# jenndrei/BayHunter

Hardware: AMD Instinct MI355X
Metric: forward-model+logL evals/sec (batched 10-layer models) (higher is better)
Workload: dtype f64

## Files before the change

bayhunter_amd/csrc/bh_device.h:

```cpp
#pragma once
#include <hip/hip_runtime.h>
#include <stddef.h>
#include <stdint.h>

#define BH_WAVE 64
#define BH_COUNTER_WORDS 16
#define BH_TRACE_WAVES 16384
#define BH_DEBUG_WORDS (BH_COUNTER_WORDS + 4 * BH_TRACE_WAVES)
#define BH_BOARD_WORDS (2 * 32768)

__device__ __forceinline__ double bh_rcp_refined(double b)
{
    double r = __builtin_amdgcn_rcp(b);
    double e = __builtin_fma(-b, r, 1.0);
    r = __builtin_fma(r, e, r);
    e = __builtin_fma(-b, r, 1.0);
    r = __builtin_fma(r, e, r);
    return r;
}
__device__ __forceinline__ double bh_quot(double a, double b, double r)
{
    const double q = a * r;
    const double rem = __builtin_fma(-b, q, a);
    return __builtin_fma(rem, r, q);
}
__device__ __forceinline__ bool bh_div_safe(double x)
{
    const unsigned ex = ((unsigned)__double2hiint(x) >> 20) & 0x7ffu;
    return (ex - 623u) <= 800u;
}

#include <atomic>
inline bool bh_allow_big_lds(std::atomic<unsigned long long> *done, const void *const *kernels, int nkernels, int bytes)
{
    int dev = 0;
    if (hipGetDevice(&dev) != hipSuccess || dev < 0 || dev > 63) return false;
    const unsigned long long bit = 1ull << dev;
    if (done->load(std::memory_order_acquire) & bit) return true;
    for (int k = 0; k < nkernels; ++k)
        if (hipFuncSetAttribute(kernels[k], hipFuncAttributeMaxDynamicSharedMemorySize, bytes) != hipSuccess) return false;
    done->fetch_or(bit, std::memory_order_release);
    return true;
}

struct SwdKernelArgs {
    int B, Lmax, K, igr, mode;
    const int32_t *nlay;
    const int32_t *perm;
    const double *h, *vp, *vs, *rho;
    ptrdiff_t sl, sb;
    const double *periods;
    double *vel;
    int ldv;
    int32_t *err;
    unsigned long long *neval;
    int look;
    int fair;
    double *nev_high;
    int fast;
    int counted;
    int farith;
    int32_t *gcount, *glist;
    int second, Bm;
    double *first;
};

struct SwdLaneBuild {
    int key[6];
    unsigned grid_x;
    int fair;
};
void bh_launch_swd(const SwdKernelArgs &a, int iwave, hipStream_t stream, SwdLaneBuild *build = nullptr);
void bh_launch_order(int B, const int32_t *nlay, int32_t *perm, int Lcut, int32_t *split, hipStream_t stream);
size_t bh_swd_lds_bytes(int Lmax, int K, int mode);
size_t bh_swd_nev_high_doubles(int B, int look);

struct SwdTarget {
    int iwave, igr, K, ldv, mode;
    int look;
    int inlook;
    const double *h, *vp, *vs, *rho;
    ptrdiff_t sl, sb;
    const double *periods;
    double *vel;
    int32_t *err;
    const int32_t *perm;
    const int32_t *count;
    int32_t *gcount, *glist;
    int refseq;
    double *first;
};
struct SwdMultiArgs {
    int B, Lmax, ntargets;
    const int32_t *nlay;
    const int32_t *perm;
    const int32_t *split;
    int Lcut;
    int rows[2], lanes[2];
    int wg_n0, wg_n1;
    unsigned long long *neval;
    unsigned *board;
    unsigned stamp;
    unsigned *started;
    int prio_low;
    int fast;
    int adapt_ok;
    int counted;
    int rerun;
    int farith;
    int restart;
    SwdTarget t[8];
};
struct SwdSiteXArgs {
    const int32_t *site;
    int nsites, nt, ldx;
    const int32_t *n;
    const double *x;
    int col[8], off[8];
};
__device__ __forceinline__ int bh_site_count(const SwdSiteXArgs &X, int ty, int ib, int cap)
{
    const int s = X.site[ib];
    if (s < 0 || s >= X.nsites) return -1;
    const int n = X.n[(size_t)s * X.nt + X.col[ty]];
    return n < 0 ? 0 : (n > cap ? cap : n);
}
__device__ __forceinline__ int bh_site_periods(const SwdSiteXArgs &X, int ty, int ib, int cap, const double *&per)
{
    const int n = bh_site_count(X, ty, ib, cap);
    per = n < 0 ? X.x : X.x + (size_t)X.site[ib] * X.ldx + X.off[ty];
    return n;
}
void bh_launch_swd_second_x(const SwdKernelArgs &a, int iwave, const SwdSiteXArgs &x, int ty, hipStream_t stream, SwdLaneBuild *build = nullptr);
int bh_swd_pick_group(int B, int ntargets, int Lmax);
double bh_swd_plan(int B, int Lmax, int ntargets, const int *iwave, int Gforce, int *G, int *look);
size_t bh_swd_group_lds_bytes(int G, int J, int Lmax, int Kmax, int maxmode, bool sitex = false);
struct SwdPairWork {
    int ncu = 0;
    int32_t *perm[2] = {nullptr, nullptr};
    int32_t *slot_rank[2] = {nullptr, nullptr};
    int cap_perm = 0, cap_rank[2] = {0, 0};
    int key_n0 = -1, key_n1 = -1;
};
struct PairOrderTarget {
    int mpw, nwaves;
    const int32_t *slot_rank;
    int32_t *perm;
    int xcd;
};
bool bh_pair_order_fits(int B);
void bh_launch_pair_order(int B, int Lmax, const int32_t *nlay, const double *vs, ptrdiff_t sl, ptrdiff_t sb, int nt,
                          const PairOrderTarget *tg, hipStream_t stream);
struct SwdLaunchInfo {
    unsigned workgroups;
    long waves;
    size_t lds;
    int wpb;
};
inline int bh_trials_fit(int G, int look)
{
    int J = look > 1 ? look : 1;
    while (J > 1 && G * J > BH_WAVE) --J;
    return J;
}
struct SwdGroupAsk {
    int B, Lmax, Lcut, ntargets;
    int G0;
    struct Target {
        int K, look, iwave, mode;
        bool group, refseq;
    } t[8];
    bool fast, farith, restart;
    bool adapt_ok, rerun;
    bool counters;
    bool sitex;
    int scan;
};
struct SwdGroupBuild {
    int fastm;
    bool simple, prof, adapt, cntb, fa;
};
struct SwdGroupPlan {
    bool fits;
    int rows[2], lanes[2];
    int wg_n0, wg_n1;
    size_t wave_lds, lds;
    dim3 grid, block;
    int Gflags;
    bool restart;
    SwdGroupBuild build;
    bool pair;
    int pair_mpw[2], pair_waves[2];
    SwdLaunchInfo info;
};
struct BhTuning;
SwdGroupPlan bh_plan_swd_group(const SwdGroupAsk &q, const BhTuning &tun);
void bh_launch_swd_group(const SwdMultiArgs &a, const SwdGroupPlan &g, hipStream_t stream);
bool bh_launch_swd_group_x(const SwdMultiArgs &a, const SwdGroupPlan &g, const SwdSiteXArgs &x, hipStream_t stream);
struct SwdGroupXStream {
    hipStream_t st;
    const SwdSiteXArgs *x;
};
bool bh_swd_group_builds_fa_x(const SwdMultiArgs &a, const SwdGroupPlan &g, SwdGroupXStream s);
bool bh_swd_group_builds_adapt_x(const SwdMultiArgs &a, const SwdGroupPlan &g, SwdGroupXStream s);
bool bh_swd_group_builds_big_x(const SwdMultiArgs &a, const SwdGroupPlan &g, SwdGroupXStream s);
bool bh_swd_group_builds_fa(const SwdMultiArgs &a, const SwdGroupPlan &g, hipStream_t stream);
bool bh_swd_group_builds_adapt(const SwdMultiArgs &a, const SwdGroupPlan &g, hipStream_t stream);
bool bh_swd_group_builds_big(const SwdMultiArgs &a, const SwdGroupPlan &g, hipStream_t stream);
int bh_swd_lean_trials(int B, int ntargets);
size_t bh_swd_lean_lds_bytes(int J, int Lmax, int Kmax, bool sitex = false);
int bh_launch_swd_lean(const SwdMultiArgs &a, hipStream_t stream, SwdLaunchInfo *info, SwdLaneBuild *build = nullptr);
int bh_launch_swd_lean_x(const SwdMultiArgs &a, const SwdSiteXArgs &x, hipStream_t stream, SwdLaunchInfo *info, SwdLaneBuild *build = nullptr);
void bh_launch_sphere(int B, int Lmax, const int32_t *nlay, const double *h, const double *vp,
                      const double *vs, const double *rho, ptrdiff_t sl, ptrdiff_t sb, double *oh,
                      double *ovp, double *ovs, double *orho_love, double *orho_ray, hipStream_t stream);
void bh_launch_interp(int B, int K0, const double *x0, const double *y0, int ld0, int K1,
                      const double *x1, double *y1, int ld1, hipStream_t stream);

struct RfKernelArgs {
    int B, Lmax, nsamp, nkeep, waveno;
    const int32_t *nlay;
    const double *h, *vp, *vs, *rho, *qp, *qs;
    ptrdiff_t sl, sb;
    double p_s_per_deg, gauss, fsamp, tshift, nsv;
    double *coef;
    double *rf;
    int ldr;
    const double *yobs;
    double *sums;
    double *zwork;
    int lds_min;
    int no_realc;
    int coef_small;
    int no_rot;
};
struct RfSiteArgs {
    const int32_t *site;
    int nsites;
    int ld;
    const double *p, *nsv;
};
size_t bh_rf_coef_doubles(int Lmax);
constexpr size_t BH_RF_MAX_LDS = 160 * 1024;
constexpr int BH_RF_MAX_NSAMP = 1 << 18;
size_t bh_rf_lds_bytes(int nsamp);
int bh_launch_rf(const RfKernelArgs &a, hipStream_t stream, const RfSiteArgs *sites = nullptr);
struct RfSiteMArgs : RfSiteArgs {
    const int32_t *n;
};
int bh_launch_rf_m(const RfKernelArgs &a, hipStream_t stream, const RfSiteMArgs &sites);
struct RfAxisRec {
    double fsamp, tshift, gauss;
    int32_t nsamp, logm, jcut;
    int32_t pad;
};
struct RfSiteTArgs : RfSiteMArgs {
    const RfAxisRec *axis;
    int nsamp_max;
};
RfAxisRec bh_rf_axis_record(int nsamp, double fsamp, double tshift, double gauss);
int bh_launch_rf_t(const RfKernelArgs &a, hipStream_t stream, const RfSiteTArgs &sites);
int bh_launch_rf_probe(int op, int n, const double *in, double *out, hipStream_t stream);

struct LikeTargetDev {
    int law, n, off;
    const double *yobs, *yerr_scaled, *rinv;
    double logdet_extra;
    const double *quad;
    int nsplit;
    const double *pre;
};
int bh_gauss_nsplit(int B, int n);
void bh_launch_gauss_quad(int B, int n, int ldy, const double *ymod, const double *yobs,
                          const double *rinv, int nsplit, double *partial, hipStream_t stream);
struct GaussSiteArgs {
    const int32_t *site;
    int nsites, ldo;
};
void bh_launch_gauss_quad_sites(int B, int n, int ldy, const double *ymod, const double *yobs, const GaussSiteArgs &sites,
                                const double *rinv, int nsplit, double *partial, hipStream_t stream);
struct GaussClassArgs {
    const int32_t *class_of;
    int nclass;
    const int32_t *row_start;
    const int32_t *tile_start;
    const int32_t *perm;
};
inline size_t bh_gauss_class_work_words(int B, int nclass) { return 4 * (size_t)nclass + 2 + (size_t)B; }
void bh_launch_gauss_quad_classes(int B, int n, int ldy, const double *ymod, const double *yobs, const GaussSiteArgs &sites,
                                  const int32_t *class_of, int nclass, const double *rinv, int nsplit, double *partial,
                                  int32_t *work, hipStream_t stream);
struct LikeKernelArgs {
    int B, nt, ldy;
    const double *ymod;
    const int32_t *err_t;
    const double *noise;
    LikeTargetDev t[8];
    double *logL;
    double *misfits;
    int32_t *err;
};
void bh_launch_like(const LikeKernelArgs &a, hipStream_t stream);
inline bool bh_like_small_form(const LikeKernelArgs &a, size_t *lds)
{
    *lds = 0;
    bool small = true;
    for (int t = 0; t < a.nt; ++t) {
        if (a.t[t].law == 3 && a.t[t].quad == nullptr && (size_t)a.t[t].n * sizeof(double) > *lds) *lds = (size_t)a.t[t].n * sizeof(double);
        small = small && (a.t[t].n <= 64 || (a.t[t].pre != nullptr && a.t[t].law != 3)) && !(a.t[t].law == 3 && a.t[t].quad == nullptr);
    }
    return small;
}
struct LikeSiteArgs {
    const int32_t *site;
    int nsites;
    const double *yobs;
    const double *yerr_scaled;
    const double *logdet_extra;
};
void bh_launch_like_sites(const LikeKernelArgs &a, const LikeSiteArgs &sites, hipStream_t stream);
struct LikeSiteXArgs : LikeSiteArgs {
    const int32_t *n;
};
void bh_launch_like_sites_x(const LikeKernelArgs &a, const LikeSiteXArgs &sites, hipStream_t stream);
void bh_launch_like_sites_m(const LikeKernelArgs &a, const LikeSiteXArgs &sites, hipStream_t stream);
struct LikeClassArgs {
    const int32_t *class_of[8];
    const double *rinv[8];
    const double *logdet[8];
};
void bh_launch_like_sites_c(const LikeKernelArgs &a, const LikeSiteXArgs &sites, const LikeClassArgs &classes, hipStream_t stream);
struct LikeLawArgs {
    const int32_t *law;
};
void bh_launch_like_sites_l(const LikeKernelArgs &a, const LikeSiteXArgs &sites, const LikeClassArgs &classes, const LikeLawArgs &laws,
                            hipStream_t stream);

void bh_launch_probe(int op, int n, const double *in, double *out, hipStream_t stream);


struct bh_engine;
__attribute__((visibility("hidden"))) int bh_engine_fail_internal(bh_engine *e, int code, const char *what);
__attribute__((visibility("hidden"))) int bh_engine_device_internal(const bh_engine *e);
```

bayhunter_amd/csrc/bh_engine.hip:

```cpp
#include "../../include/bh_engine_debug.h"
#include "../../include/bh_engine_sites.h"
#include "../../include/bh_engine_sites_rf.h"
#include "../../include/bh_engine_sites_x.h"
#include "../../include/bh_engine_sites_x_all.h"
#include "../../include/bh_engine_sites_missing.h"
#include "../../include/bh_engine_sites_gauss.h"
#include "../../include/bh_engine_sites_rf_axis.h"
#include "../../include/bh_engine_sites_laws.h"
#include "bh_device.h"

#include <algorithm>
#include <cmath>
#include <cstdio>
#include <cstdlib>
#include <cstring>
#include <new>
#include <string>
#include <vector>

#include "bh_tuning.h"
#include <cstring>
#include <mutex>

namespace {
BhTuning g_tuning;
std::once_flag g_tuning_once;
int tuning_value(const char *env, const char *txt, int dflt)
{
    if (!txt) return dflt;
    if (!std::strcmp(env, "BH_SWD_SEARCH")) return (txt[0] == 'f' || txt[0] == '1') ? ((std::strstr(txt, "ray") || txt[0] == '2') ? BH_SEARCH_FAST_RAYLEIGH : BH_SEARCH_FAST) : (txt[0] == '2' ? BH_SEARCH_FAST_RAYLEIGH : BH_SEARCH_REFERENCE);
    if (!std::strcmp(env, "BH_SWD_ARITH")) return (txt[0] == 'e' || txt[0] == '0') ? BH_ARITH_EXACT : BH_ARITH_FAST;
    if (!std::strcmp(env, "BH_SWD_SCAN")) return (txt[0] == 's' || txt[0] == '0') ? BH_SCAN_STEPS : ((txt[0] == 'c' || txt[0] == '1') ? BH_SCAN_COUNTED : BH_SCAN_AUTO);
    char *end = nullptr;
    const long v = std::strtol(txt, &end, 10);
    if (end == txt) return 1;
    return (int)v;
}
void tuning_clamp()
{
    if (g_tuning.rf_lds_gated < 0 || g_tuning.rf_lds_gated > 160 * 1024) g_tuning.rf_lds_gated = 0;
    if (g_tuning.rf_lds_beside > 160 * 1024) g_tuning.rf_lds_beside = -1;
    if (g_tuning.swd_love_inlook < 0 || g_tuning.swd_love_inlook > 4) g_tuning.swd_love_inlook = 0;
    if (g_tuning.swd_gsplit < 0 || g_tuning.swd_gsplit > (1 << 24)) g_tuning.swd_gsplit = 0;
}
void tuning_parse()
{
#ifndef BH_NO_EXPERIMENTS
#define X(field, env, dflt, doc) g_tuning.field = tuning_value(env, std::getenv(env), dflt);
    BH_TUNING_TABLE(X)
#undef X
    tuning_clamp();
#endif
    g_tuning.under_pmc = std::getenv("ROCPROF_COUNTER_COLLECTION") != nullptr ? 1 : 0;
}
}
const BhTuning &bh_tuning()
{
    std::call_once(g_tuning_once, tuning_parse);
    return g_tuning;
}
int bh_tuning_set(const char *name, int value)
{
#ifdef BH_NO_EXPERIMENTS
    (void)name; (void)value;
    return -1;
#else
    (void)bh_tuning();
    if (!name) return -1;
#define X(field, env, dflt, doc) if (!std::strcmp(name, #field)) { g_tuning.field = value; tuning_clamp(); return 0; }
    BH_TUNING_TABLE(X)
#undef X
    return -1;
#endif
}
int bh_tuning_get(const char *name, int *value)
{
    const BhTuning &t = bh_tuning();
    if (!name || !value) return -1;
#define X(field, env, dflt, doc) if (!std::strcmp(name, #field)) { *value = t.field; return 0; }
    BH_TUNING_TABLE(X)
#undef X
    return -1;
}

namespace {

struct DevBuf {
    void *p = nullptr;
    size_t cap = 0;
};

struct TargetHost {
    bh_target_desc d{};
    int off = 0;
    DevBuf x, yobs, yerr_scaled, rinv, quad;
    DevBuf sums;
    DevBuf x60, vel60;
    int kfwd = 0;
    double logdet_extra = 0.0;
    int gc_nclass = 0;
    DevBuf gc_rinv, gc_logdet, gc_class;
    bool site_lacks = false;
    bool law_other = false;
    bool rf_own_counts = false;
    int axis_nsamp_max = 0;
};

}

struct bh_engine {
    int device = 0;
    hipStream_t stream = nullptr;
    hipStream_t aux = nullptr;
    hipEvent_t ev_fork = nullptr, ev_join = nullptr;
    hipStream_t aux2 = nullptr;
    hipEvent_t ev_fork2 = nullptr, ev_join2 = nullptr;
    bool overlap_rf = true;
    int rf_lds_beside_swd = 40 * 1024;
    unsigned *started = nullptr;
    unsigned started_expected = 0;
    int swd_prio_low = 1;
    SwdPairWork pairwork{};
    int swd_trials = 0;
    int last_swd_kernel = -1;
    bh_swd_launch swd_launches[3 * BH_MAX_TARGETS]{};
    int n_swd_launches = 0;
    int err_t_nt = -1, err_t_B = -1;
    std::string err;
    DevBuf nlay, h, vp, vs, rho, qp, qs, periods, vel, errb, rf, coef, ymod, noise, logL,
        misfits, err_t, probe_in, probe_out, counter, sph, perm, board, nevhi, rfz, gfirst, nevhi2;
    unsigned swd_stamp = 0;
    int nt = 0;
    int ldy = 0;
    std::vector<TargetHost> targets;
    int nsites = 0;
    DevBuf site_yobs, site_yerr, site_logdet;
    DevBuf site_idx;
    bool site_rf = false;
    DevBuf site_p, site_nsv;
    bool site_rf_axis = false;
    DevBuf site_axis;
    bool site_x = false;
    bool site_x_all = false;
    bool site_missing = false;
    DevBuf site_xn, site_xper;
    std::vector<int32_t> site_xn_host;
    bool site_missing_gauss = false;
    DevBuf gc_xn;
    DevBuf gc_work;
    bool site_laws = false;
    DevBuf law_tab, law_yerr, law_logdet;
    std::vector<int32_t> site_law_host;
    bool timing = false, counting = false;
    bool no_mfma = false;
    bool as_given = false;
    int force_group = 0;
    int force_look = 0;
    int hint_layers = 0;
    int swd_search = BH_SEARCH_FAST;
    int swd_arith = BH_ARITH_FAST;
    int swd_scan = 2;
    DevBuf guard;
    uint64_t rerun_launches = 0;
    uint64_t guard_total[BH_MAX_TARGETS] = {0};
    bool guard_fresh = true;
    bool guard_last = false;
    struct EventSet {
        hipEvent_t ev[8];
        bool used[4];
    };
    std::vector<EventSet> evsets;
    size_t ncalls = 0;
    uint64_t last_neval = 0;
    bool neval_pending = false;
};

namespace {

int fail(bh_engine *e, int code, const char *what, hipError_t he = hipSuccess)
{
    if (e) {
        e->err = what;
        if (he != hipSuccess) {
            e->err += ": ";
            e->err += hipGetErrorString(he);
        }
    }
    return code;
}

#define HIPCHK(e, call)                                                  \
    do {                                                                 \
        hipError_t _he = (call);                                         \
        if (_he != hipSuccess) return fail((e), BH_EHIP, #call, _he);    \
    } while (0)

int ensure(bh_engine *e, DevBuf &b, size_t bytes)
{
    if (bytes <= b.cap) return BH_OK;
    if (b.p) {
        HIPCHK(e, hipStreamSynchronize(e->stream));
        if (e->aux) HIPCHK(e, hipStreamSynchronize(e->aux));
        if (e->aux2) HIPCHK(e, hipStreamSynchronize(e->aux2));
        HIPCHK(e, hipFree(b.p));
        b.p = nullptr;
        b.cap = 0;
    }
    size_t want = bytes + bytes / 4 + 256;
    hipError_t he = hipMalloc(&b.p, want);
    if (he != hipSuccess) return fail(e, BH_ENOMEM, "hipMalloc", he);
    b.cap = want;
    return BH_OK;
}

void release(DevBuf &b)
{
    if (b.p) (void)hipFree(b.p);
    b.p = nullptr;
    b.cap = 0;
}

void release_target(TargetHost &t)
{
    for (DevBuf *b : {&t.x, &t.yobs, &t.yerr_scaled, &t.rinv, &t.quad, &t.sums, &t.x60, &t.vel60, &t.gc_rinv, &t.gc_logdet, &t.gc_class}) release(*b);
    t.gc_nclass = 0;
}

void release_gauss_classes(bh_engine *e)
{
    for (auto &t : e->targets) {
        for (DevBuf *b : {&t.gc_rinv, &t.gc_logdet, &t.gc_class}) release(*b);
        t.gc_nclass = 0;
    }
    release(e->gc_xn);
}

void release_laws(bh_engine *e)
{
    for (DevBuf *b : {&e->law_tab, &e->law_yerr, &e->law_logdet}) release(*b);
    e->site_laws = false;
    e->site_law_host.clear();
    for (auto &t : e->targets) t.law_other = false;
    release_gauss_classes(e);
}

void release_sites(bh_engine *e)
{
    for (DevBuf *b : {&e->site_yobs, &e->site_yerr, &e->site_logdet, &e->site_idx, &e->site_p, &e->site_nsv, &e->site_xn, &e->site_xper, &e->site_axis}) release(*b);
    e->nsites = 0;
    e->site_rf = e->site_rf_axis = false;
    e->site_x = e->site_x_all = e->site_missing = e->site_missing_gauss = false;
    e->site_xn_host.clear();
    release_laws(e);
    for (auto &t : e->targets) {
        t.site_lacks = t.rf_own_counts = false;
        t.axis_nsamp_max = 0;
    }
}

double scaled_errors(const double *yerr, int n, double *out)
{
    double mn = yerr[0];
    for (int i = 0; i < n; ++i) mn = yerr[i] < mn ? yerr[i] : mn;
    double prod = 1.0;
    for (int i = 0; i < n; ++i) {
        out[i] = yerr[i] / mn;
        prod *= out[i];
    }
    return std::log(prod);
}

size_t span_elems(int B, int Lmax, ptrdiff_t sl, ptrdiff_t sb)
{
    return (size_t)((ptrdiff_t)(Lmax - 1) * sl + (ptrdiff_t)(B - 1) * sb + 1);
}

__global__ void rho_from_vp_kernel(size_t n, const double *vp, double *rho)
{
    const size_t i = (size_t)blockIdx.x * blockDim.x + threadIdx.x;
    if (i < n) rho[i] = vp[i] * 0.32 + 0.77;
}

int check_models(bh_engine *e, int B, int Lmax, ptrdiff_t sl, ptrdiff_t sb)
{
    if (!e) return BH_EINVAL;
    if (B < 0 || Lmax < 1 || Lmax > BH_MAX_LAYERS) return fail(e, BH_EINVAL, "bad B or Lmax (1..100)");
    if (sl <= 0 || sb <= 0) return fail(e, BH_EINVAL, "strides must be positive");
    return BH_OK;
}

struct Staged {
    const int32_t *nlay;
    const double *h, *vp, *vs, *rho, *qp, *qs;
    int typ_layers = 0;
};

int stage_models(bh_engine *e, int B, int Lmax, ptrdiff_t sl, ptrdiff_t sb, Staged &m)
{
    const size_t bytes = span_elems(B, Lmax, sl, sb) * sizeof(double);
    {
        long sum = 0;
        for (int b = 0; b < B; ++b) sum += m.nlay[b];
        m.typ_layers = B > 0 ? (int)((sum + B - 1) / B) : 0;
    }
    int rc;
    if ((rc = ensure(e, e->nlay, (size_t)B * sizeof(int32_t)))) return rc;
    HIPCHK(e, hipMemcpyAsync(e->nlay.p, m.nlay, (size_t)B * sizeof(int32_t), hipMemcpyHostToDevice, e->stream));
    m.nlay = (const int32_t *)e->nlay.p;
    const double **arr[6] = {&m.h, &m.vp, &m.vs, &m.rho, &m.qp, &m.qs};
    DevBuf *buf[6] = {&e->h, &e->vp, &e->vs, &e->rho, &e->qp, &e->qs};
    for (int k = 0; k < 6; ++k) {
        if (!*arr[k]) continue;
        if ((rc = ensure(e, *buf[k], bytes))) return rc;
        HIPCHK(e, hipMemcpyAsync(buf[k]->p, *arr[k], bytes, hipMemcpyHostToDevice, e->stream));
        *arr[k] = (const double *)buf[k]->p;
    }
    return BH_OK;
}

bh_engine::EventSet *cur_set(bh_engine *e)
{
    return (e->timing && e->ncalls > 0) ? &e->evsets[e->ncalls - 1] : nullptr;
}
void ev_begin(bh_engine *e, int fam, hipStream_t st)
{
    bh_engine::EventSet *s = cur_set(e);
    if (!s) return;
    if (!s->used[fam]) {
        (void)hipEventRecord(s->ev[2 * fam], st);
        s->used[fam] = true;
    }
}
void ev_end(bh_engine *e, int fam, hipStream_t st)
{
    bh_engine::EventSet *s = cur_set(e);
    if (s) (void)hipEventRecord(s->ev[2 * fam + 1], st);
}
void call_begin(bh_engine *e, hipStream_t st)
{
    e->neval_pending = false;
    if (!e->timing) return;
    if (e->ncalls == e->evsets.size()) {
        bh_engine::EventSet s{};
        for (auto &ev : s.ev)
            if (hipEventCreate(&ev) != hipSuccess) return;
        e->evsets.push_back(s);
    }
    bh_engine::EventSet &s = e->evsets[e->ncalls++];
    for (bool &u : s.used) u = false;
    (void)hipEventRecord(s.ev[6], st);
    s.used[3] = true;
}
void call_end(bh_engine *e, hipStream_t st)
{
    bh_engine::EventSet *s = cur_set(e);
    if (s) (void)hipEventRecord(s->ev[7], st);
}

int swd_supported(bh_engine *e, int K, int iwave, int &igr, int mode, int flsph)
{
    if (K < 0 || K > BH_MAX_PERIODS) return fail(e, BH_EINVAL, "K must be 0..60 (surfdisp96.f:61-62)");
    if (iwave != BH_WAVE_LOVE && iwave != BH_WAVE_RAYLEIGH) return fail(e, BH_EINVAL, "iwave must be 1 (Love) or 2 (Rayleigh)");
    if (igr < 0) return fail(e, BH_EINVAL, "igr must be 0 (phase velocity) or > 0 (group velocity)");
    if (mode < 1 || mode > 16) return fail(e, BH_EINVAL, "mode must be 1..16");
    if (flsph != 0 && flsph != 1) return fail(e, BH_EINVAL, "flsph must be 0 or 1");
    igr = igr > 0 ? BH_VEL_GROUP : BH_VEL_PHASE;
    return BH_OK;
}

struct SwdSiteJob {
    const SwdSiteXArgs *tab;
    int col, off;
};

struct SwdJob {
    int K, iwave, igr, ldv;
    const double *periods_dev;
    double *vel;
    int32_t *err;
    int mode = 1;
    int flsph = 0;
    SwdSiteJob sx{};
};

int swd_counter(bh_engine *e, hipStream_t st, unsigned long long **out)
{
    *out = nullptr;
    if (!e->counting) return BH_OK;
    int rc = ensure(e, e->counter, BH_DEBUG_WORDS * sizeof(unsigned long long));
    if (rc) return rc;
    if (!e->neval_pending) {
        HIPCHK(e, hipMemsetAsync(e->counter.p, 0, BH_COUNTER_WORDS * sizeof(unsigned long long), st));
        e->neval_pending = true;
    }
    *out = (unsigned long long *)e->counter.p;
    return BH_OK;
}

constexpr int GUARD_HEAD = 24;
int guard_space(bh_engine *e, hipStream_t st, int B, int32_t **counts, int32_t **lists)
{
    const size_t need = ((size_t)GUARD_HEAD + (size_t)BH_MAX_TARGETS * (size_t)(B + 4)) * sizeof(int32_t);
    if (need > e->guard.cap) {
        if (e->guard.p) {
            int32_t cum[BH_MAX_TARGETS];
            HIPCHK(e, hipStreamSynchronize(st));
            HIPCHK(e, hipMemcpy(cum, (int32_t *)e->guard.p + 2 * BH_MAX_TARGETS, sizeof(cum), hipMemcpyDeviceToHost));
            for (int t = 0; t < BH_MAX_TARGETS; ++t) e->guard_total[t] += (uint64_t)(uint32_t)cum[t];
        }
        e->guard_fresh = true;
    }
    int rc = ensure(e, e->guard, need);
    if (rc) return rc;
    *counts = (int32_t *)e->guard.p;
    *lists = (int32_t *)e->guard.p + GUARD_HEAD;
    HIPCHK(e, hipMemsetAsync(e->guard.p, 0, (e->guard_fresh ? GUARD_HEAD : 2 * BH_MAX_TARGETS) * sizeof(int32_t), st));
    e->guard_fresh = false;
    return BH_OK;
}

bool takes_fast(int search, const SwdJob &J)
{
    return J.igr == BH_VEL_PHASE && J.mode <= 1 && (search == BH_SEARCH_FAST || (search == BH_SEARCH_FAST_RAYLEIGH && J.iwave == BH_WAVE_RAYLEIGH));
}

enum SwdOrder { ORDER_NONE, ORDER_DEPTH, ORDER_LENGTH, ORDER_PAIR };

struct SwdPlan {
    bool first_roots[BH_MAX_TARGETS];
    int nsplit;
    int ntargets, kmax, maxmode;
    bool any_sphere;
    int typ_layers;
    int kernel;
    int G, lean_trials;
    int order, Lcut;
    int len_mpw, len_xcd;
    bool sitex;
    bool any_fast, farith, adapt_ok;
    int job[BH_MAX_TARGETS], look[BH_MAX_TARGETS], inlook[BH_MAX_TARGETS], look_group[BH_MAX_TARGETS];
    bool fast[BH_MAX_TARGETS], refseq[BH_MAX_TARGETS];
};

SwdPlan plan_swd(const bh_engine *e, int B, int Lmax, int typ_given, int njobs, const SwdJob *jobs)
{
    const BhTuning &tun = bh_tuning();
    SwdPlan p{};
    p.maxmode = 1;
    for (int j = 0; j < njobs; ++j) p.sitex = p.sitex || jobs[j].sx.tab != nullptr;
    int iw[BH_MAX_TARGETS], nfast = 0;
    for (int j = 0; j < njobs; ++j) {
        const SwdJob &J = jobs[j];
        if (J.K == 0) continue;
        p.first_roots[j] = J.igr == BH_VEL_GROUP && J.mode <= 1 && tun.swd_gsplit > 0 && (long)B * J.K <= (long)tun.swd_gsplit;
        p.nsplit += p.first_roots[j] ? 1 : 0;
        const int t = p.ntargets++;
        p.job[t] = j;
        iw[t] = J.iwave;
        p.fast[t] = takes_fast(e->swd_search, J);
        nfast += p.fast[t] ? 1 : 0;
        p.kmax = J.K > p.kmax ? J.K : p.kmax;
        p.maxmode = J.mode > p.maxmode ? J.mode : p.maxmode;
        p.any_sphere = p.any_sphere || J.flsph == 1;
    }
    const int nlive = p.ntargets;
    if (nlive == 0) return p;
    p.typ_layers = ((long)nlive * B <= 2048 && tun.swd_hint_always == 0) ? 0 : typ_given;
    int look[BH_MAX_TARGETS];
    {
        int Lplan = p.typ_layers > 0 ? p.typ_layers : Lmax;
        if (Lplan > Lmax) Lplan = Lmax;
        bh_swd_plan(B, Lplan, nlive, iw, e->force_group, &p.G, look);
        if (e->force_look > 0)
            for (int t = 0; t < nlive; ++t) look[t] = e->force_look;
    }
    const size_t lds_cap = 64 * 1024;
    if (p.G <= 1 && (p.sitex || bh_swd_lds_bytes(Lmax, p.kmax, p.maxmode) > lds_cap)) p.G = 2;
    {
        bool all = e->swd_arith == BH_ARITH_FAST && e->swd_search == BH_SEARCH_FAST && e->force_group == 0 && e->force_look == 0 &&
                   tun.swd_look_r == 0 && tun.swd_look_l == 0 && tun.swd_no_lean == 0 && p.maxmode <= 1 && p.kmax <= BH_MAX_PERIODS &&
                   Lmax <= 32 && (long)B * nlive <= (tun.swd_lean_pairs > 0 ? (long)tun.swd_lean_pairs : (1L << 20));
        for (int t = 0; t < nlive; ++t) all = all && jobs[p.job[t]].igr == BH_VEL_PHASE;
        if (all) p.lean_trials = e->swd_trials > 0 ? e->swd_trials : bh_swd_lean_trials(B, nlive);
        if (p.lean_trials >= 4 && bh_swd_lean_lds_bytes(p.lean_trials, Lmax, p.kmax, p.sitex) > lds_cap) p.lean_trials = 0;
    }
    const bool lean = p.lean_trials >= 4;
    if (lean && p.G <= 1) p.G = bh_swd_pick_group(B, nlive, Lmax);
    p.kernel = p.G <= 1 ? BH_KERNEL_LANE : (lean ? BH_KERNEL_LEAN : BH_KERNEL_GROUP);
    const bool ordered = B > 1 && tun.no_order == 0 && !e->as_given;
    const bool shallow_bulk = p.typ_layers > 0 && p.typ_layers + 2 < Lmax;
    if (ordered && !lean && tun.swd_no_pair == 0 && p.G > 1 && nlive == 2 && bh_pair_order_fits(B) && !shallow_bulk) {
        long plan_waves = 0, wmin = 0, wmax = 0;
        for (int t = 0; t < nlive; ++t) {
            const int mpw = BH_WAVE / (p.G * bh_trials_fit(p.G, look[t]));
            const long w = (B + mpw - 1) / mpw;
            plan_waves += w;
            wmin = (t == 0 || w < wmin) ? w : wmin;
            wmax = w > wmax ? w : wmax;
        }
        const int pair_min = tun.swd_pair_minwaves;
        if (plan_waves >= (pair_min >= 0 ? pair_min : 7 * (long)e->pairwork.ncu) && (pair_min >= 0 || 2 * wmax >= 3 * wmin))
            p.order = ORDER_PAIR;
    }
    p.Lcut = Lmax;
    if (ordered && p.order != ORDER_PAIR) {
        if (lean && bh_pair_order_fits(B) && tun.swd_lean_no_sort == 0) {
            p.order = ORDER_LENGTH;
            p.len_mpw = 1;
            const int mpw = BH_WAVE / p.lean_trials, per_wg = (nlive == 2) ? 2 : 4;
            if (tun.swd_lean_xcd != 0 && tun.swd_lean_r < 4 && tun.swd_lean_l < 4 && B % mpw == 0 && B % 8 == 0 && (B / mpw) % (8 * per_wg) == 0) {
                p.len_mpw = mpw;
                p.len_xcd = per_wg;
            }
        } else {
            p.order = ORDER_DEPTH;
            if (shallow_bulk) p.Lcut = p.typ_layers + 2;
        }
    }
    p.any_fast = nfast > 0;
    p.farith = e->swd_arith == BH_ARITH_FAST;
    p.adapt_ok = e->force_group == 0 && e->force_look == 0 && tun.swd_look_r == 0 && tun.swd_look_l == 0;
    for (int t = 0; t < nlive; ++t) {
        p.refseq[t] = nfast > 0 && jobs[p.job[t]].igr == BH_VEL_PHASE && !p.fast[t];
        if (p.kernel == BH_KERNEL_LANE) {
            p.look[t] = look[t] > 1 ? look[t] : 1;
            continue;
        }
        p.inlook[t] = (iw[t] != BH_WAVE_LOVE) ? 1 : (tun.swd_love_inlook > 0 ? tun.swd_love_inlook : (look[t] <= 2 ? 2 : 1));
        int L = look[t];
        if (tun.swd_look_r > 0 && iw[t] == BH_WAVE_RAYLEIGH) L = tun.swd_look_r;
        if (tun.swd_look_l > 0 && iw[t] == BH_WAVE_LOVE) L = tun.swd_look_l;
        p.look_group[t] = L;
        if (lean) {
            L = p.lean_trials;
            if (iw[t] == BH_WAVE_RAYLEIGH && tun.swd_lean_r >= 4) L = tun.swd_lean_r;
            if (iw[t] == BH_WAVE_LOVE && tun.swd_lean_l >= 4) L = tun.swd_lean_l;
        }
        p.look[t] = L;
    }
    return p;
}

enum EvalRole { ROLE_NONE, ROLE_SWD, ROLE_SWD60, ROLE_RF };
enum EvalLike { LIKE_PLAIN, LIKE_SITES, LIKE_SITES_X, LIKE_SITES_M, LIKE_SITES_C, LIKE_SITES_L };
enum EvalGauss { GAUSS_PLAIN, GAUSS_SITES, GAUSS_CLASSES };

struct EvalPlan {
    int B, nt, ldy;
    EvalRole role[BH_MAX_TARGETS];
    bool rf_fused[BH_MAX_TARGETS];
    int nswd;
    bool no_forward;
    bool fork;
    bool want_gate;
    int prio_low;
    bool x_table, rf_table;
    bool missing;
    bool rf_needs_table;
    bool rf_axis;
    bool rf_axis_needs_table;
    bool rf_axis_gauss_needs_table;
    bool rf_axis_no_mfma;
    EvalGauss gauss[BH_MAX_TARGETS];
    bool gauss_needs_table;
    bool laws;
    bool law_gauss_needs_table;
    EvalLike like;
    bool err_zero_always;
};

EvalPlan plan_eval(const bh_engine *e, int B, bool sites, bool want_ymod)
{
    const BhTuning &tun = bh_tuning();
    EvalPlan p{};
    p.B = B; p.nt = e->nt; p.ldy = e->ldy;
    bool have_rf = false;
    for (int t = 0; t < p.nt; ++t) {
        const TargetHost &T = e->targets[(size_t)t];
        const bh_target_desc &d = T.d;
        if (d.kind == BH_TARGET_SWD) {
            p.role[t] = T.kfwd == d.n ? ROLE_SWD : ROLE_SWD60;
            ++p.nswd;
        } else if (d.kind == BH_TARGET_RF) {
            p.role[t] = ROLE_RF;
            have_rf = true;
            p.rf_fused[t] = !want_ymod && !sites && tun.rf_no_fuse == 0 && (d.law == BH_LAW_NOCORR || d.law == BH_LAW_EXP) && tun.rf_threads != 128;
        } else {
            p.no_forward = true;
        }
    }
    p.fork = have_rf && p.nswd > 0 && e->overlap_rf;
    p.want_gate = p.fork && e->started != nullptr;
    p.prio_low = p.want_gate ? e->swd_prio_low : 0;
    p.x_table = sites && e->site_x;
    p.rf_table = sites && e->site_rf;
    p.missing = p.x_table && e->site_missing;
    p.rf_needs_table = p.missing && have_rf && !p.rf_table;
    p.rf_axis = p.rf_table && p.x_table && e->site_rf_axis;
    p.like = p.missing ? LIKE_SITES_M : (p.x_table ? LIKE_SITES_X : (sites ? LIKE_SITES : LIKE_PLAIN));
    for (int t = 0; t < p.nt; ++t) {
        const TargetHost &T = e->targets[(size_t)t];
        p.gauss[t] = !sites ? GAUSS_PLAIN : (T.gc_nclass > 0 ? GAUSS_CLASSES : GAUSS_SITES);
        if (sites && T.rf_own_counts && !p.rf_axis) p.rf_axis_needs_table = true;
        if (T.d.law != BH_LAW_GAUSS) continue;
        if (p.gauss[t] == GAUSS_CLASSES) p.like = LIKE_SITES_C;
        else if (sites && e->site_missing_gauss && T.site_lacks) p.gauss_needs_table = true;
        else if (sites && T.rf_own_counts) p.rf_axis_gauss_needs_table = true;
        if (sites && T.rf_own_counts && e->no_mfma) p.rf_axis_no_mfma = true;
    }
    p.laws = p.x_table && e->site_laws;
    if (p.laws) {
        p.like = LIKE_SITES_L;
        for (int t = 0; t < p.nt; ++t) {
            const TargetHost &T = e->targets[(size_t)t];
            if (T.d.law == BH_LAW_GAUSS && T.law_other && p.gauss[t] != GAUSS_CLASSES) p.law_gauss_needs_table = true;
        }
    }
    p.err_zero_always = tun.err_memset != 0;
    return p;
}

unsigned gate_need(const SwdLaunchInfo &s)
{
    const unsigned resident = 2048u / (unsigned)(s.lds > 0 && s.wpb > 0 ? s.wpb : 2);
    return s.workgroups < resident ? s.workgroups : resident;
}

struct RfPlace {
    int lds_min = 0, coef_small = 0;
};

RfPlace rf_place(bool beside_swd, bool gated, const BhTuning &tun, int rf_lds_beside_swd)
{
    RfPlace w;
    if (!beside_swd) return w;
    w.lds_min = !gated ? rf_lds_beside_swd : (tun.rf_lds_gated > 0 ? tun.rf_lds_gated : 0);
    w.coef_small = (gated && tun.rf_coef_big == 0) ? 1 : 0;
    return w;
}

SwdGroupPlan plan_group(const bh_engine *e, const SwdPlan &p, int B, int Lmax, const SwdJob *jobs)
{
    SwdGroupAsk q{};
    q.B = B; q.Lmax = Lmax; q.Lcut = p.Lcut; q.ntargets = p.ntargets; q.G0 = p.G;
    for (int t = 0; t < p.ntargets; ++t) {
        const SwdJob &J = jobs[p.job[t]];
        q.t[t] = SwdGroupAsk::Target{J.K, p.look[t], J.iwave, J.mode, J.igr != BH_VEL_PHASE, p.refseq[t]};
    }
    q.fast = p.any_fast; q.farith = p.farith;
    q.restart = true;
    q.adapt_ok = p.adapt_ok; q.counters = e->counting; q.scan = e->swd_scan; q.sitex = p.sitex;
    return bh_plan_swd_group(q, bh_tuning());
}

struct SwdCall {
    bh_engine *e; hipStream_t st;
    int B, Lmax; const Staged &m; ptrdiff_t sl, sb;
    const SwdJob *jobs; const SwdPlan &p;
    const double *sph = nullptr;
    double *first[BH_MAX_TARGETS] = {};
    SwdGroupPlan g{};
    const int32_t *perm = nullptr, *split = nullptr;
    const int32_t *pair_perm[2] = {};
    unsigned long long *counter = nullptr;
    int32_t *gcounts = nullptr, *glists = nullptr;
    SwdSiteXArgs sx{};
    int prio_low = 0;
    SwdLaunchInfo info{};
};

SwdTarget swd_target(const SwdCall &c, int j)
{
    const SwdJob &J = c.jobs[j];
    SwdTarget t{};
    t.iwave = J.iwave; t.igr = c.p.first_roots[j] ? 2 : J.igr; t.K = J.K; t.ldv = J.ldv; t.mode = J.mode;
    t.h = c.m.h; t.vp = c.m.vp; t.vs = c.m.vs; t.rho = c.m.rho; t.sl = c.sl; t.sb = c.sb;
    if (J.flsph == 1) {
        const size_t ne = (size_t)c.Lmax * c.B;
        t.h = c.sph; t.vp = c.sph + ne; t.vs = c.sph + 2 * ne; t.rho = c.sph + (J.iwave == BH_WAVE_LOVE ? 3 : 4) * ne;
        t.sl = c.B; t.sb = 1;
    }
    t.periods = J.periods_dev; t.vel = J.vel; t.err = J.err;
    t.first = c.first[j];
    return t;
}

SwdKernelArgs lane_args(const SwdCall &c, const SwdTarget &t)
{
    SwdKernelArgs a{};
    a.B = c.B; a.Lmax = c.Lmax; a.K = t.K; a.igr = t.igr; a.mode = t.mode; a.perm = c.perm;
    a.nlay = c.m.nlay; a.h = t.h; a.vp = t.vp; a.vs = t.vs; a.rho = t.rho; a.sl = t.sl; a.sb = t.sb;
    a.periods = t.periods; a.vel = t.vel; a.ldv = t.ldv; a.err = t.err; a.first = t.first;
    a.neval = c.counter; a.counted = c.e->swd_scan;
    return a;
}

int swd_board(bh_engine *e, hipStream_t st, unsigned **board)
{
    if (!e->board.p) {
        int rc = ensure(e, e->board, (size_t)BH_BOARD_WORDS * sizeof(unsigned));
        if (rc) return rc;
        HIPCHK(e, hipMemsetAsync(e->board.p, 0, (size_t)BH_BOARD_WORDS * sizeof(unsigned), st));
    }
    *board = (unsigned *)e->board.p;
    return BH_OK;
}

unsigned swd_stamp(bh_engine *e)
{
    const unsigned s = (++e->swd_stamp) & 0xffffu;
    return s != 0 ? s : (++e->swd_stamp) & 0xffffu;
}

int wait_for(bh_engine *e, hipEvent_t ev, hipStream_t from, hipStream_t to)
{
    HIPCHK(e, hipEventRecord(ev, from));
    HIPCHK(e, hipStreamWaitEvent(to, ev, 0));
    return BH_OK;
}

void note_launch(bh_engine *e, int family, int role, const int key[6], bool two, bool inter, bool pair, bool restart, unsigned grid_x, int fair)
{
    if (e->n_swd_launches >= (int)(sizeof(e->swd_launches) / sizeof(e->swd_launches[0]))) return;
    bh_swd_launch &r = e->swd_launches[e->n_swd_launches++];
    r.family = family; r.role = role;
    for (int k = 0; k < 6; ++k) r.key[k] = key[k];
    r.two_classes = two; r.interleaved = inter; r.pair_order = pair; r.restart = restart; r.grid_x = (int)grid_x; r.fair = fair;
}
void note_lane(bh_engine *e, int role, const SwdLaneBuild &b) { note_launch(e, BH_KERNEL_LANE, role, b.key, false, false, false, false, b.grid_x, b.fair); }
void note_group(bh_engine *e, int role, const SwdGroupPlan &g, bool pair)
{
    const SwdGroupBuild &b = g.build;
    const int key[6] = {b.fastm, b.simple, b.prof, b.adapt, b.cntb, b.fa};
    note_launch(e, BH_KERNEL_GROUP, role, key, g.grid.z == 2, g.wg_n1 > 0, pair, g.restart, g.grid.x, 0);
}

void set_group_args(SwdMultiArgs &a, const SwdGroupPlan &g)
{
    for (int k = 0; k < 2; ++k) {
        a.rows[k] = g.rows[k];
        a.lanes[k] = g.lanes[k];
    }
    a.wg_n0 = g.wg_n0;
    a.wg_n1 = g.wg_n1;
    a.fast = g.build.fastm;
    a.counted = g.build.cntb ? 1 : 0;
    a.farith = g.build.fa ? 1 : 0;
    a.restart = g.restart ? 1 : 0;
}

bool build_slot_ranks(int n0, int n1, int ncu, std::vector<int32_t> rank[2])
{
    const int NW = n0 + n1, nwg = (NW + 1) / 2;
    if (ncu <= 0 || nwg > 4 * ncu) return false;
    auto target_of = [&](int W, int &ty, int &wid) {
        if (n1 > 0) {
            const long long N = NW;
            const int l0 = (int)(((long long)W * n1) / N), l1 = (int)((((long long)W + 1) * n1) / N);
            ty = (l1 > l0) ? 1 : 0;
            wid = (l1 > l0) ? l0 : W - l0;
        } else {
            ty = 0;
            wid = W;
        }
    };
    std::vector<int> on_simd[2];
    on_simd[0].assign((size_t)ncu * 4, -1);
    on_simd[1].assign((size_t)ncu * 4, -1);
    for (int W = 0; W < NW; ++W) {
        const int g = W / 2, j = W % 2, cu = g % ncu, pass = g / ncu, simd = (pass + j) % 4;
        on_simd[j][(size_t)cu * 4 + simd] = W;
    }
    std::vector<double> q((size_t)NW, 0.0);
    int npairs = 0;
    for (size_t k = 0; k < on_simd[0].size(); ++k) npairs += (on_simd[0][k] >= 0 && on_simd[1][k] >= 0);
    int ip = 0;
    for (size_t k = 0; k < on_simd[0].size(); ++k) {
        const int a = on_simd[0][k], b = on_simd[1][k];
        if (a >= 0 && b >= 0) {
            const double u = (ip + 0.5) / (2.0 * npairs);
            q[(size_t)((ip & 1) ? a : b)] = u;
            q[(size_t)((ip & 1) ? b : a)] = 1.0 - u;
            ++ip;
        } else if (a >= 0) {
            q[(size_t)a] = 0.0;
        } else if (b >= 0) {
            q[(size_t)b] = 0.0;
        }
    }
    const int nw[2] = {n0, n1};
    for (int t = 0; t < 2; ++t) {
        std::vector<std::pair<double, int>> v;
        for (int W = 0; W < NW; ++W) {
            int ty, wid;
            target_of(W, ty, wid);
            if (ty == t && wid < nw[t] - 1) v.emplace_back(q[(size_t)W], wid);
        }
        std::sort(v.begin(), v.end());
        rank[t].assign((size_t)(nw[t] > 0 ? nw[t] : 1), 0);
        for (size_t r = 0; r < v.size(); ++r) rank[t][(size_t)v[r].second] = (int32_t)r;
    }
    return true;
}

int launch_swd_rerun(bh_engine *e, hipStream_t st, const SwdMultiArgs &main, int32_t *counts, int32_t *lists, const SwdSiteXArgs *sx = nullptr)
{
    SwdMultiArgs a = main;
    a.rerun = 1;
    a.perm = nullptr;
    a.split = nullptr;
    a.Lcut = a.Lmax;
    a.started = nullptr;
    a.stamp = swd_stamp(e);
    a.adapt_ok = 1;
    SwdGroupAsk q{};
    q.B = a.B; q.Lmax = q.Lcut = a.Lmax; q.ntargets = a.ntargets;
    q.G0 = bh_swd_pick_group(a.B, a.ntargets, a.Lmax);
    for (int t = 0; t < a.ntargets; ++t) {
        SwdTarget &T = a.t[t];
        T.perm = lists + (size_t)t * (size_t)(a.B + 4);
        T.count = counts + t;
        T.gcount = nullptr;
        T.glist = nullptr;
        T.look = 64 / q.G0 > 1 ? 64 / q.G0 : 1;
        T.inlook = 1;
        q.t[t] = SwdGroupAsk::Target{T.K, T.look, T.iwave, T.mode, T.igr != 0, T.refseq != 0};
    }
    q.adapt_ok = q.rerun = true; q.counters = a.neval != nullptr; q.scan = e->swd_scan; q.sitex = sx != nullptr;
    const SwdGroupPlan g = bh_plan_swd_group(q, bh_tuning());
    if (!g.fits) return fail(e, BH_EINVAL, "model too deep for LDS");
    set_group_args(a, g);
    if (sx == nullptr) bh_launch_swd_group(a, g, st);
    else if (!bh_launch_swd_group_x(a, g, *sx, st)) return fail(e, BH_EUNSUPPORTED, "no site-period build of this dispersion launch");
    note_group(e, BH_SWD_RERUN, g, false);
    HIPCHK(e, hipGetLastError());
    ++e->rerun_launches;
    return BH_OK;
}

int pair_models(SwdCall &c)
{
    SwdPairWork &pw = c.e->pairwork;
    const SwdGroupPlan &g = c.g;
    const int nt = c.p.ntargets, B = c.B;
    const int *n = g.pair_waves;
    bool ok = true, geom = true;
    if (pw.key_n0 != n[0] || pw.key_n1 != n[1]) {
        std::vector<int32_t> rank[2];
        geom = build_slot_ranks(n[0], n[1], pw.ncu, rank);
        for (int t = 0; ok && geom && t < nt; ++t) {
            if (pw.cap_rank[t] < n[t]) {
                if (pw.slot_rank[t]) (void)hipFree(pw.slot_rank[t]);
                pw.slot_rank[t] = nullptr;
                ok = hipMalloc((void **)&pw.slot_rank[t], (size_t)(n[t] + 64) * sizeof(int32_t)) == hipSuccess;
                pw.cap_rank[t] = ok ? n[t] + 64 : 0;
            }
            if (ok) {
                ok = hipStreamSynchronize(c.st) == hipSuccess &&
                     hipMemcpy(pw.slot_rank[t], rank[t].data(), (size_t)n[t] * sizeof(int32_t), hipMemcpyHostToDevice) == hipSuccess;
            }
        }
        pw.key_n0 = (ok && geom) ? n[0] : -1;
        pw.key_n1 = (ok && geom) ? n[1] : -1;
    }
    if (ok && pw.cap_perm < B) {
        for (int t = 0; t < 2; ++t) {
            if (pw.perm[t]) (void)hipFree(pw.perm[t]);
            pw.perm[t] = nullptr;
            ok = ok && hipStreamSynchronize(c.st) == hipSuccess &&
                 hipMalloc((void **)&pw.perm[t], (size_t)(B + B / 4 + 64) * sizeof(int32_t)) == hipSuccess;
        }
        pw.cap_perm = ok ? B + B / 4 + 64 : 0;
    }
    if (ok) {
        PairOrderTarget tg[2];
        for (int t = 0; t < nt; ++t) tg[t] = PairOrderTarget{g.pair_mpw[t], n[t], geom ? pw.slot_rank[t] : nullptr, pw.perm[t]};
        const SwdTarget t0 = swd_target(c, c.p.job[0]);
        bh_launch_pair_order(B, c.Lmax, c.m.nlay, t0.vs, t0.sl, t0.sb, nt, tg, c.st);
        for (int t = 0; t < nt; ++t) c.pair_perm[t] = pw.perm[t];
    }
    (void)hipGetLastError();
    return BH_OK;
}

int order_models(SwdCall &c)
{
    const SwdPlan &p = c.p;
    if (p.order == ORDER_NONE) return BH_OK;
    if (p.order == ORDER_PAIR) return c.g.pair ? pair_models(c) : BH_OK;
    bh_engine *e = c.e;
    int rc;
    if ((rc = ensure(e, e->perm, ((size_t)c.B + 4) * sizeof(int32_t)))) return rc;
    int32_t *perm = (int32_t *)e->perm.p;
    if (p.order == ORDER_LENGTH) {
        const PairOrderTarget tg{p.len_mpw, c.B / p.len_mpw, nullptr, perm + 4, p.len_xcd};
        bh_launch_pair_order(c.B, c.Lmax, c.m.nlay, c.m.vs, c.sl, c.sb, 1, &tg, c.st);
    } else {
        bh_launch_order(c.B, c.m.nlay, perm + 4, p.Lcut, perm, c.st);
        c.split = (p.Lcut < c.Lmax) ? perm : nullptr;
    }
    c.perm = perm + 4;
    return BH_OK;
}

int launch_swd_lanes(SwdCall &c, SwdMultiArgs &ra)
{
    bh_engine *e = c.e;
    const SwdPlan &p = c.p;
    const int B = c.B, n = p.ntargets;
    const bool fork = n > 1 && e->aux2 != nullptr;
    int rc;
    size_t nev_off[BH_MAX_TARGETS + 1] = {0};
    for (int t = 0; t < n; ++t) nev_off[t + 1] = nev_off[t] + bh_swd_nev_high_doubles(B, p.look[t]);
    if ((rc = ensure(e, e->nevhi, nev_off[n] * sizeof(double)))) return rc;
    long lane_waves = 0;
    for (int t = 0; t < n; ++t) lane_waves += (long)((B + 63) / 64) * p.look[t];
    e->guard_last = p.any_fast;
    ra.B = B; ra.Lmax = c.Lmax; ra.nlay = c.m.nlay; ra.neval = c.counter; ra.counted = e->swd_scan;
    if (p.any_fast && ((rc = guard_space(e, c.st, B, &c.gcounts, &c.glists)) || (rc = swd_board(e, c.st, &ra.board)))) return rc;
    e->last_swd_kernel = BH_KERNEL_LANE;
    ev_begin(e, 0, c.st);
    if (fork && (rc = wait_for(e, e->ev_fork2, c.st, e->aux2))) return rc;
    for (int t = 0; t < n; ++t) {
        const SwdTarget tg = swd_target(c, p.job[t]);
        SwdKernelArgs a = lane_args(c, tg);
        a.look = p.look[t];
        a.fair = lane_waves <= 1024 ? -1 : (lane_waves <= 2048 ? 18 : 12);
        a.nev_high = (double *)e->nevhi.p + nev_off[t];
        a.fast = p.fast[t] ? 1 : 0;
        a.farith = (p.fast[t] && p.farith) ? 1 : 0;
        if (a.fast) {
            a.gcount = c.gcounts + t;
            a.glist = c.glists + (size_t)t * (size_t)(B + 4);
        }
        SwdLaneBuild lb{};
        bh_launch_swd(a, tg.iwave, (fork && (t & 1)) ? e->aux2 : c.st, &lb);
        note_lane(e, BH_SWD_MAIN, lb);
        ra.t[ra.ntargets++] = tg;
    }
    if (fork && (rc = wait_for(e, e->ev_join2, e->aux2, c.st))) return rc;
    HIPCHK(e, hipGetLastError());
    return BH_OK;
}

int launch_swd_multi(SwdCall &c, SwdMultiArgs &a)
{
    bh_engine *e = c.e;
    const SwdPlan &p = c.p;
    const int B = c.B;
    int rc;
    if ((rc = swd_board(e, c.st, &a.board))) return rc;
    a.stamp = swd_stamp(e);
    a.B = B; a.Lmax = c.Lmax; a.nlay = c.m.nlay; a.neval = c.counter; a.perm = c.perm;
    a.split = c.split; a.Lcut = p.Lcut;
    a.ntargets = p.ntargets;
    for (int t = 0; t < p.ntargets; ++t) {
        a.t[t] = swd_target(c, p.job[t]);
        a.t[t].look = p.look[t];
        a.t[t].inlook = p.inlook[t];
        a.t[t].refseq = p.refseq[t] ? 1 : 0;
    }
    a.started = e->started;
    a.prio_low = c.prio_low;
    a.adapt_ok = p.adapt_ok ? 1 : 0;
    if (p.sitex) {
        c.sx = *c.jobs[p.job[0]].sx.tab;
        for (int t = 0; t < p.ntargets; ++t) {
            c.sx.col[t] = c.jobs[p.job[t]].sx.col;
            c.sx.off[t] = c.jobs[p.job[t]].sx.off;
        }
    }
    const bool lean = p.kernel == BH_KERNEL_LEAN;
    if (lean) {
        a.counted = e->swd_scan;
        a.farith = p.farith ? 1 : 0;
        a.fast = p.any_fast ? 1 : 0;
    } else {
        for (int t = 0; t < 2; ++t) a.t[t].perm = c.pair_perm[t];
        set_group_args(a, c.g);
    }
    if (bh_tuning().debug_plan != 0) {
        std::fprintf(stderr, "[bh] dispersion plan B=%d Lmax=%d: lanes per model %d, typical layers %d (hint %d), Lcut %d%s, pairing %d; trials per round:",
                     B, c.Lmax, p.G, c.m.typ_layers, e->hint_layers, p.Lcut, p.Lcut < c.Lmax ? " (two depth classes)" : "", (int)(p.order == ORDER_PAIR));
        for (int t = 0; t < p.ntargets; ++t) std::fprintf(stderr, " %s %d/%d", a.t[t].iwave == BH_WAVE_LOVE ? "L" : "R", p.look_group[t], p.inlook[t]);
        if (!lean) std::fprintf(stderr, "; launched lanes per model %d/%d", c.g.lanes[0], c.g.lanes[1]);
        std::fprintf(stderr, "\n");
    }
    e->guard_last = p.any_fast;
    if (p.any_fast) {
        if ((rc = guard_space(e, c.st, B, &c.gcounts, &c.glists))) return rc;
        for (int t = 0; t < a.ntargets; ++t)
            if (a.t[t].igr == BH_VEL_PHASE) {
                a.t[t].gcount = c.gcounts + t;
                a.t[t].glist = c.glists + (size_t)t * (size_t)(B + 4);
            }
    }
    ev_begin(e, 0, c.st);
    e->last_swd_kernel = p.kernel;
    if (lean) {
        SwdLaneBuild lb{};
        if ((p.sitex ? bh_launch_swd_lean_x(a, c.sx, c.st, &c.info, &lb) : bh_launch_swd_lean(a, c.st, &c.info, &lb)) != 0)
            return fail(e, BH_EINVAL, "model too deep for LDS");
        note_launch(e, BH_KERNEL_LEAN, BH_SWD_MAIN, lb.key, false, p.ntargets == 2, false, false, lb.grid_x, 0);
    } else {
        if (!p.sitex) bh_launch_swd_group(a, c.g, c.st);
        else if (!bh_launch_swd_group_x(a, c.g, c.sx, c.st)) return fail(e, BH_EUNSUPPORTED, "no site-period build of this dispersion launch");
        note_group(e, BH_SWD_MAIN, c.g, c.pair_perm[0] != nullptr);
        c.info = c.g.info;
    }
    const hipError_t le = hipGetLastError();
    if (le != hipSuccess) return fail(e, BH_EHIP, "dispersion kernel launch", le);
    if (e->started) e->started_expected += c.info.workgroups;
    return BH_OK;
}

int launch_second_roots(const SwdCall &c)
{
    bh_engine *e = c.e;
    const int B = c.B;
    const bool sitex = c.p.sitex && e->site_x_all;
    int J2 = 16;
    {
        long searches = 0;
        for (int t = 0; t < c.p.ntargets; ++t) searches += c.p.first_roots[c.p.job[t]] ? (long)B * c.jobs[c.p.job[t]].K : 0;
        while (J2 > 1 && searches * J2 > 2048L * 64) J2 >>= 1;
    }
    size_t off[BH_MAX_TARGETS + 1] = {0};
    int n = 0;
    for (int t = 0; t < c.p.ntargets; ++t)
        if (c.p.first_roots[c.p.job[t]]) {
            off[n + 1] = off[n] + bh_swd_nev_high_doubles(B * c.jobs[c.p.job[t]].K, J2);
            ++n;
        }
    int rc = ensure(e, e->nevhi2, off[n] * sizeof(double));
    if (rc) return rc;
    const bool fork = n > 1 && e->aux2 != nullptr;
    if (fork && (rc = wait_for(e, e->ev_fork2, c.st, e->aux2))) return rc;
    n = 0;
    for (int t = 0; t < c.p.ntargets; ++t) {
        if (!c.p.first_roots[c.p.job[t]]) continue;
        const SwdTarget tg = swd_target(c, c.p.job[t]);
        SwdKernelArgs a = lane_args(c, tg);
        a.B = B * tg.K; a.Bm = B; a.second = 1;
        a.igr = BH_VEL_GROUP; a.mode = 1; a.perm = nullptr;
        a.look = J2;
        const long waves = ((long)a.B * J2 + 63) / 64;
        a.fair = waves <= 1024 ? -1 : (waves <= 2048 ? 18 : 12);
        a.nev_high = (double *)e->nevhi2.p + off[n];
        SwdLaneBuild lb{};
        if (sitex) bh_launch_swd_second_x(a, tg.iwave, c.sx, t, (fork && (n & 1)) ? e->aux2 : c.st, &lb);
        else bh_launch_swd(a, tg.iwave, (fork && (n & 1)) ? e->aux2 : c.st, &lb);
        note_lane(e, BH_SWD_SECOND, lb);
        ++n;
    }
    if (fork && (rc = wait_for(e, e->ev_join2, e->aux2, c.st))) return rc;
    HIPCHK(e, hipGetLastError());
    return BH_OK;
}

int launch_swd_jobs(bh_engine *e, hipStream_t st, int B, int Lmax, const Staged &m, ptrdiff_t sl,
                    ptrdiff_t sb, int njobs, const SwdJob *jobs, int prio_low, SwdLaunchInfo *main)
{
    if (B == 0 || njobs == 0) return BH_OK;
    const SwdPlan p = plan_swd(e, B, Lmax, m.typ_layers > 0 ? m.typ_layers : e->hint_layers, njobs, jobs);
    SwdCall c{e, st, B, Lmax, m, sl, sb, jobs, p};
    c.prio_low = prio_low;
    if (p.kernel == BH_KERNEL_GROUP) {
        c.g = plan_group(e, p, B, Lmax, jobs);
        if (!c.g.fits) return fail(e, BH_EINVAL, "model too deep for LDS");
    }
    int rc;
    if (p.nsplit > 0) {
        if ((rc = ensure(e, e->gfirst, (size_t)p.nsplit * B * sizeof(double)))) return rc;
        int n = 0;
        for (int j = 0; j < njobs; ++j)
            if (p.first_roots[j]) c.first[j] = (double *)e->gfirst.p + (size_t)(n++) * B;
    }
    if (p.ntargets == 0) return BH_OK;
    e->n_swd_launches = 0;
    if (p.any_sphere) {
        const size_t ne = (size_t)Lmax * B;
        if ((rc = ensure(e, e->sph, 5 * ne * sizeof(double)))) return rc;
        double *base = (double *)e->sph.p;
        bh_launch_sphere(B, Lmax, m.nlay, m.h, m.vp, m.vs, m.rho, sl, sb, base, base + ne, base + 2 * ne, base + 3 * ne, base + 4 * ne, st);
        c.sph = base;
    }
    if ((rc = swd_counter(e, st, &c.counter)) || (rc = order_models(c))) return rc;
    SwdMultiArgs a{};
    rc = p.kernel == BH_KERNEL_LANE ? launch_swd_lanes(c, a) : launch_swd_multi(c, a);
    if (main) *main = c.info;
    if (!rc && p.any_fast && !(p.kernel == BH_KERNEL_GROUP && c.g.restart)) rc = launch_swd_rerun(e, st, a, c.gcounts, c.glists, p.sitex ? &c.sx : nullptr);
    if (!rc && p.nsplit > 0) rc = launch_second_roots(c);
    ev_end(e, 0, st);
    return rc;
}

struct RfJob {
    double p, gauss;
    int nsamp;
    double fsamp, tshift, nsv;
    int waveno, nkeep;
    double *rf; int ldr;
    const double *yobs; double *sums;
    const RfSiteArgs *sites;
    const RfSiteMArgs *msites;
    const RfSiteTArgs *tsites;
};

int launch_rf(bh_engine *e, hipStream_t st, int B, int Lmax, const Staged &m, ptrdiff_t sl, ptrdiff_t sb, const RfJob &j, const RfPlace &where)
{
    if (B == 0) return BH_OK;
    int rc;
    if ((rc = ensure(e, e->coef, (size_t)B * bh_rf_coef_doubles(Lmax) * sizeof(double)))) return rc;
    RfKernelArgs a{};
    a.B = B; a.Lmax = Lmax; a.nsamp = j.nsamp; a.nkeep = j.nkeep; a.waveno = j.waveno;
    a.nlay = m.nlay; a.h = m.h; a.vp = m.vp; a.vs = m.vs; a.rho = m.rho; a.qp = m.qp; a.qs = m.qs;
    a.sl = sl; a.sb = sb;
    a.p_s_per_deg = j.p; a.gauss = j.gauss; a.fsamp = j.fsamp; a.tshift = j.tshift; a.nsv = j.nsv;
    a.coef = (double *)e->coef.p; a.rf = j.rf; a.ldr = j.ldr;
    a.yobs = j.yobs; a.sums = j.sums;
    if (!j.tsites && bh_rf_lds_bytes(j.nsamp) > BH_RF_MAX_LDS) {
        if ((rc = ensure(e, e->rfz, (size_t)B * (size_t)(j.nsamp / 2) * 2 * sizeof(double)))) return rc;
        a.zwork = (double *)e->rfz.p;
    }
    a.lds_min = where.lds_min;
    a.coef_small = where.coef_small;
    ev_begin(e, 1, st);
    const int lrc = j.tsites ? bh_launch_rf_t(a, st, *j.tsites) : j.msites ? bh_launch_rf_m(a, st, *j.msites) : bh_launch_rf(a, st, j.sites);
    ev_end(e, 1, st);
    if (lrc != 0) return fail(e, BH_EUNSUPPORTED, "receiver function: nsamp above 262144 is not supported");
    HIPCHK(e, hipGetLastError());
    return BH_OK;
}

int prepare_like_target(bh_engine *e, hipStream_t st, int B, int ldy, const double *ymod_d, TargetHost &T,
                        LikeTargetDev &L, bool fused, const int32_t *site, EvalGauss how)
{
    L.law = T.d.law; L.n = T.d.n; L.off = T.off;
    L.yobs = (const double *)T.yobs.p;
    L.yerr_scaled = (const double *)T.yerr_scaled.p;
    L.rinv = (const double *)T.rinv.p;
    L.logdet_extra = T.logdet_extra;
    L.quad = nullptr;
    L.nsplit = 0;
    L.pre = fused ? (const double *)T.sums.p : nullptr;
    if (T.d.law == BH_LAW_GAUSS && !e->no_mfma) {
        const int nsplit = bh_gauss_nsplit(B, T.d.n);
        int rc = ensure(e, T.quad, (size_t)B * nsplit * sizeof(double));
        if (rc) return rc;
        if (how == GAUSS_CLASSES && (rc = ensure(e, e->gc_work, bh_gauss_class_work_words(B, T.gc_nclass) * sizeof(int32_t)))) return rc;
        ev_begin(e, 2, st);
        if (how == GAUSS_CLASSES) {
            const GaussSiteArgs gs{site, e->nsites, ldy};
            bh_launch_gauss_quad_classes(B, T.d.n, ldy, ymod_d + T.off, (const double *)e->site_yobs.p + T.off, gs, (const int32_t *)T.gc_class.p,
                                         T.gc_nclass, (const double *)T.gc_rinv.p, nsplit, (double *)T.quad.p, (int32_t *)e->gc_work.p, st);
        } else if (site) {
            const GaussSiteArgs gs{site, e->nsites, ldy};
            bh_launch_gauss_quad_sites(B, T.d.n, ldy, ymod_d + T.off, (const double *)e->site_yobs.p + T.off, gs, L.rinv, nsplit,
                                       (double *)T.quad.p, st);
        } else {
            bh_launch_gauss_quad(B, T.d.n, ldy, ymod_d + T.off, L.yobs, L.rinv, nsplit, (double *)T.quad.p, st);
        }
        L.quad = (const double *)T.quad.p;
        L.nsplit = nsplit;
    }
    return BH_OK;
}

int rf_args_ok(bh_engine *e, int nsamp, int nkeep, double gauss, double fsamp, int waveno)
{
    if (nsamp < 4 || (nsamp & (nsamp - 1)) != 0)
        return fail(e, BH_EINVAL, "nsamp must be a power of two >= 4");
    if (nsamp > BH_RF_MAX_NSAMP)
        return fail(e, BH_EUNSUPPORTED, "nsamp above 262144 is not supported");
    if (nkeep < 0 || nkeep > nsamp) return fail(e, BH_EINVAL, "nkeep must be 0..nsamp");
    if (!(gauss > 0.0) || !(fsamp > 0.0)) return fail(e, BH_EINVAL, "gauss and fsamp must be > 0");
    if (waveno != BH_RF_P && waveno != BH_RF_SV) return fail(e, BH_EINVAL, "waveno must be 0 (P) or 1 (SV)");
    return BH_OK;
}

}

extern "C" {

int bh_abi_version(void) { return BH_ABI_VERSION; }

int bh_engine_create(int device, bh_engine **out)
{
    if (!out) return BH_EINVAL;
    *out = nullptr;
    int ndev = 0;
    if (hipGetDeviceCount(&ndev) != hipSuccess || ndev <= 0) return BH_EHIP;
    if (device < 0 || device >= ndev) return BH_EINVAL;
    bh_engine *e = new (std::nothrow) bh_engine;
    if (!e) return BH_ENOMEM;
    e->device = device;
    if (hipSetDevice(device) != hipSuccess || hipStreamCreate(&e->stream) != hipSuccess ||
        hipStreamCreateWithFlags(&e->aux, hipStreamNonBlocking) != hipSuccess ||
        hipEventCreateWithFlags(&e->ev_fork, hipEventDisableTiming) != hipSuccess ||
        hipEventCreateWithFlags(&e->ev_join, hipEventDisableTiming) != hipSuccess ||
        hipStreamCreateWithFlags(&e->aux2, hipStreamNonBlocking) != hipSuccess ||
        hipEventCreateWithFlags(&e->ev_fork2, hipEventDisableTiming) != hipSuccess ||
        hipEventCreateWithFlags(&e->ev_join2, hipEventDisableTiming) != hipSuccess) {
        delete e;
        return BH_EHIP;
    }
    const BhTuning &tun = bh_tuning();
    if (tun.no_overlap) e->overlap_rf = false;
    if (tun.rf_lds_beside >= 0) e->rf_lds_beside_swd = tun.rf_lds_beside;
    {
        hipDeviceProp_t prop;
        e->pairwork.ncu = (hipGetDeviceProperties(&prop, device) == hipSuccess) ? prop.multiProcessorCount : 0;
    }
    if (tun.swd_prio_low >= 0) e->swd_prio_low = tun.swd_prio_low != 0 ? 1 : 0;
    {
        int can = 0;
        (void)hipDeviceGetAttribute(&can, hipDeviceAttributeCanUseStreamWaitValue, device);
        if (tun.no_started) can = 0;
        if (tun.under_pmc) can = 0;
        if (can && hipMalloc((void **)&e->started, 8) != hipSuccess) e->started = nullptr;
        if (e->started && hipMemset(e->started, 0, 8) != hipSuccess) {
            (void)hipFree(e->started);
            e->started = nullptr;
        }
        (void)hipGetLastError();
    }
    e->force_group = tun.swd_group;
    e->force_look = tun.swd_lookahead;
    if (tun.swd_search >= 0) e->swd_search = tun.swd_search;
    if (tun.swd_arith >= 0) e->swd_arith = tun.swd_arith != 0 ? BH_ARITH_FAST : BH_ARITH_EXACT;
    if (tun.swd_scan >= 0) e->swd_scan = tun.swd_scan;
    if (tun.no_mfma) e->no_mfma = true;
    *out = e;
    return BH_OK;
}

int bh_engine_set_typical_layers(bh_engine *e, int nlay)
{
    if (!e) return BH_EINVAL;
    if (nlay < 0 || nlay > BH_MAX_LAYERS) return fail(e, BH_EINVAL, "typical layer count must be 0 (unknown) or 1..100");
    e->hint_layers = nlay;
    return BH_OK;
}

int bh_engine_set_model_order(bh_engine *e, int sort_by_depth)
{
    if (!e) return BH_EINVAL;
    e->as_given = (sort_by_depth == 0);
    return BH_OK;
}

int bh_engine_set_swd_search(bh_engine *e, int search)
{
    if (!e) return BH_EINVAL;
    if (search != BH_SEARCH_REFERENCE && search != BH_SEARCH_FAST && search != BH_SEARCH_FAST_RAYLEIGH)
        return fail(e, BH_EINVAL, "search must be BH_SEARCH_REFERENCE (0), BH_SEARCH_FAST (1) or BH_SEARCH_FAST_RAYLEIGH (2)");
    e->swd_search = search;
    return BH_OK;
}

int bh_engine_get_swd_search(const bh_engine *e) { return e ? e->swd_search : 0; }

int bh_engine_set_swd_scan(bh_engine *e, int scan)
{
    if (!e) return BH_EINVAL;
    if (scan != BH_SCAN_STEPS && scan != BH_SCAN_COUNTED && scan != BH_SCAN_AUTO) return fail(e, BH_EINVAL, "scan must be BH_SCAN_STEPS, BH_SCAN_COUNTED or BH_SCAN_AUTO");
    e->swd_scan = scan;
    return BH_OK;
}
int bh_engine_get_swd_scan(const bh_engine *e) { return e ? e->swd_scan : 0; }

int bh_engine_set_tuning(bh_engine *e, const char *name, int value)
{
    if (!e) return BH_EINVAL;
    if (bh_tuning_set(name, value) != 0) return fail(e, BH_EINVAL, "unknown experiment switch (csrc/bh_tuning.h), or a build with BH_NO_EXPERIMENTS");
    return BH_OK;
}
int bh_engine_get_tuning(bh_engine *e, const char *name, int *value)
{
    if (!e) return BH_EINVAL;
    if (bh_tuning_get(name, value) != 0) return fail(e, BH_EINVAL, "unknown experiment switch (csrc/bh_tuning.h)");
    return BH_OK;
}

int bh_engine_set_swd_arith(bh_engine *e, int arith)
{
    if (!e) return BH_EINVAL;
    if (arith != BH_ARITH_EXACT && arith != BH_ARITH_FAST) return fail(e, BH_EINVAL, "arith must be BH_ARITH_EXACT (0) or BH_ARITH_FAST (1)");
    e->swd_arith = arith;
    return BH_OK;
}
int bh_engine_get_swd_arith(const bh_engine *e) { return e ? e->swd_arith : 0; }
int bh_engine_last_swd_kernel(const bh_engine *e) { return e ? e->last_swd_kernel : -1; }
int bh_engine_last_swd_launches(const bh_engine *e, bh_swd_launch *out, int max, int *n)
{
    if (!e || !n || max < 0 || (max > 0 && !out)) return BH_EINVAL;
    const int m = e->n_swd_launches < max ? e->n_swd_launches : max;
    for (int i = 0; i < m; ++i) out[i] = e->swd_launches[i];
    *n = m;
    return BH_OK;
}
int bh_engine_set_swd_trials(bh_engine *e, int trials)
{
    if (!e) return BH_EINVAL;
    if (trials != 0 && trials != 4 && trials != 8 && trials != 16 && trials != 32 && trials != 64)
        return fail(e, BH_EINVAL, "trials must be 0 (by the call's shape), 4, 8, 16, 32 or 64");
    e->swd_trials = trials;
    return BH_OK;
}
int bh_engine_get_swd_trials(const bh_engine *e) { return e ? e->swd_trials : 0; }
int bh_engine_guard_stats(bh_engine *e, int32_t *counts, uint64_t *rerun_launches, uint64_t *total)
{
    if (!e) return BH_EINVAL;
    if (rerun_launches) *rerun_launches = e->rerun_launches;
    if (counts || total) {
        int32_t w[3 * BH_MAX_TARGETS] = {0};
        if (e->guard.p && !e->guard_fresh) {
            HIPCHK(e, hipDeviceSynchronize());
            HIPCHK(e, hipMemcpy(w, e->guard.p, sizeof(w), hipMemcpyDeviceToHost));
        }
        if (counts)
            for (int t = 0; t < BH_MAX_TARGETS; ++t) counts[t] = e->guard_last ? w[t] + w[BH_MAX_TARGETS + t] : 0;
        if (total)
            for (int t = 0; t < BH_MAX_TARGETS; ++t) total[t] = e->guard_total[t] + (uint64_t)(uint32_t)w[2 * BH_MAX_TARGETS + t];
    }
    return BH_OK;
}

int bh_engine_set_swd_lookahead(bh_engine *e, int trials_per_round)
{
    if (!e) return BH_EINVAL;
    if (trials_per_round < 0 || trials_per_round > 16)
        return fail(e, BH_EINVAL, "look-ahead must be 0 (auto) or 1..16 trial velocities per round");
    e->force_look = trials_per_round;
    return BH_OK;
}

int bh_engine_set_swd_group(bh_engine *e, int lanes_per_model)
{
    if (!e) return BH_EINVAL;
    if (lanes_per_model < 0 || lanes_per_model > 32)
        return fail(e, BH_EINVAL, "lanes per model must be 0 (auto) or 1..32");
    e->force_group = lanes_per_model;
    return BH_OK;
}

void bh_engine_destroy(bh_engine *e)
{
    if (!e) return;
    (void)hipSetDevice(e->device);
    (void)hipStreamSynchronize(e->stream);
    for (DevBuf *b : {&e->nlay, &e->h, &e->vp, &e->vs, &e->rho, &e->qp, &e->qs, &e->periods, &e->vel,
                      &e->errb, &e->rf, &e->coef, &e->ymod, &e->noise, &e->logL, &e->misfits,
                      &e->err_t, &e->probe_in, &e->probe_out, &e->counter, &e->sph, &e->perm, &e->board, &e->nevhi, &e->guard, &e->rfz, &e->gfirst, &e->nevhi2, &e->gc_work})
        release(*b);
    for (auto &t : e->targets) {
        release_target(t);
    }
    release_sites(e);
    for (auto &s : e->evsets)
        for (auto &ev : s.ev)
            if (ev) (void)hipEventDestroy(ev);
    if (e->started) (void)hipFree(e->started);
    for (int t = 0; t < 2; ++t) {
        if (e->pairwork.perm[t]) (void)hipFree(e->pairwork.perm[t]);
        if (e->pairwork.slot_rank[t]) (void)hipFree(e->pairwork.slot_rank[t]);
    }
    if (e->ev_fork) (void)hipEventDestroy(e->ev_fork);
    if (e->ev_join) (void)hipEventDestroy(e->ev_join);
    if (e->aux) (void)hipStreamDestroy(e->aux);
    if (e->ev_fork2) (void)hipEventDestroy(e->ev_fork2);
    if (e->ev_join2) (void)hipEventDestroy(e->ev_join2);
    if (e->aux2) (void)hipStreamDestroy(e->aux2);
    (void)hipStreamDestroy(e->stream);
    delete e;
}

const char *bh_engine_last_error(const bh_engine *e) { return e ? e->err.c_str() : "null engine"; }

}

int bh_engine_fail_internal(bh_engine *e, int code, const char *what) { return fail(e, code, what); }
int bh_engine_device_internal(const bh_engine *e) { return e->device; }

extern "C" {
void *bh_engine_stream(bh_engine *e) { return e ? (void *)e->stream : nullptr; }

int bh_engine_synchronize(bh_engine *e)
{
    if (!e) return BH_EINVAL;
    HIPCHK(e, hipStreamSynchronize(e->stream));
    return BH_OK;
}

int bh_engine_set_instrumentation(bh_engine *e, int timing, int counting)
{
    if (!e) return BH_EINVAL;
    e->timing = timing != 0;
    e->counting = counting != 0;
    return BH_OK;
}

int bh_timing_reset(bh_engine *e)
{
    if (!e) return BH_EINVAL;
    e->ncalls = 0;
    return BH_OK;
}

int bh_timing_collect(bh_engine *e, int *ncalls, double *total_ms, double family_ms[3])
{
    if (!e) return BH_EINVAL;
    double tot = 0.0, fam[3] = {0.0, 0.0, 0.0};
    for (size_t i = 0; i < e->ncalls; ++i) {
        bh_engine::EventSet &s = e->evsets[i];
        HIPCHK(e, hipEventSynchronize(s.ev[7]));
        float ms = 0.f;
        HIPCHK(e, hipEventElapsedTime(&ms, s.ev[6], s.ev[7]));
        tot += ms;
        for (int f = 0; f < 3; ++f) {
            if (!s.used[f]) continue;
            float fm = 0.f;
            HIPCHK(e, hipEventElapsedTime(&fm, s.ev[2 * f], s.ev[2 * f + 1]));
            fam[f] += fm;
        }
    }
    if (ncalls) *ncalls = (int)e->ncalls;
    if (total_ms) *total_ms = tot;
    if (family_ms)
        for (int f = 0; f < 3; ++f) family_ms[f] = fam[f];
    return BH_OK;
}

int bh_timing_steps(bh_engine *e, int max, double *step_ms, int *n)
{
    if (!e || !step_ms || !n || max < 0) return BH_EINVAL;
    int k = 0;
    for (size_t i = 0; i < e->ncalls && k < max; ++i, ++k) {
        bh_engine::EventSet &s = e->evsets[i];
        HIPCHK(e, hipEventSynchronize(s.ev[7]));
        float ms = 0.f;
        if (i + 1 < e->ncalls) HIPCHK(e, hipEventElapsedTime(&ms, s.ev[6], e->evsets[i + 1].ev[6]));
        else HIPCHK(e, hipEventElapsedTime(&ms, s.ev[6], s.ev[7]));
        step_ms[k] = ms;
    }
    *n = k;
    return BH_OK;
}

int bh_debug_counters(bh_engine *e, uint64_t out[16])
{
    if (!e || !out) return BH_EINVAL;
    if (!e->counter.p) return fail(e, BH_EINVAL, "counting was never enabled");
    HIPCHK(e, hipStreamSynchronize(e->stream));
    HIPCHK(e, hipMemcpy(out, e->counter.p, 16 * sizeof(uint64_t), hipMemcpyDeviceToHost));
    return BH_OK;
}

int bh_debug_trace(bh_engine *e, uint64_t *out, int nwaves)
{
    if (!e || !out || nwaves < 0 || nwaves > BH_TRACE_WAVES) return BH_EINVAL;
    if (!e->counter.p) return fail(e, BH_EINVAL, "counting was never enabled");
    HIPCHK(e, hipStreamSynchronize(e->stream));
    HIPCHK(e, hipMemcpy(out, (uint64_t *)e->counter.p + BH_COUNTER_WORDS, (size_t)4 * nwaves * sizeof(uint64_t), hipMemcpyDeviceToHost));
    return BH_OK;
}

int bh_last_neval(bh_engine *e, uint64_t *neval)
{
    if (!e || !neval) return BH_EINVAL;
    if (e->neval_pending) {
        unsigned long long v = 0;
        HIPCHK(e, hipMemcpy(&v, e->counter.p, sizeof(v), hipMemcpyDeviceToHost));
        e->last_neval = v;
        e->neval_pending = false;
    }
    *neval = e->last_neval;
    return BH_OK;
}

int bh_swd_batch(bh_engine *e, int memspace, void *stream, int B, int Lmax, const int32_t *nlay,
                 const double *h, const double *vp, const double *vs, const double *rho,
                 ptrdiff_t sl, ptrdiff_t sb, int K, const double *periods, int iwave, int igr,
                 int mode, int flsph, double *vel, int32_t *err)
{
    int rc;
    if ((rc = check_models(e, B, Lmax, sl, sb))) return rc;
    if ((rc = swd_supported(e, K, iwave, igr, mode, flsph))) return rc;
    if (!nlay || !h || !vp || !vs || !rho || !periods || !vel || !err) return fail(e, BH_EINVAL, "null argument");
    if (B == 0) return BH_OK;
    HIPCHK(e, hipSetDevice(e->device));
    const bool host = (memspace != BH_DEVICE);
    hipStream_t st = (!host && stream) ? (hipStream_t)stream : e->stream;
    Staged m{nlay, h, vp, vs, rho, nullptr, nullptr};
    SwdJob job{K, iwave, igr, K, periods, vel, err, mode, flsph};
    if (host) {
        if ((rc = stage_models(e, B, Lmax, sl, sb, m))) return rc;
        if ((rc = ensure(e, e->periods, (size_t)BH_MAX_PERIODS * sizeof(double)))) return rc;
        if ((rc = ensure(e, e->vel, (size_t)B * K * sizeof(double)))) return rc;
        if ((rc = ensure(e, e->errb, (size_t)B * sizeof(int32_t)))) return rc;
        HIPCHK(e, hipMemcpyAsync(e->periods.p, periods, (size_t)K * sizeof(double), hipMemcpyHostToDevice, st));
        job.periods_dev = (const double *)e->periods.p; job.vel = (double *)e->vel.p; job.err = (int32_t *)e->errb.p;
    }
    call_begin(e, st);
    rc = launch_swd_jobs(e, st, B, Lmax, m, sl, sb, 1, &job, 0, nullptr);
    call_end(e, st);
    if (rc || !host) return rc;
    HIPCHK(e, hipMemcpyAsync(vel, e->vel.p, (size_t)B * K * sizeof(double), hipMemcpyDeviceToHost, st));
    HIPCHK(e, hipMemcpyAsync(err, e->errb.p, (size_t)B * sizeof(int32_t), hipMemcpyDeviceToHost, st));
    HIPCHK(e, hipStreamSynchronize(st));
    return BH_OK;
}

int bh_rf_batch(bh_engine *e, int memspace, void *stream, int B, int Lmax, const int32_t *nlay,
                const double *h, const double *vp, const double *vs, const double *rho,
                const double *qp, const double *qs, ptrdiff_t sl, ptrdiff_t sb, double p,
                double gauss, int nsamp, double fsamp, double tshift, double nsv, int waveno,
                int nkeep, double *rf)
{
    int rc;
    if ((rc = check_models(e, B, Lmax, sl, sb))) return rc;
    if ((rc = rf_args_ok(e, nsamp, nkeep, gauss, fsamp, waveno))) return rc;
    if (!nlay || !h || !vp || !vs || !rho || !rf) return fail(e, BH_EINVAL, "null argument");
    if (B == 0 || nkeep == 0) return BH_OK;
    HIPCHK(e, hipSetDevice(e->device));
    const bool host = (memspace != BH_DEVICE);
    hipStream_t st = (!host && stream) ? (hipStream_t)stream : e->stream;
    Staged m{nlay, h, vp, vs, rho, qp, qs};
    RfJob job{p, gauss, nsamp, fsamp, tshift, nsv, waveno, nkeep, rf, nkeep, nullptr, nullptr, nullptr};
    if (host) {
        if ((rc = stage_models(e, B, Lmax, sl, sb, m))) return rc;
        if ((rc = ensure(e, e->rf, (size_t)B * nkeep * sizeof(double)))) return rc;
        job.rf = (double *)e->rf.p;
    }
    call_begin(e, st);
    rc = launch_rf(e, st, B, Lmax, m, sl, sb, job, RfPlace{});
    call_end(e, st);
    if (rc || !host) return rc;
    HIPCHK(e, hipMemcpyAsync(rf, e->rf.p, (size_t)B * nkeep * sizeof(double), hipMemcpyDeviceToHost, st));
    HIPCHK(e, hipStreamSynchronize(st));
    return BH_OK;
}

int bh_targets_set(bh_engine *e, int nt, const bh_target_desc *td)
{
    if (!e) return BH_EINVAL;
    if (nt < 0 || nt > BH_MAX_TARGETS || (nt > 0 && !td)) return fail(e, BH_EINVAL, "nt must be 0..8");
    HIPCHK(e, hipSetDevice(e->device));
    HIPCHK(e, hipStreamSynchronize(e->stream));
    for (auto &t : e->targets) {
        release_target(t);
    }
    release_sites(e);
    e->targets.clear();
    e->nt = 0;
    e->ldy = 0;
    int off = 0;
    std::vector<TargetHost> tmp((size_t)nt);
    for (int i = 0; i < nt; ++i) {
        const bh_target_desc &d = td[i];
        TargetHost &t = tmp[(size_t)i];
        t.d = d;
        t.off = off;
        int rc = BH_OK;
        if (d.n < 1 || !d.yobs) rc = fail(e, BH_EINVAL, "target needs n >= 1 and yobs");
        if (!rc && d.law != BH_LAW_NOCORR && d.law != BH_LAW_NOCORR_SCALED && d.law != BH_LAW_EXP && d.law != BH_LAW_GAUSS)
            rc = fail(e, BH_EINVAL, "unknown covariance law");
        if (!rc && d.kind == BH_TARGET_SWD) {
            if (!d.x) rc = fail(e, BH_EINVAL, "SWD target needs periods x");
            if (!rc) rc = swd_supported(e, d.n > BH_MAX_PERIODS ? BH_MAX_PERIODS : d.n, d.iwave, t.d.igr, d.mode, d.flsph);
        } else if (!rc && d.kind == BH_TARGET_RF) {
            rc = rf_args_ok(e, d.nsamp, d.n, d.gauss, d.fsamp, d.waveno);
        } else if (!rc && d.kind == BH_TARGET_USER) {
        } else if (!rc) {
            rc = fail(e, BH_EINVAL, "unknown target kind");
        }
        if (!rc && d.law == BH_LAW_NOCORR_SCALED && !d.yerr) rc = fail(e, BH_EINVAL, "scaled-error law needs yerr");
        if (!rc && d.law == BH_LAW_GAUSS && !d.rinv) rc = fail(e, BH_EINVAL, "Gauss law needs rinv");
        const size_t nb = (size_t)d.n * sizeof(double);
        if (!rc) rc = ensure(e, t.yobs, nb);
        if (!rc && hipMemcpy(t.yobs.p, d.yobs, nb, hipMemcpyHostToDevice) != hipSuccess) rc = fail(e, BH_EHIP, "copy yobs");
        if (!rc && d.kind == BH_TARGET_SWD) {
            rc = ensure(e, t.x, nb);
            if (!rc && hipMemcpy(t.x.p, d.x, nb, hipMemcpyHostToDevice) != hipSuccess) rc = fail(e, BH_EHIP, "copy x");
            t.kfwd = d.n;
            if (!rc && d.n > BH_MAX_PERIODS) {
                double lo = d.x[0], hi = d.x[0];
                for (int k = 1; k < d.n; ++k) {
                    lo = d.x[k] < lo ? d.x[k] : lo;
                    hi = d.x[k] > hi ? d.x[k] : hi;
                }
                double g[BH_MAX_PERIODS];
                const double step = (hi - lo) / (double)(BH_MAX_PERIODS - 1);
                for (int k = 0; k < BH_MAX_PERIODS; ++k) g[k] = (double)k * step + lo;
                g[BH_MAX_PERIODS - 1] = hi;
                t.kfwd = BH_MAX_PERIODS;
                rc = ensure(e, t.x60, sizeof(g));
                if (!rc && hipMemcpy(t.x60.p, g, sizeof(g), hipMemcpyHostToDevice) != hipSuccess) rc = fail(e, BH_EHIP, "copy x60");
            }
        }
        if (!rc && d.law == BH_LAW_NOCORR_SCALED) {
            std::vector<double> se((size_t)d.n);
            t.logdet_extra = scaled_errors(d.yerr, d.n, se.data());
            rc = ensure(e, t.yerr_scaled, nb);
            if (!rc && hipMemcpy(t.yerr_scaled.p, se.data(), nb, hipMemcpyHostToDevice) != hipSuccess) rc = fail(e, BH_EHIP, "copy yerr");
        }
        if (!rc && d.law == BH_LAW_GAUSS) {
            t.logdet_extra = d.logdet_r;
            rc = ensure(e, t.rinv, nb * (size_t)d.n);
            if (!rc && hipMemcpy(t.rinv.p, d.rinv, nb * (size_t)d.n, hipMemcpyHostToDevice) != hipSuccess) rc = fail(e, BH_EHIP, "copy rinv");
        }
        if (rc) {
            for (auto &u : tmp) release_target(u);
            return rc;
        }
        t.d.x = t.d.yobs = t.d.yerr = t.d.rinv = nullptr;
        off += d.n;
    }
    e->targets.swap(tmp);
    e->nt = nt;
    e->ldy = off;
    e->err_t_nt = e->err_t_B = -1;
    return BH_OK;
}

}

namespace {

int stage_like_io(bh_engine *e, hipStream_t st, LikeKernelArgs &la)
{
    const int B = la.B, nt = la.nt;
    int rc;
    if ((rc = ensure(e, e->noise, (size_t)B * 2 * nt * sizeof(double)))) return rc;
    if ((rc = ensure(e, e->logL, (size_t)B * sizeof(double)))) return rc;
    if ((rc = ensure(e, e->misfits, (size_t)B * (nt + 1) * sizeof(double)))) return rc;
    if ((rc = ensure(e, e->errb, (size_t)B * sizeof(int32_t)))) return rc;
    HIPCHK(e, hipMemcpyAsync(e->noise.p, la.noise, (size_t)B * 2 * nt * sizeof(double), hipMemcpyHostToDevice, st));
    la.noise = (const double *)e->noise.p; la.logL = (double *)e->logL.p;
    la.misfits = (double *)e->misfits.p; la.err = (int32_t *)e->errb.p;
    return BH_OK;
}

int return_like_io(bh_engine *e, hipStream_t st, const LikeKernelArgs &la, double *logL, double *misfits, int32_t *err)
{
    HIPCHK(e, hipMemcpyAsync(logL, la.logL, (size_t)la.B * sizeof(double), hipMemcpyDeviceToHost, st));
    HIPCHK(e, hipMemcpyAsync(misfits, la.misfits, (size_t)la.B * (la.nt + 1) * sizeof(double), hipMemcpyDeviceToHost, st));
    HIPCHK(e, hipMemcpyAsync(err, la.err, (size_t)la.B * sizeof(int32_t), hipMemcpyDeviceToHost, st));
    return BH_OK;
}

struct EvalCall {
    hipStream_t st;
    int Lmax;
    Staged m;
    ptrdiff_t sl, sb;
    const int32_t *site;
    double *ymod;
    LikeKernelArgs la;
};

int eval_args_ok(bh_engine *e, const EvalPlan &p, bool host, const EvalCall &c)
{
    if (p.nt < 1) return fail(e, BH_EINVAL, "no targets registered (bh_targets_set)");
    if (p.no_forward) return fail(e, BH_EINVAL, "a BH_TARGET_USER target has no forward model: use bh_loglike_batch");
    if (p.rf_needs_table) return fail(e, BH_EINVAL, "bh_sites_set_missing with a receiver-function target needs bh_sites_set_rf");
    if (p.rf_axis_needs_table) return fail(e, BH_EINVAL, "bh_sites_set_axes with a receiver-function count that differs from its descriptor's needs the table of bh_sites_set_rf_axis");
    if (p.gauss_needs_table) return fail(e, BH_EINVAL, "bh_sites_set_missing_gauss with a Gauss-law target that a site lacks needs the table of bh_sites_set_gauss");
    if (p.law_gauss_needs_table) return fail(e, BH_EINVAL, "bh_sites_set_laws with a Gauss-law target that has a site under another law needs the table of bh_sites_set_gauss (that site in class -1)");
    if (p.rf_axis_gauss_needs_table) return fail(e, BH_EINVAL, "bh_sites_set_axes with a Gauss-law receiver function whose counts differ from its descriptor's needs the table of bh_sites_set_gauss (every site's matrix padded to the capacity)");
    if (p.rf_axis_no_mfma) return fail(e, BH_EUNSUPPORTED, "BH_NO_MFMA: the in-kernel mat-vec does not serve a Gauss-law receiver function with per-site counts (bh_sites_set_axes)");
    if (!c.m.nlay || !c.m.h || !c.m.vp || !c.m.vs || !c.la.noise || !c.la.logL || !c.la.misfits || !c.la.err) return fail(e, BH_EINVAL, "null argument");
    if (c.site && host)
        for (int b = 0; b < p.B; ++b)
            if (c.site[b] < 0 || c.site[b] >= e->nsites) return fail(e, BH_EINVAL, "site index out of range (bh_sites_set)");
    return BH_OK;
}

int stage_eval_inputs(bh_engine *e, bool host, int B, EvalCall &c)
{
    int rc;
    if (host) {
        if ((rc = stage_models(e, B, c.Lmax, c.sl, c.sb, c.m))) return rc;
        if ((rc = stage_like_io(e, c.st, c.la))) return rc;
        if (c.site) {
            if ((rc = ensure(e, e->site_idx, (size_t)B * sizeof(int32_t)))) return rc;
            HIPCHK(e, hipMemcpyAsync(e->site_idx.p, c.site, (size_t)B * sizeof(int32_t), hipMemcpyHostToDevice, c.st));
            c.site = (const int32_t *)e->site_idx.p;
        }
        c.ymod = nullptr;
    }
    if (!c.m.rho) {
        const size_t nel = span_elems(B, c.Lmax, c.sl, c.sb);
        if ((rc = ensure(e, e->rho, nel * sizeof(double)))) return rc;
        hipLaunchKernelGGL(rho_from_vp_kernel, dim3((unsigned)((nel + 255) / 256)), dim3(256), 0, c.st, nel, c.m.vp, (double *)e->rho.p);
        c.m.rho = (const double *)e->rho.p;
    }
    return BH_OK;
}

int size_eval_workspaces(bh_engine *e, const EvalPlan &p, EvalCall &c)
{
    int rc;
    if (!c.ymod) {
        if ((rc = ensure(e, e->ymod, (size_t)p.B * p.ldy * sizeof(double)))) return rc;
        c.ymod = (double *)e->ymod.p;
    }
    const size_t cap0 = e->err_t.cap;
    if ((rc = ensure(e, e->err_t, (size_t)p.nt * p.B * sizeof(int32_t)))) return rc;
    if (e->err_t.cap != cap0) e->err_t_nt = e->err_t_B = -1;
    c.la.ymod = c.ymod; c.la.err_t = (const int32_t *)e->err_t.p;
    for (int t = 0; t < p.nt; ++t) {
        TargetHost &T = e->targets[(size_t)t];
        if (p.role[t] == ROLE_SWD60 && (rc = ensure(e, T.vel60, (size_t)p.B * T.kfwd * sizeof(double)))) return rc;
        if (p.rf_fused[t] && (rc = ensure(e, T.sums, (size_t)p.B * 4 * sizeof(double)))) return rc;
    }
    return BH_OK;
}

int run_forward(bh_engine *e, const EvalPlan &p, const EvalCall &c)
{
    const int B = p.B, nt = p.nt, ldy = p.ldy;
    hipStream_t st = c.st, rst = p.fork ? e->aux : st;
    int rc;
    if (p.err_zero_always || e->err_t_nt != nt || e->err_t_B != B) {
        HIPCHK(e, hipMemsetAsync(e->err_t.p, 0, (size_t)nt * B * sizeof(int32_t), st));
        e->err_t_nt = nt;
        e->err_t_B = B;
    }
    SwdJob jobs[BH_MAX_TARGETS];
    int njobs = 0;
    const SwdSiteXArgs xtab{c.site, e->nsites, nt, ldy, (const int32_t *)e->site_xn.p, (const double *)e->site_xper.p, {}, {}};
    for (int t = 0; t < nt; ++t) {
        const TargetHost &T = e->targets[(size_t)t];
        const bh_target_desc &d = T.d;
        int32_t *errp = (int32_t *)e->err_t.p + (size_t)t * B;
        if (p.role[t] == ROLE_SWD) {
            jobs[njobs++] = SwdJob{d.n, d.iwave, d.igr, ldy, (const double *)T.x.p, c.ymod + T.off, errp, d.mode, d.flsph};
            if (p.x_table) jobs[njobs - 1].sx = SwdSiteJob{&xtab, t, T.off};
        } else if (p.role[t] == ROLE_SWD60) {
            jobs[njobs++] = SwdJob{T.kfwd, d.iwave, d.igr, T.kfwd, (const double *)T.x60.p, (double *)T.vel60.p, errp, d.mode, d.flsph};
        }
    }
    if (p.fork && (rc = wait_for(e, e->ev_fork, st, e->aux))) return rc;
    if (e->started != nullptr && e->started_expected > 0x70000000u) {
        HIPCHK(e, hipStreamSynchronize(st));
        HIPCHK(e, hipStreamSynchronize(e->aux));
        HIPCHK(e, hipMemset(e->started, 0, sizeof(unsigned)));
        e->started_expected = 0;
    }
    SwdLaunchInfo swd{};
    if ((rc = launch_swd_jobs(e, st, B, c.Lmax, c.m, c.sl, c.sb, njobs, jobs, p.prio_low, &swd))) return rc;
    const bool gate = p.want_gate && swd.workgroups > 0;
    if (gate)
        HIPCHK(e, hipStreamWaitValue32(e->aux, e->started, e->started_expected - swd.workgroups + gate_need(swd), hipStreamWaitValueGte, 0xffffffffu));
    const RfPlace where = rf_place(p.fork, gate && bh_tuning().rf_keep_floor == 0, bh_tuning(), e->rf_lds_beside_swd);
    for (int t = 0; t < nt; ++t) {
        TargetHost &T = e->targets[(size_t)t];
        const bh_target_desc &d = T.d;
        if (p.role[t] == ROLE_SWD60)
            bh_launch_interp(B, T.kfwd, (const double *)T.x60.p, (const double *)T.vel60.p, T.kfwd, d.n,
                             (const double *)T.x.p, c.ymod + T.off, ldy, st);
        if (p.role[t] != ROLE_RF) continue;
        RfSiteArgs rs{};
        if (p.rf_table) rs = RfSiteArgs{c.site, e->nsites, nt, (const double *)e->site_p.p + t, (const double *)e->site_nsv.p + t};
        RfSiteMArgs rm{};
        if (p.missing) {
            static_cast<RfSiteArgs &>(rm) = rs;
            rm.n = (const int32_t *)e->site_xn.p + t;
        }
        RfSiteTArgs ra{};
        if (p.rf_axis) {
            static_cast<RfSiteArgs &>(ra) = rs;
            ra.n = (const int32_t *)e->site_xn.p + t;
            ra.axis = (const RfAxisRec *)e->site_axis.p + t;
            ra.nsamp_max = T.axis_nsamp_max;
        }
        const RfJob job{d.p_s_per_deg, d.gauss, d.nsamp, d.fsamp, d.tshift, d.nsv, d.waveno, d.n, c.ymod + T.off, ldy,
                        p.rf_fused[t] ? (const double *)T.yobs.p : nullptr, p.rf_fused[t] ? (double *)T.sums.p : nullptr, p.rf_table ? &rs : nullptr,
                        p.missing ? &rm : nullptr, p.rf_axis ? &ra : nullptr};
        if ((rc = launch_rf(e, rst, B, c.Lmax, c.m, c.sl, c.sb, job, where))) return rc;
    }
    return p.fork ? wait_for(e, e->ev_join, e->aux, st) : BH_OK;
}

int run_like(bh_engine *e, hipStream_t st, LikeKernelArgs la, const bool *fused, EvalLike like, const int32_t *site, const EvalGauss *gauss)
{
    int rc;
    for (int t = 0; t < la.nt; ++t)
        if ((rc = prepare_like_target(e, st, la.B, la.ldy, la.ymod, e->targets[(size_t)t], la.t[t], fused[t], site, gauss[t]))) return rc;
    LikeSiteXArgs lx{};
    lx.site = site; lx.nsites = e->nsites; lx.yobs = (const double *)e->site_yobs.p; lx.yerr_scaled = (const double *)e->site_yerr.p;
    lx.logdet_extra = (const double *)e->site_logdet.p; lx.n = (const int32_t *)e->site_xn.p;
    if (like == LIKE_SITES_C || like == LIKE_SITES_L) {
        LikeClassArgs lc{};
        for (int t = 0; t < la.nt; ++t) {
            const TargetHost &T = e->targets[(size_t)t];
            if (gauss[t] != GAUSS_CLASSES || T.d.law != BH_LAW_GAUSS) continue;
            lc.class_of[t] = (const int32_t *)T.gc_class.p;
            lc.rinv[t] = (const double *)T.gc_rinv.p;
            lc.logdet[t] = (const double *)T.gc_logdet.p;
        }
        if (!e->site_x) lx.n = (const int32_t *)e->gc_xn.p;
        ev_begin(e, 2, st);
        if (like == LIKE_SITES_L) {
            lx.yerr_scaled = (const double *)e->law_yerr.p;
            lx.logdet_extra = (const double *)e->law_logdet.p;
            const LikeLawArgs lw{(const int32_t *)e->law_tab.p};
            bh_launch_like_sites_l(la, lx, lc, lw, st);
        } else {
            bh_launch_like_sites_c(la, lx, lc, st);
        }
        ev_end(e, 2, st);
        return BH_OK;
    }
    ev_begin(e, 2, st);
    if (like == LIKE_SITES_M) bh_launch_like_sites_m(la, lx, st);
    else if (like == LIKE_SITES_X) bh_launch_like_sites_x(la, lx, st);
    else if (like == LIKE_SITES) bh_launch_like_sites(la, lx, st);
    else bh_launch_like(la, st);
    ev_end(e, 2, st);
    return BH_OK;
}

int evaluate(bh_engine *e, int memspace, void *stream, int B, int Lmax, const int32_t *nlay, const double *h, const double *vp,
             const double *vs, const double *rho, ptrdiff_t sl, ptrdiff_t sb, const int32_t *site, const double *noise,
             double *logL, double *misfits, int32_t *err, double *ymod)
{
    int rc;
    if ((rc = check_models(e, B, Lmax, sl, sb))) return rc;
    const bool host = (memspace != BH_DEVICE);
    const EvalPlan p = plan_eval(e, B, site != nullptr, ymod != nullptr);
    LikeKernelArgs la{};
    la.B = B; la.nt = p.nt; la.ldy = p.ldy; la.noise = noise; la.logL = logL; la.misfits = misfits; la.err = err;
    EvalCall c{(!host && stream) ? (hipStream_t)stream : e->stream, Lmax, Staged{nlay, h, vp, vs, rho, nullptr, nullptr}, sl, sb, site, ymod, la};
    if ((rc = eval_args_ok(e, p, host, c))) return rc;
    if (B == 0) return BH_OK;
    HIPCHK(e, hipSetDevice(e->device));
    if ((rc = stage_eval_inputs(e, host, B, c)) || (rc = size_eval_workspaces(e, p, c))) return rc;
    call_begin(e, c.st);
    if ((rc = run_forward(e, p, c)) || (rc = run_like(e, c.st, c.la, p.rf_fused, p.like, c.site, p.gauss))) return rc;
    call_end(e, c.st);
    HIPCHK(e, hipGetLastError());
    if (!host) return BH_OK;
    if ((rc = return_like_io(e, c.st, c.la, logL, misfits, err))) return rc;
    if (ymod) HIPCHK(e, hipMemcpyAsync(ymod, c.ymod, (size_t)B * p.ldy * sizeof(double), hipMemcpyDeviceToHost, c.st));
    HIPCHK(e, hipStreamSynchronize(c.st));
    return BH_OK;
}

}

extern "C" {

int bh_evaluate_batch(bh_engine *e, int memspace, void *stream, int B, int Lmax,
                      const int32_t *nlay, const double *h, const double *vp, const double *vs,
                      const double *rho, ptrdiff_t sl, ptrdiff_t sb, const double *noise,
                      double *logL, double *misfits, int32_t *err, double *ymod)
{
    return evaluate(e, memspace, stream, B, Lmax, nlay, h, vp, vs, rho, sl, sb, nullptr, noise, logL, misfits, err, ymod);
}

static int sites_register(bh_engine *e, int nsites, const int32_t *n, const double *yobs, const double *yerr)
{
    const int nt = e->nt, ldy = e->ldy;
    HIPCHK(e, hipSetDevice(e->device));
    HIPCHK(e, hipStreamSynchronize(e->stream));
    release_sites(e);
    const size_t S = (size_t)nsites;
    std::vector<double> se(S * ldy, 1.0), ld(S * nt, 0.0), yo;
    if (n) yo.assign(S * ldy, 0.0);
    for (size_t s = 0; s < S; ++s)
        for (int t = 0; t < nt; ++t) {
            const TargetHost &T = e->targets[(size_t)t];
            const int ns = n ? n[s * nt + t] : T.d.n;
            ld[s * nt + t] = T.logdet_extra;
            if (T.d.law == BH_LAW_NOCORR_SCALED)
                ld[s * nt + t] = scaled_errors(yerr + s * ldy + T.off, ns, se.data() + s * ldy + T.off);
            if (n) std::copy(yobs + s * ldy + T.off, yobs + s * ldy + T.off + ns, yo.data() + s * ldy + T.off);
        }
    int rc;
    if ((rc = ensure(e, e->site_yobs, S * ldy * sizeof(double))) || (rc = ensure(e, e->site_yerr, S * ldy * sizeof(double))) ||
        (rc = ensure(e, e->site_logdet, S * nt * sizeof(double)))) {
        release_sites(e);
        return rc;
    }
    if (hipMemcpy(e->site_yobs.p, n ? yo.data() : yobs, S * ldy * sizeof(double), hipMemcpyHostToDevice) != hipSuccess ||
        hipMemcpy(e->site_yerr.p, se.data(), S * ldy * sizeof(double), hipMemcpyHostToDevice) != hipSuccess ||
        hipMemcpy(e->site_logdet.p, ld.data(), S * nt * sizeof(double), hipMemcpyHostToDevice) != hipSuccess) {
        release_sites(e);
        return fail(e, BH_EHIP, "copy site table");
    }
    e->nsites = nsites;
    return BH_OK;
}

int bh_sites_set(bh_engine *e, int nsites, const double *yobs, const double *yerr)
{
    if (!e) return BH_EINVAL;
    if (e->nt < 1) return fail(e, BH_EINVAL, "no targets registered (bh_targets_set)");
    if (nsites < 1 || !yobs) return fail(e, BH_EINVAL, "bh_sites_set needs nsites >= 1 and yobs");
    bool scaled = false;
    for (const auto &T : e->targets) scaled = scaled || T.d.law == BH_LAW_NOCORR_SCALED;
    if (scaled && !yerr) return fail(e, BH_EINVAL, "a BH_LAW_NOCORR_SCALED target needs yerr of every site");
    return sites_register(e, nsites, nullptr, yobs, yerr);
}

static int sites_register_x(bh_engine *e, const char *who, bool all, bool missing, bool missing_gauss, bool axes, int nsites, const int32_t *n, const double *x, const double *yobs, const double *yerr)
{
    if (!e) return BH_EINVAL;
    const std::string w(who);
    if (e->nt < 1) return fail(e, BH_EINVAL, "no targets registered (bh_targets_set)");
    if (nsites < 1 || !n || !x || !yobs) return fail(e, BH_EINVAL, (w + " needs nsites >= 1, n, x and yobs").c_str());
    const int nt = e->nt, ldy = e->ldy;
    bool scaled = false;
    for (const auto &T : e->targets) scaled = scaled || T.d.law == BH_LAW_NOCORR_SCALED;
    if (scaled && !yerr) return fail(e, BH_EINVAL, "a BH_LAW_NOCORR_SCALED target needs yerr of every site");
    const size_t S = (size_t)nsites;
    if (missing) {
        for (size_t s = 0; s < S; ++s) {
            bool any = false;
            for (int t = 0; t < nt; ++t) any = any || n[s * nt + t] != 0;
            if (!any) return fail(e, BH_EINVAL, (w + ": a site with no target (every count 0)").c_str());
        }
        for (int t = 0; t < nt; ++t) {
            bool any = false, lacks = false;
            for (size_t s = 0; s < S; ++s) {
                any = any || n[s * nt + t] != 0;
                lacks = lacks || n[s * nt + t] == 0;
            }
            if (!any) return fail(e, BH_EINVAL, (w + ": a target no site has (every count 0)").c_str());
            if (lacks && !missing_gauss && e->targets[(size_t)t].d.law == BH_LAW_GAUSS)
                return fail(e, BH_EUNSUPPORTED, (w + ": a Gauss-law target that a site lacks (the contraction gathers every site's rows)").c_str());
        }
    }
    for (int t = 0; t < nt; ++t) {
        const TargetHost &T = e->targets[(size_t)t];
        const bh_target_desc &d = T.d;
        if (d.kind != BH_TARGET_SWD) {
            for (size_t s = 0; s < S; ++s) {
                if (axes && d.kind == BH_TARGET_RF && n[s * nt + t] >= 0 && n[s * nt + t] <= d.n) continue;
                if (axes && d.kind == BH_TARGET_RF) return fail(e, BH_EINVAL, (w + ": a receiver function's sample count is below 0 or above its descriptor's n (the capacity)").c_str());
                if (n[s * nt + t] != d.n && !(missing && n[s * nt + t] == 0)) return fail(e, BH_EINVAL, (w + ": the sample count of a target that is no dispersion curve differs from its descriptor's").c_str());
            }
            continue;
        }
        if (d.law == BH_LAW_GAUSS) return fail(e, BH_EINVAL, (w + ": a dispersion target with the Gauss law (its R^-1 depends on the sample count)").c_str());
        if (T.kfwd != d.n) return fail(e, BH_EUNSUPPORTED, (w + ": a dispersion target of more than 60 periods (the interpolation path)").c_str());
        for (size_t s = 0; s < S; ++s) {
            const int ns = n[s * nt + t];
            if (missing && ns == 0) continue;
            if (ns < 1 || ns > d.n) return fail(e, BH_EINVAL, (w + ": a site's period count is below 1 or above the descriptor's n (the capacity)").c_str());
            for (int i = 0; i < ns; ++i) {
                const double v = x[s * ldy + T.off + i];
                if (!std::isfinite(v) || !(v > 0.0)) return fail(e, BH_EINVAL, (w + ": a period that is not finite and positive").c_str());
            }
        }
        if (!all && (d.igr != BH_VEL_PHASE || d.mode > 1)) {
            std::vector<double> x0((size_t)d.n);
            HIPCHK(e, hipSetDevice(e->device));
            HIPCHK(e, hipMemcpy(x0.data(), T.x.p, (size_t)d.n * sizeof(double), hipMemcpyDeviceToHost));
            for (size_t s = 0; s < S; ++s)
                if (n[s * nt + t] != d.n || std::memcmp(x0.data(), x + s * ldy + T.off, (size_t)d.n * sizeof(double)) != 0)
                    return fail(e, BH_EUNSUPPORTED, (w + ": per-site periods on a group-velocity or higher-mode target").c_str());
        }
    }
    int rc = sites_register(e, nsites, n, yobs, yerr);
    if (rc) return rc;
    std::vector<double> xs(S * ldy, 0.0);
    for (size_t s = 0; s < S; ++s)
        for (int t = 0; t < nt; ++t) {
            const TargetHost &T = e->targets[(size_t)t];
            if (T.d.kind == BH_TARGET_SWD) std::copy(x + s * ldy + T.off, x + s * ldy + T.off + n[s * nt + t], xs.data() + s * ldy + T.off);
        }
    if ((rc = ensure(e, e->site_xn, S * nt * sizeof(int32_t))) || (rc = ensure(e, e->site_xper, S * ldy * sizeof(double)))) {
        release_sites(e);
        return rc;
    }
    if (hipMemcpy(e->site_xn.p, n, S * nt * sizeof(int32_t), hipMemcpyHostToDevice) != hipSuccess ||
        hipMemcpy(e->site_xper.p, xs.data(), S * ldy * sizeof(double), hipMemcpyHostToDevice) != hipSuccess) {
        release_sites(e);
        return fail(e, BH_EHIP, "copy site table");
    }
    e->site_x = true;
    e->site_x_all = all;
    e->site_missing = missing;
    e->site_missing_gauss = missing_gauss;
    e->site_xn_host.assign(n, n + S * nt);
    for (int t = 0; t < nt; ++t)
        for (size_t s = 0; s < S; ++s)
            if (n[s * nt + t] == 0) e->targets[(size_t)t].site_lacks = true;
            else if (e->targets[(size_t)t].d.kind == BH_TARGET_RF && n[s * nt + t] != e->targets[(size_t)t].d.n) e->targets[(size_t)t].rf_own_counts = true;
    return BH_OK;
}

int bh_sites_set_x(bh_engine *e, int nsites, const int32_t *n, const double *x, const double *yobs, const double *yerr)
{
    return sites_register_x(e, "bh_sites_set_x", false, false, false, false, nsites, n, x, yobs, yerr);
}

int bh_sites_set_x_all(bh_engine *e, int nsites, const int32_t *n, const double *x, const double *yobs, const double *yerr)
{
    return sites_register_x(e, "bh_sites_set_x_all", true, false, false, false, nsites, n, x, yobs, yerr);
}

int bh_sites_set_missing(bh_engine *e, int nsites, const int32_t *n, const double *x, const double *yobs, const double *yerr)
{
    return sites_register_x(e, "bh_sites_set_missing", true, true, false, false, nsites, n, x, yobs, yerr);
}

int bh_sites_set_missing_gauss(bh_engine *e, int nsites, const int32_t *n, const double *x, const double *yobs, const double *yerr)
{
    return sites_register_x(e, "bh_sites_set_missing_gauss", true, true, true, false, nsites, n, x, yobs, yerr);
}

int bh_sites_set_axes(bh_engine *e, int nsites, const int32_t *n, const double *x, const double *yobs, const double *yerr)
{
    return sites_register_x(e, "bh_sites_set_axes", true, true, true, true, nsites, n, x, yobs, yerr);
}

int bh_sites_set_gauss(bh_engine *e, int target, int nsites, int nclass, const int32_t *class_of, const double *rinv, const double *logdet_r)
{
    if (!e) return BH_EINVAL;
    if (e->nsites < 1) return fail(e, BH_EINVAL, "no site table registered (bh_sites_set)");
    if (nsites != e->nsites) return fail(e, BH_EINVAL, "bh_sites_set_gauss: nsites differs from the site table's");
    if (target < 0 || target >= e->nt || e->targets[(size_t)target].d.law != BH_LAW_GAUSS)
        return fail(e, BH_EINVAL, "bh_sites_set_gauss: not a BH_LAW_GAUSS target");
    if (nclass < 1) return fail(e, BH_EINVAL, "bh_sites_set_gauss: nclass must be at least 1");
    if (!class_of || !rinv || !logdet_r) return fail(e, BH_EINVAL, "null argument");
    TargetHost &T = e->targets[(size_t)target];
    const size_t nn = (size_t)T.d.n * (size_t)T.d.n, S = (size_t)nsites, nt = (size_t)e->nt;
    if ((size_t)nclass > BH_SITES_GAUSS_MAXBYTES / sizeof(double) / nn)
        return fail(e, BH_EUNSUPPORTED, "bh_sites_set_gauss: the matrices take more than BH_SITES_GAUSS_MAXBYTES (1 GiB)");
    if (nclass > BH_SITES_GAUSS_MAXCLASSES) return fail(e, BH_EUNSUPPORTED, "bh_sites_set_gauss: more than BH_SITES_GAUSS_MAXCLASSES (4096) classes");
    for (size_t s = 0; s < S; ++s) {
        const int c = class_of[s];
        if (c < -1 || c >= nclass) return fail(e, BH_EINVAL, "bh_sites_set_gauss: a class index outside [-1, nclass)");
        const bool has = e->site_xn_host.empty() || e->site_xn_host[s * nt + (size_t)target] != 0;
        if (has && e->site_laws) {
            const bool gauss = e->site_law_host[s * nt + (size_t)target] == BH_LAW_GAUSS;
            if (gauss && c < 0) return fail(e, BH_EINVAL, "bh_sites_set_gauss: class -1 for a site under the Gauss law on the target (bh_sites_set_laws)");
            if (!gauss && c >= 0) return fail(e, BH_EINVAL, "bh_sites_set_gauss: a class for a site under another law than BH_LAW_GAUSS on the target (bh_sites_set_laws)");
            continue;
        }
        if (has && c < 0) return fail(e, BH_EINVAL, "bh_sites_set_gauss: class -1 for a site that has the target");
        if (!has && c >= 0) return fail(e, BH_EINVAL, "bh_sites_set_gauss: a class for a site that lacks the target (count 0)");
    }
    for (size_t i = 0; i < (size_t)nclass * nn; ++i)
        if (!std::isfinite(rinv[i])) return fail(e, BH_EINVAL, "bh_sites_set_gauss: a non-finite value in rinv");
    for (int c = 0; c < nclass; ++c)
        if (!std::isfinite(logdet_r[c])) return fail(e, BH_EINVAL, "bh_sites_set_gauss: a non-finite value in logdet_r");
    HIPCHK(e, hipSetDevice(e->device));
    HIPCHK(e, hipStreamSynchronize(e->stream));
    T.gc_nclass = 0;
    int rc;
// ... 209 lines not shown
```

bayhunter_amd/csrc/swd_kernel.hip:

```cpp
#include "../../include/bh_engine_debug.h"
#include "bh_device.h"
#include "bh_tuning.h"
#include <cmath>
#include <cstdlib>

#define BH_HD __device__ __forceinline__
#define BH_TAB static __device__ const
#include "bh_libm.h"

namespace {
#include "swd_common.h"

constexpr int LANE_TAB_PAD = (LIBM_TAB_BYTES + 15) & ~15;
#ifndef BH_NEV_LO
#define BH_NEV_LO 5
#endif
constexpr int NEV_LO = BH_NEV_LO;
__host__ __device__ inline size_t lane_wave_bytes(int Lmax, int K, int mode)
{
    const size_t b = (size_t)4 * Lmax * 64 * sizeof(float) + (size_t)2 * NEV_LO * 64 * sizeof(double) +
                     (size_t)((K + 1) & ~1) * sizeof(double) + (mode > 1 ? (size_t)2 * K * 64 * sizeof(double) : 0);
    return (b + 15) & ~(size_t)15;
}

#ifndef BH_SWD_SITEX
#define BH_SWD_SITEX 0
#endif
template <int IFUNC, bool LOOK, int LANE_WPB, int FAST, bool SIMPLE, bool FA = false>
#if BH_SWD_SITEX
__global__ __launch_bounds__(BH_WAVE * LANE_WPB) void swd_kernel(SwdKernelArgs A, SwdSiteXArgs X)
#else
__global__ __launch_bounds__(BH_WAVE * LANE_WPB) void swd_kernel(SwdKernelArgs A)
#endif
{
    extern __shared__ __align__(16) unsigned char smem_all[];
    const int lane = threadIdx.x & (BH_WAVE - 1);
    const int wave = threadIdx.x / BH_WAVE;
    const int wid = blockIdx.x * LANE_WPB + wave;
    const int J = LOOK ? A.look : 1;
    const int r = lane & (J - 1);
    const int lbase = lane - r;
    const int sidx = (wid * BH_WAVE + lane) / J;
#if BH_SWD_SITEX
    static_assert(!SIMPLE && FAST == 0 && !FA, "the site-period build is the launch of second roots");
    const bool inrange = sidx < A.B;
    const int iv = inrange ? (A.perm ? A.perm[sidx] : sidx) : 0;
    const bool second = true;
    const int ib = iv % A.Bm;
    const int Lmax = A.Lmax;
    const double *per = X.x;
    const int Kown = inrange ? bh_site_periods(X, 0, ib, A.K, per) : -1;
    const bool valid = inrange && iv / A.Bm < Kown;
    const int K = valid ? Kown : 0;
    constexpr int KROW = 0;
#else
    const bool valid = sidx < A.B;
    const int iv = valid ? (A.perm ? A.perm[sidx] : sidx) : 0;
    const bool second = !SIMPLE && FAST == 0 && A.second != 0;
    const int ib = second ? iv % A.Bm : iv;
    const int Lmax = A.Lmax;
    const int K = A.K;
#endif

    const LibmTabs LT = stage_libm_tables(smem_all, threadIdx.x, BH_WAVE * LANE_WPB);
#if BH_SWD_SITEX
    unsigned char *smem = smem_all + LANE_TAB_PAD + (size_t)wave * lane_wave_bytes(Lmax, KROW, 1);
#else
    unsigned char *smem = smem_all + LANE_TAB_PAD + (size_t)wave * lane_wave_bytes(Lmax, K, A.mode);
#endif
    float *mdl = reinterpret_cast<float *>(smem);
    double *xs = reinterpret_cast<double *>(smem + (size_t)4 * Lmax * BH_WAVE * sizeof(float));
    double *ys = xs + NEV_LO * BH_WAVE;
#if BH_SWD_SITEX
    double *cpl = ys + NEV_LO * BH_WAVE;
#else
    double *per = ys + NEV_LO * BH_WAVE;
    double *cpl = per + ((K + 1) & ~1);

    for (int k = lane; k < K; k += BH_WAVE) per[k] = A.periods[k];
#endif

    const int mmax = valid ? A.nlay[ib] : 2;
    int mtop = mmax;
    for (int off = 32; off > 0; off >>= 1) mtop = max(mtop, __shfl_xor(mtop, off));
    {
        const ptrdiff_t base = (ptrdiff_t)ib * A.sb;
        for (int l = 0; l < Lmax; ++l) {
            float fd = 0.f, fa = 1.f, fb = 1.f, fr = 1.f;
            if (valid && l < mmax) {
                const ptrdiff_t o = base + (ptrdiff_t)l * A.sl;
                fd = (float)A.h[o];
                fa = (float)A.vp[o];
                fb = (float)A.vs[o];
                fr = (float)A.rho[o];
            }
            mdl[(0 * Lmax + l) * BH_WAVE + lane] = fd;
            mdl[(1 * Lmax + l) * BH_WAVE + lane] = fa;
            mdl[(2 * Lmax + l) * BH_WAVE + lane] = fb;
            mdl[(3 * Lmax + l) * BH_WAVE + lane] = fr;
        }
    }
    __syncthreads();
    ModelLds md;
    md.d = mdl + 0 * Lmax * BH_WAVE + lane;
    md.a = mdl + 1 * Lmax * BH_WAVE + lane;
    md.b = mdl + 2 * Lmax * BH_WAVE + lane;
    md.rho = mdl + 3 * Lmax * BH_WAVE + lane;
    const int llw = (md.Bf(0) <= 0.0f) ? 2 : 1;

    SearchT<BH_WAVE, NEV_LO, FAST, SIMPLE> S;
#if BH_SWD_SITEX
    S.init(md, mmax, valid, BH_VEL_GROUP, K, per, xs + lane, ys + lane, A.vel + (size_t)ib * A.ldv, r == 0, 1,
           cpl + lane, cpl + lane, IFUNC, A.counted != 0, false, FA);
#else
    S.init(md, mmax, valid, A.igr, K, per, xs + lane, ys + lane, A.vel + (size_t)ib * A.ldv, r == 0, A.mode,
           cpl + lane, cpl + (size_t)K * BH_WAVE + lane, IFUNC, A.counted != 0, false, FA);
#endif
    {
        const size_t nl = (size_t)gridDim.x * LANE_WPB * BH_WAVE;
        double *hx = A.nev_high + (size_t)wid * BH_WAVE + lane;
        S.set_high(hx, hx + (size_t)(NEV_MAX - NEV_LO) * nl, nl);
    }
    if (second) S.template enter_second<IFUNC == 1>(iv / A.Bm, A.first[ib]);

    unsigned hw_id;
    asm volatile("s_getreg_b32 %0, hwreg(HW_REG_HW_ID)" : "=s"(hw_id));
    const unsigned nrounds = hw_id & 1u;
    const bool fair = A.fair != 0;
    while (__ballot(S.active) != 0ull) {
        if (fair) {
            const unsigned slice = (unsigned)(__builtin_readcyclecounter() >> A.fair);
            if (((slice ^ nrounds) & 1u) != 0u) __builtin_amdgcn_s_setprio(3);
            else __builtin_amdgcn_s_setprio(0);
        }
        if (!S.active) continue;
        const double omg = S.omega;
        const double cev = LOOK ? S.template candidate<IFUNC == 1>(r) : S.ceval;
        const double wvno = omg / cev;
        double del;
        int nv = -1;
        DivRange dr;
        dr.reset();
        if (FA) {
            if (IFUNC == 1) del = fa::love_secular(wvno, omg, md, mmax, llw, mtop, &nv);
            else del = fa::rayleigh_secular(wvno, omg, md, mmax, llw, mtop);
        } else if (IFUNC == 1)
            del = love_secular<false>(wvno, omg, md, mmax, llw, mtop, dr, LT, &nv);
        else
            del = rayleigh_secular<false>(wvno, omg, md, mmax, llw, mtop, dr, LT);
        if (!FA && !dr.ok()) {
            if (IFUNC == 1)
                del = love_secular<true>(wvno, omg, md, mmax, llw, mtop, dr, LT, &nv);
            else
                del = rayleigh_secular<true>(wvno, omg, md, mmax, llw, mtop, dr, LT);
        }
        if (!LOOK) {
            S.template advance<IFUNC == 1>(del, nv);
        } else {
            bool live = true;
            for (int j = 0; j < J; ++j) {
                const double cj = __shfl(cev, lbase + j);
                const double dj = __shfl(del, lbase + j);
                const int nj = (IFUNC == 1) ? __shfl(nv, lbase + j) : -1;
                if (j > 0) live = live && S.active && S.ceval == cj && S.omega == omg;
                if (__ballot(live) == 0ull) break;
                if (live) S.template advance<IFUNC == 1>(dj, nj);
            }
        }
    }
    if (valid && r == 0) {
        if (!second) A.err[ib] = S.errflag;
        if (!SIMPLE && FAST == 0 && A.igr == 2 && A.first != nullptr) A.first[ib] = S.del1st;
        if (FAST != 0 && S.has(S.F_GUARD) && A.gcount != nullptr) {
            A.glist[atomicAdd(A.gcount, 1)] = ib;
            atomicAdd(A.gcount + 2 * BH_MAX_TARGETS, 1);
        }
    }
    if (A.neval != nullptr) {
        unsigned long long tot = (r == 0) ? S.evals : 0u, lps = tot * (unsigned long long)(valid ? mmax - 1 : 0);
        for (int off = 32; off > 0; off >>= 1) {
            tot += __shfl_xor(tot, off);
            lps += __shfl_xor(lps, off);
        }
        if (lane == 0) {
            atomicAdd(A.neval, tot);
            atomicAdd(A.neval + (IFUNC == 2 ? 8 : 9), tot);
            atomicAdd(A.neval + (IFUNC == 2 ? 10 : 11), lps);
        }
    }
}

#if !BH_SWD_SITEX
__global__ __launch_bounds__(1024) void order_kernel(int B, const int32_t *nlay, int32_t *perm, int Lcut, int32_t *split)
{
    __shared__ int bin[BH_MAX_LAYERS + 2];
    const int tid = threadIdx.x;
    for (int i = tid; i < BH_MAX_LAYERS + 2; i += 1024) bin[i] = 0;
    __syncthreads();
    for (int b = tid; b < B; b += 1024) {
        int n = nlay[b];
        n = n < 0 ? 0 : (n > BH_MAX_LAYERS + 1 ? BH_MAX_LAYERS + 1 : n);
        atomicAdd(&bin[n], 1);
    }
    __syncthreads();
    if (tid == 0) {
        int acc = 0;
        for (int n = BH_MAX_LAYERS + 1; n >= 0; --n) {
            const int c = bin[n];
            bin[n] = acc;
            acc += c;
            if (n == Lcut + 1 && split != nullptr) split[0] = acc;
        }
        if (split != nullptr && Lcut + 1 > BH_MAX_LAYERS + 1) split[0] = 0;
    }
    __syncthreads();
    for (int b = tid; b < B; b += 1024) {
        int n = nlay[b];
        n = n < 0 ? 0 : (n > BH_MAX_LAYERS + 1 ? BH_MAX_LAYERS + 1 : n);
        perm[atomicAdd(&bin[n], 1)] = b;
    }
}

constexpr int PAIR_BUCKETS = 1024;
constexpr int PAIR_MAX_B = 12288;
__global__ __launch_bounds__(1024) void pair_order_kernel(int B, int Lmax, const int32_t *nlay, const double *vs, ptrdiff_t sl, ptrdiff_t sb,
                                                          int nt, PairOrderTarget t0, PairOrderTarget t1)
{
    __shared__ int bin[PAIR_BUCKETS];
    __shared__ int sorted[PAIR_MAX_B];
    __shared__ unsigned cmin_bits, cmax_bits;
    __shared__ int nmin, nmax;
    const int tid = threadIdx.x;
    for (int i = tid; i < PAIR_BUCKETS; i += 1024) bin[i] = 0;
    if (tid == 0) {
        cmin_bits = 0x7f800000u;
        cmax_bits = 0u;
        nmin = BH_MAX_LAYERS + 1;
        nmax = 0;
    }
    __syncthreads();
    constexpr int PER_THREAD = PAIR_MAX_B / 1024;
    float cost[PER_THREAD];
    int depth[PER_THREAD];
    {
        unsigned tcmin = 0x7f800000u, tcmax = 0u;
        int tnmin = BH_MAX_LAYERS + 1, tnmax = 0;
#pragma unroll
        for (int i = 0; i < PER_THREAD; ++i) {
            const int b = tid + 1024 * i;
            cost[i] = 0.0f;
            depth[i] = 1;
            if (b >= B) continue;
            int n = nlay[b];
            n = n < 1 ? 1 : (n > Lmax ? Lmax : n);
            float lo = 1e30f, hi = -1e30f;
            for (int l = 0; l < n; ++l) {
                const float v = (float)vs[(ptrdiff_t)b * sb + (ptrdiff_t)l * sl];
                lo = v < lo ? v : lo;
                hi = v > hi ? v : hi;
            }
            float c = hi - lo;
            c = (c >= 0.0f && c < 1e30f) ? c : 0.0f;
            cost[i] = c;
            depth[i] = n;
            const unsigned cb = __float_as_uint(c);
            tcmin = cb < tcmin ? cb : tcmin;
            tcmax = cb > tcmax ? cb : tcmax;
            tnmin = n < tnmin ? n : tnmin;
            tnmax = n > tnmax ? n : tnmax;
        }
        for (int off = 32; off > 0; off >>= 1) {
            tcmin = min(tcmin, (unsigned)__shfl_xor((int)tcmin, off));
            tcmax = max(tcmax, (unsigned)__shfl_xor((int)tcmax, off));
            tnmin = min(tnmin, __shfl_xor(tnmin, off));
            tnmax = max(tnmax, __shfl_xor(tnmax, off));
        }
        if ((tid & (BH_WAVE - 1)) == 0) {
            atomicMin(&cmin_bits, tcmin);
            atomicMax(&cmax_bits, tcmax);
            atomicMin(&nmin, tnmin);
            atomicMax(&nmax, tnmax);
        }
    }
    __syncthreads();
    const bool ragged = nmin != nmax;
    const bool blocked = !ragged && t0.xcd > 0;
    const int per = B / 8;
    const float cmin = __uint_as_float(cmin_bits), cmax = __uint_as_float(cmax_bits);
    const float scale = (cmax > cmin) ? (float)(PAIR_BUCKETS - 1) / (cmax - cmin) : 0.0f;
    auto bucket = [&](int i) {
        if (ragged) return (nmax - depth[i]) < PAIR_BUCKETS ? (nmax - depth[i]) : PAIR_BUCKETS - 1;
        int k = (int)((cmax - cost[i]) * scale);
        k = k < 0 ? 0 : (k > PAIR_BUCKETS - 1 ? PAIR_BUCKETS - 1 : k);
        if (blocked) k = ((tid + 1024 * i) / per) * (PAIR_BUCKETS / 8) + (k >> 3);
        return k;
    };
#pragma unroll
    for (int i = 0; i < PER_THREAD; ++i)
        if (tid + 1024 * i < B) atomicAdd(&bin[bucket(i)], 1);
    __syncthreads();
    {
        __shared__ int wsum[1024 / BH_WAVE];
        const int lane = tid & (BH_WAVE - 1), wv = tid / BH_WAVE;
        const int mine = bin[tid];
        int acc = mine;
        for (int off = 1; off < BH_WAVE; off <<= 1) {
            const int o = __shfl_up(acc, off);
            if (lane >= off) acc += o;
        }
        if (lane == BH_WAVE - 1) wsum[wv] = acc;
        __syncthreads();
        if (tid < 1024 / BH_WAVE) {
            int w = wsum[tid];
            for (int off = 1; off < 1024 / BH_WAVE; off <<= 1) {
                const int o = __shfl_up(w, off);
                if (tid >= off) w += o;
            }
            wsum[tid] = w;
        }
        __syncthreads();
        bin[tid] = (wv > 0 ? wsum[wv - 1] : 0) + acc - mine;
        __syncthreads();
    }
#pragma unroll
    for (int i = 0; i < PER_THREAD; ++i)
        if (tid + 1024 * i < B) sorted[atomicAdd(&bin[bucket(i)], 1)] = tid + 1024 * i;
    __syncthreads();
    for (int t = 0; t < nt; ++t) {
        const PairOrderTarget T = t == 0 ? t0 : t1;
        for (int pos = tid; pos < B; pos += 1024) {
            const int wid = pos / T.mpw, m = pos - wid * T.mpw;
            int src = pos;
            if (!ragged && T.slot_rank != nullptr && wid < T.nwaves - 1) src = T.slot_rank[wid] * T.mpw + m;
            if (blocked) {
                const int x = (T.xcd == 2) ? (wid >> 1) & 7 : (wid >> 2) & 7;
                const int q = (T.xcd == 2) ? (((wid >> 4) << 1) | (wid & 1)) : (((wid >> 5) << 2) | (wid & 3));
                src = x * per + q * T.mpw + m;
            }
            T.perm[pos] = sorted[src];
        }
    }
}

__device__ __forceinline__ double sphere_log(double x)
{
    double y;
    return bhp_log(x, &y, bhp_log_data) ? y : log(x);
}
__device__ __forceinline__ float sphere_powf(float x, float y)
{
    float r;
    return bhp_powf(x, y, &r, bhp_powf_log2_data, bhp_exp2f_data) ? r : powf(x, y);
}

__global__ void sphere_kernel(int B, int Lmax, const int32_t *nlay, const double *h, const double *vp,
                              const double *vs, const double *rho, ptrdiff_t sl, ptrdiff_t sb, double *oh,
                              double *ovp, double *ovs, double *orl, double *orr)
{
    const int b = blockIdx.x * blockDim.x + threadIdx.x;
    if (b >= B) return;
    const int mmax = nlay[b];
    const double ar = 6370.0;
    double dr = 0.0, r0 = ar;
    for (int i = 0; i < mmax; ++i) {
        const ptrdiff_t o = (ptrdiff_t)b * sb + (ptrdiff_t)i * sl;
        const float d = (i == mmax - 1) ? 1.0f : (float)h[o];
        const float a = (float)vp[o], bb = (float)vs[o], rt = (float)rho[o];
        dr = dr + (double)d;
        const double r1 = ar - dr;
        const double z0 = ar * sphere_log(ar / r0);
        const double z1 = ar * sphere_log(ar / r1);
        const float dn = (i == mmax - 1) ? 0.0f : (float)(z1 - z0);
        const double tmp = (ar + ar) / (r0 + r1);
        const float btp = (float)tmp;
        float p5 = btp * btp;
        p5 = p5 * p5;
        p5 = btp * p5;
        const size_t q = (size_t)i * B + b;
        oh[q] = (double)dn;
        ovp[q] = (double)(float)((double)a * tmp);
        ovs[q] = (double)(float)((double)bb * tmp);
        orl[q] = (double)(rt * (1.0f / p5));
        orr[q] = (double)(rt * sphere_powf(btp, -2.275f));
        r0 = r1;
    }
}

__global__ void interp_kernel(int B, int K0, const double *x0, const double *y0, int ld0, int K1,
                              const double *x1, double *y1, int ld1)
{
    const int t = blockIdx.x * blockDim.x + threadIdx.x;
    if (t >= B * K1) return;
    const int b = t / K1, k = t % K1;
    const double x = x1[k];
    const double *fp = y0 + (size_t)b * ld0;
    double r;
    if (x < x0[0]) r = fp[0];
    else if (x > x0[K0 - 1]) r = fp[K0 - 1];
    else {
        int j = 0;
        for (int lo = 0, hi = K0; lo < hi;) {
            const int mid = (lo + hi) >> 1;
            if (x0[mid] <= x) { j = mid; lo = mid + 1; } else hi = mid;
        }
        if (j == K0 - 1 || x0[j] == x) r = fp[j];
        else {
            const double slope = (fp[j + 1] - fp[j]) / (x0[j + 1] - x0[j]);
            r = slope * (x - x0[j]) + fp[j];
            if (r != r) {
                r = slope * (x - x0[j + 1]) + fp[j + 1];
                if (r != r && fp[j] == fp[j + 1]) r = fp[j];
            }
        }
    }
    y1[(size_t)b * ld1 + k] = r;
}
#endif

}

#if BH_SWD_SITEX
void bh_launch_swd_second_x(const SwdKernelArgs &a, int iwave, const SwdSiteXArgs &x, int ty, hipStream_t stream, SwdLaneBuild *build)
{
    SwdKernelArgs b = a;
    SwdSiteXArgs xt = x;
    xt.col[0] = x.col[ty];
    xt.off[0] = x.off[ty];
    int J = 1;
    while (2 * J <= a.look && 2 * J <= 16) J *= 2;
    b.look = J;
    b.second = 1; b.igr = BH_VEL_GROUP; b.mode = 1; b.fast = 0; b.farith = 0;
    const int no_fair = bh_tuning().swd_no_fair ? 1 : 0;
    const int slice = bh_tuning().swd_slice;
    b.fair = (no_fair || a.fair < 0) ? 0 : (slice > 0 ? slice : (a.fair > 0 ? a.fair : 16));
    const int mpw = BH_WAVE / J;
    const int waves = (a.B + mpw - 1) / mpw;
    const size_t wb = lane_wave_bytes(a.Lmax, 0, 1);
    const bool two = a.fair == 12 && LANE_TAB_PAD + 2 * wb <= 64 * 1024;
    const size_t lds = LANE_TAB_PAD + (two ? 2 : 1) * wb;
    const dim3 grid(two ? (waves + 1) / 2 : waves), block((two ? 2 : 1) * BH_WAVE);
    if (build != nullptr) *build = SwdLaneBuild{{iwave == 1 ? 1 : 2, J > 1, two ? 2 : 1, 0, false, false}, grid.x, b.fair};
#define BH_SECOND_LAUNCH(IF, LK, WP) hipLaunchKernelGGL((swd_kernel<IF, LK, WP, 0, false>), grid, block, lds, stream, b, xt)
#define BH_SECOND_PICK_WP(IF, LK) do { if (two) BH_SECOND_LAUNCH(IF, LK, 2); else BH_SECOND_LAUNCH(IF, LK, 1); } while (0)
#define BH_SECOND_PICK_LK(IF) do { if (J > 1) BH_SECOND_PICK_WP(IF, true); else BH_SECOND_PICK_WP(IF, false); } while (0)
    if (iwave == 1) BH_SECOND_PICK_LK(1);
    else BH_SECOND_PICK_LK(2);
#undef BH_SECOND_PICK_LK
#undef BH_SECOND_PICK_WP
#undef BH_SECOND_LAUNCH
}
#else

void bh_launch_order(int B, const int32_t *nlay, int32_t *perm, int Lcut, int32_t *split, hipStream_t stream)
{
    hipLaunchKernelGGL(order_kernel, dim3(1), dim3(1024), 0, stream, B, nlay, perm, Lcut, split);
}

void bh_launch_pair_order(int B, int Lmax, const int32_t *nlay, const double *vs, ptrdiff_t sl, ptrdiff_t sb, int nt,
                          const PairOrderTarget *tg, hipStream_t stream)
{
    hipLaunchKernelGGL(pair_order_kernel, dim3(1), dim3(1024), 0, stream, B, Lmax, nlay, vs, sl, sb, nt, tg[0], tg[nt > 1 ? 1 : 0]);
}
bool bh_pair_order_fits(int B) { return B <= PAIR_MAX_B; }

void bh_launch_sphere(int B, int Lmax, const int32_t *nlay, const double *h, const double *vp,
                      const double *vs, const double *rho, ptrdiff_t sl, ptrdiff_t sb, double *oh,
                      double *ovp, double *ovs, double *orho_love, double *orho_ray, hipStream_t stream)
{
    hipLaunchKernelGGL(sphere_kernel, dim3((B + 127) / 128), dim3(128), 0, stream, B, Lmax, nlay, h, vp, vs, rho,
                       sl, sb, oh, ovp, ovs, orho_love, orho_ray);
}

void bh_launch_interp(int B, int K0, const double *x0, const double *y0, int ld0, int K1,
                      const double *x1, double *y1, int ld1, hipStream_t stream)
{
    const int n = B * K1;
    hipLaunchKernelGGL(interp_kernel, dim3((n + 255) / 256), dim3(256), 0, stream, B, K0, x0, y0, ld0, K1, x1, y1, ld1);
}

size_t bh_swd_lds_bytes(int Lmax, int K, int mode) { return LANE_TAB_PAD + lane_wave_bytes(Lmax, K, mode); }

size_t bh_swd_nev_high_doubles(int B, int look)
{
    int J = 1;
    while (2 * J <= look && 2 * J <= 16) J *= 2;
    const int mpw = BH_WAVE / J;
    const size_t waves = (size_t)(((B + mpw - 1) / mpw + 1) / 2) * 2;
    return (size_t)2 * (NEV_MAX - NEV_LO) * waves * BH_WAVE;
}

void bh_launch_swd(const SwdKernelArgs &a, int iwave, hipStream_t stream, SwdLaneBuild *build)
{
    SwdKernelArgs b = a;
    int J = 1;
    while (2 * J <= a.look && 2 * J <= 16) J *= 2;
    b.look = J;
    const int no_fair = bh_tuning().swd_no_fair ? 1 : 0;
    const int slice = bh_tuning().swd_slice;
    b.fair = (no_fair || a.fair < 0) ? 0 : (slice > 0 ? slice : (a.fair > 0 ? a.fair : 16));
    const int mpw = BH_WAVE / J;
    const int waves = (a.B + mpw - 1) / mpw;
    const bool two = a.fair == 12 && LANE_TAB_PAD + 2 * lane_wave_bytes(a.Lmax, a.K, a.mode) <= 64 * 1024;
    const size_t wb = lane_wave_bytes(a.Lmax, a.K, a.mode);
    const size_t lds = LANE_TAB_PAD + (two ? 2 : 1) * wb;
    const dim3 grid(two ? (waves + 1) / 2 : waves), block((two ? 2 : 1) * BH_WAVE);
    const bool no_simple = bh_tuning().swd_no_simple != 0;
    const bool simple = a.igr == 0 && a.mode <= 1 && !no_simple && (J > 1 || a.fast);
    if (build != nullptr) {
        const int fs = (a.fast && a.igr == 0) ? 2 : 0;
        *build = SwdLaneBuild{{iwave == 1 ? 1 : 2, J > 1, two ? 2 : 1, fs, simple, fs == 2 && simple && a.farith != 0}, grid.x, b.fair};
    }
#define BH_LANE_LAUNCH(IF, LK, WP, FS, SI) hipLaunchKernelGGL((swd_kernel<IF, LK, WP, FS, SI>), grid, block, lds, stream, b)
#define BH_LANE_PICK_FS(IF, LK, WP)                                                  \
    do {                                                                             \
        if (a.fast && a.igr == 0) {                                                  \
            if (simple && a.farith) hipLaunchKernelGGL((swd_kernel<IF, LK, WP, 2, true, true>), grid, block, lds, stream, b); \
            else if (simple) BH_LANE_LAUNCH(IF, LK, WP, 2, true);                    \
            else BH_LANE_LAUNCH(IF, LK, WP, 2, false);                               \
        } else if (simple) BH_LANE_LAUNCH(IF, LK, WP, 0, true);                      \
        else BH_LANE_LAUNCH(IF, LK, WP, 0, false);                                   \
    } while (0)
#define BH_LANE_PICK_WP(IF, LK) do { if (two) BH_LANE_PICK_FS(IF, LK, 2); else BH_LANE_PICK_FS(IF, LK, 1); } while (0)
#define BH_LANE_PICK_LK(IF) do { if (J > 1) BH_LANE_PICK_WP(IF, true); else BH_LANE_PICK_WP(IF, false); } while (0)
    if (iwave == 1) BH_LANE_PICK_LK(1);
    else BH_LANE_PICK_LK(2);
#undef BH_LANE_PICK_LK
#undef BH_LANE_PICK_WP
#undef BH_LANE_PICK_FS
#undef BH_LANE_LAUNCH
}

namespace {
constexpr int PLAN_LEVELS = 5;
const int plan_trials[PLAN_LEVELS] = {1, 2, 3, 4, 7};
const double plan_dur[2][PLAN_LEVELS] = {{0.735, 0.54, 0.39, 0.33, 0.26}, {1.0, 0.64, 0.52, 0.45, 0.36}};
constexpr int PLAN_SLOTS = 2048;
constexpr double PLAN_LANE_PER_MODEL = 3.44;
constexpr int PLAN_LANE_LEVELS = 5;
const double plan_lane_dur[PLAN_LANE_LEVELS] = {1.0, 0.60, 0.40, 0.30, 0.26};

int plan_fit(int G, int level)
{
    int J = plan_trials[level];
    while (J > 1 && G * J > BH_WAVE) --J;
    return J;
}
}

int bh_swd_pick_group(int B, int ntargets, int Lmax)
{
    int G = Lmax - 1;
    if (G < 5) G = 5;
    if (G > 16) G = 16;
    (void)B; (void)ntargets;
    return G;
}

double bh_swd_plan(int B, int Lmax, int ntargets, const int *iwave, int Gforce, int *G, int *look)
{
    const int Gg = Gforce > 1 ? Gforce : bh_swd_pick_group(B, ntargets, Lmax);
    int lvl[8] = {0, 0, 0, 0, 0, 0, 0, 0}, best_lvl[8] = {0, 0, 0, 0, 0, 0, 0, 0};
    double best = 1e300;
    auto cost = [&](const int *l) {
        long waves = 0;
        double dmax = 0.0, dsum = 0.0;
        for (int t = 0; t < ntargets; ++t) {
            const int J = plan_fit(Gg, l[t]);
            const int mpw = BH_WAVE / (Gg * J);
            waves += (B + mpw - 1) / mpw;
            const double d = plan_dur[iwave[t] == 2 ? 1 : 0][l[t]];
            dmax = d > dmax ? d : dmax;
            dsum += d;
        }
        const long rounds = (waves + PLAN_SLOTS - 1) / PLAN_SLOTS;
        return (double)rounds * dmax * (waves > PLAN_SLOTS / 2 ? 1.15 : 1.0) + 1e-3 * dsum;
    };
    if (ntargets <= 4) {
        for (;;) {
            const double c = cost(lvl);
            if (c < best) {
                best = c;
                for (int t = 0; t < ntargets; ++t) best_lvl[t] = lvl[t];
            }
            int t = 0;
            while (t < ntargets && ++lvl[t] == PLAN_LEVELS) lvl[t++] = 0;
            if (t == ntargets) break;
        }
    } else {
        for (int l = 0; l < PLAN_LEVELS; ++l) {
            for (int t = 0; t < ntargets; ++t) lvl[t] = l;
            const double c = cost(lvl);
            if (c < best) {
                best = c;
                for (int t = 0; t < ntargets; ++t) best_lvl[t] = l;
            }
        }
    }
    double c1 = 1e300;
    int J1 = 1;
    bool any_rayleigh = false;
    for (int t = 0; t < ntargets; ++t) any_rayleigh = any_rayleigh || iwave[t] == 2;
    for (int l = 0; l < PLAN_LANE_LEVELS; ++l) {
        const int J = 1 << l;
        const int mpw = BH_WAVE / J;
        const long w = (long)ntargets * ((B + mpw - 1) / mpw);
        double c = PLAN_LANE_PER_MODEL * plan_lane_dur[l] * (any_rayleigh ? 1.0 : 0.85);
        if (w > PLAN_SLOTS) c *= 1.4 * std::pow((double)w / PLAN_SLOTS, 0.85);
        else if (w > PLAN_SLOTS / 2) c *= 1.25 + 0.15 * (double)(w - PLAN_SLOTS / 2) / (PLAN_SLOTS / 2);
        if (c < c1) {
            c1 = c;
            J1 = J;
        }
    }
    if (Gforce == 1 || (Gforce <= 0 && c1 < best)) {
        *G = 1;
        for (int t = 0; t < ntargets; ++t) look[t] = J1;
        return c1;
    }
    *G = Gg;
    for (int t = 0; t < ntargets; ++t) look[t] = plan_fit(Gg, best_lvl[t]);
    return best;
}
#endif
```

bayhunter_amd/engine.py:

```python
import contextlib
import ctypes as C
import os
import sys

import numpy as np

_HERE = os.path.dirname(os.path.abspath(__file__))
LIB_PATH = os.path.join(_HERE, "libbh_engine.so")

BH_OK, BH_EINVAL, BH_EHIP, BH_ENOMEM, BH_EUNSUPPORTED = 0, -1, -2, -3, -4
HOST, DEVICE = 0, 1
WAVE_LOVE, WAVE_RAYLEIGH = 1, 2
VEL_PHASE, VEL_GROUP = 0, 1
RF_P, RF_SV = 0, 1
LAW_NOCORR, LAW_NOCORR_SCALED, LAW_EXP, LAW_GAUSS = 0, 1, 2, 3
TARGET_SWD, TARGET_RF, TARGET_USER = 0, 1, 2
SEARCH_REFERENCE, SEARCH_FAST, SEARCH_FAST_RAYLEIGH = 0, 1, 2
ARITH_EXACT, ARITH_FAST = 0, 1
SCAN_STEPS, SCAN_COUNTED, SCAN_AUTO = 0, 1, 2
MAX_PERIODS, MAX_LAYERS, MAX_TARGETS = 60, 100, 8

_d = C.POINTER(C.c_double)
_i32 = C.POINTER(C.c_int32)


class EngineError(RuntimeError):
    pass


class SwdLaunch(C.Structure):
    _fields_ = [("family", C.c_int), ("role", C.c_int), ("key", C.c_int * 6), ("two_classes", C.c_int), ("interleaved", C.c_int),
                ("pair_order", C.c_int), ("restart", C.c_int), ("grid_x", C.c_int), ("fair", C.c_int)]


class TargetDesc(C.Structure):
    _fields_ = [("kind", C.c_int32), ("law", C.c_int32), ("n", C.c_int32),
                ("iwave", C.c_int32), ("igr", C.c_int32), ("mode", C.c_int32), ("flsph", C.c_int32),
                ("waveno", C.c_int32), ("nsamp", C.c_int32),
                ("p_s_per_deg", C.c_double), ("gauss", C.c_double), ("fsamp", C.c_double),
                ("tshift", C.c_double), ("nsv", C.c_double),
                ("x", _d), ("yobs", _d), ("yerr", _d), ("rinv", _d), ("logdet_r", C.c_double)]


BH_MAX_TARGETS = 8
BH_CHAIN_MAXLAYERS = 32
BH_CHAIN_MAXDEPTH = 7


class ChainConfig(C.Structure):
    _fields_ = [("nt", C.c_int32), ("maxlayers", C.c_int32), ("layermin", C.c_int32), ("layermax", C.c_int32),
                ("iter_burnin", C.c_int32), ("iterations", C.c_int32),
                ("vsmin", C.c_double), ("vsmax", C.c_double), ("zmin", C.c_double), ("zmax", C.c_double),
                ("thickmin", C.c_double), ("lvz", C.c_double), ("hvz", C.c_double),
                ("vpvsmin", C.c_double), ("vpvsmax", C.c_double), ("mantle_vs", C.c_double), ("mantle_vpvs", C.c_double),
                ("acc_lo", C.c_double), ("acc_hi", C.c_double),
                ("noise_lo", C.c_double * (2 * BH_MAX_TARGETS)), ("noise_hi", C.c_double * (2 * BH_MAX_TARGETS)),
                ("seed", C.c_uint64), ("chain_offset", C.c_int64)]


class ChainPrior(C.Structure):
    _fields_ = [("layermin", C.c_int32), ("layermax", C.c_int32),
                ("vsmin", C.c_double), ("vsmax", C.c_double), ("zmin", C.c_double), ("zmax", C.c_double),
                ("thickmin", C.c_double), ("lvz", C.c_double), ("hvz", C.c_double),
                ("vpvsmin", C.c_double), ("vpvsmax", C.c_double), ("mantle_vs", C.c_double), ("mantle_vpvs", C.c_double),
                ("acc_lo", C.c_double), ("acc_hi", C.c_double),
                ("noise_lo", C.c_double * (2 * BH_MAX_TARGETS)), ("noise_hi", C.c_double * (2 * BH_MAX_TARGETS))]


CHAIN_STATE_FIELDS = ("n", "vs", "z", "vpvs", "noise", "like", "misfits", "propdist", "proposed", "accepted", "naccepted",
                      "beta", "pn", "move", "valid", "pvs", "pz", "pvpvs", "pnoise", "dvs2", "lay_n", "lay_h", "lay_vp", "lay_vs",
                      "inject", "lay_rho")


class ChainState(C.Structure):
    _fields_ = [(k, C.c_void_p) for k in CHAIN_STATE_FIELDS]


class ChainRecord(C.Structure):
    _fields_ = [("models", C.c_void_p), ("likes", C.c_void_p), ("vpvs", C.c_void_p), ("misfits", C.c_void_p), ("noise", C.c_void_p),
                ("beta", C.c_void_p), ("rows", C.c_int64), ("thinning", C.c_int64), ("row0", C.c_int64)]


_lib = None


def load_library():
    global _lib
    if _lib is not None:
        return _lib
    if not os.path.exists(LIB_PATH):
        raise EngineError("native engine %s is not built; run `python -c 'import __graft_entry__ as g; "
                          "g.build()'` (or `make -C bayhunter_amd/csrc`)" % LIB_PATH)
    if "torch" not in sys.modules and os.environ.get("BH_NO_TORCH", "0") != "1":
        try:
            import torch
        except Exception:
            pass
    L = C.CDLL(LIB_PATH, mode=C.RTLD_GLOBAL)
    vp = C.c_void_p
    L.bh_abi_version.restype = C.c_int
    L.bh_engine_create.argtypes = [C.c_int, C.POINTER(vp)]
    L.bh_engine_destroy.argtypes = [vp]
    L.bh_engine_destroy.restype = None
    L.bh_engine_last_error.argtypes = [vp]
    L.bh_engine_last_error.restype = C.c_char_p
    L.bh_engine_stream.argtypes = [vp]
    L.bh_engine_stream.restype = vp
    L.bh_engine_synchronize.argtypes = [vp]
    L.bh_engine_set_instrumentation.argtypes = [vp, C.c_int, C.c_int]
    L.bh_engine_set_swd_group.argtypes = [vp, C.c_int]
    L.bh_engine_set_swd_lookahead.argtypes = [vp, C.c_int]
    L.bh_engine_set_swd_search.argtypes = [vp, C.c_int]
    L.bh_engine_get_swd_search.argtypes = [vp]
    L.bh_engine_set_swd_arith.argtypes = [vp, C.c_int]
    L.bh_engine_last_swd_kernel.argtypes = [vp]
    L.bh_engine_last_swd_launches.argtypes = [vp, C.POINTER(SwdLaunch), C.c_int, C.POINTER(C.c_int)]
    L.bh_engine_set_swd_trials.argtypes = [vp, C.c_int]
    L.bh_engine_get_swd_trials.argtypes = [vp]
    L.bh_engine_get_swd_arith.argtypes = [vp]
    L.bh_engine_set_swd_scan.argtypes = [vp, C.c_int]
    L.bh_engine_get_swd_scan.argtypes = [vp]
    L.bh_engine_set_tuning.argtypes = [vp, C.c_char_p, C.c_int]
    L.bh_engine_get_tuning.argtypes = [vp, C.c_char_p, C.POINTER(C.c_int)]
    L.bh_engine_guard_stats.argtypes = [vp, C.POINTER(C.c_int32), C.POINTER(C.c_uint64), C.POINTER(C.c_uint64)]
    L.bh_engine_set_typical_layers.argtypes = [vp, C.c_int]
    L.bh_engine_set_model_order.argtypes = [vp, C.c_int]
    L.bh_timing_reset.argtypes = [vp]
    L.bh_timing_collect.argtypes = [vp, C.POINTER(C.c_int), _d, _d]
    L.bh_timing_steps.argtypes = [vp, C.c_int, _d, C.POINTER(C.c_int)]
    L.bh_last_neval.argtypes = [vp, C.POINTER(C.c_uint64)]
    L.bh_debug_counters.argtypes = [vp, C.POINTER(C.c_uint64)]
    L.bh_debug_trace.argtypes = [vp, C.POINTER(C.c_uint64), C.c_int]
    L.bh_swd_batch.argtypes = [vp, C.c_int, vp, C.c_int, C.c_int, vp, vp, vp, vp, vp, C.c_ssize_t,
                               C.c_ssize_t, C.c_int, vp, C.c_int, C.c_int, C.c_int, C.c_int, vp, vp]
    L.bh_rf_batch.argtypes = [vp, C.c_int, vp, C.c_int, C.c_int, vp, vp, vp, vp, vp, vp, vp,
                              C.c_ssize_t, C.c_ssize_t, C.c_double, C.c_double, C.c_int, C.c_double,
                              C.c_double, C.c_double, C.c_int, C.c_int, vp]
    L.bh_targets_set.argtypes = [vp, C.c_int, C.POINTER(TargetDesc)]
    L.bh_evaluate_batch.argtypes = [vp, C.c_int, vp, C.c_int, C.c_int, vp, vp, vp, vp, vp,
                                    C.c_ssize_t, C.c_ssize_t, vp, vp, vp, vp, vp]
    L.bh_loglike_batch.argtypes = [vp, C.c_int, vp, C.c_int, vp, vp, vp, vp, vp, vp]
    L.bh_probe_math.argtypes = [vp, C.c_int, C.c_int, _d, _d]
    L.bh_sites_set.argtypes = [vp, C.c_int, vp, vp]
    L.bh_sites_set_rf.argtypes = [vp, C.c_int, vp, vp]
    L.bh_sites_set_x.argtypes = [vp, C.c_int, vp, vp, vp, vp]
    L.bh_sites_set_x_all.argtypes = [vp, C.c_int, vp, vp, vp, vp]
    L.bh_sites_set_missing.argtypes = [vp, C.c_int, vp, vp, vp, vp]
    L.bh_sites_set_missing_gauss.argtypes = [vp, C.c_int, vp, vp, vp, vp]
    L.bh_sites_set_gauss.argtypes = [vp, C.c_int, C.c_int, C.c_int, vp, vp, vp]
    L.bh_sites_set_axes.argtypes = [vp, C.c_int, vp, vp, vp, vp]
    L.bh_sites_set_rf_axis.argtypes = [vp, C.c_int, vp, vp, vp, vp]
    L.bh_sites_set_laws.argtypes = [vp, C.c_int, vp, vp]
    L.bh_chain_propose_sites.argtypes = [vp, C.POINTER(ChainConfig), C.POINTER(ChainState), C.c_int, C.c_int, vp]
    L.bh_chain_propose_window_sites.argtypes = [vp, C.POINTER(ChainConfig), C.POINTER(ChainState), C.c_int, C.c_int, C.c_int, C.c_ssize_t, vp]
    _cc, _cs, _cp = C.POINTER(ChainConfig), C.POINTER(ChainState), C.c_void_p
    L.bh_chain_propose_priors.argtypes = [vp, _cc, _cs, C.c_int, C.c_int, _cp, C.c_int, vp, vp]
    L.bh_chain_propose_window_priors.argtypes = [vp, _cc, _cs, C.c_int, C.c_int, C.c_int, C.c_ssize_t, _cp, C.c_int, vp, vp]
    L.bh_chain_accept_priors.argtypes = [vp, _cc, _cs, C.c_int, C.c_int, vp, vp, _cp, C.c_int, vp]
    L.bh_chain_accept_window_priors.argtypes = [vp, _cc, _cs, C.c_int, C.c_int, C.c_int, C.c_ssize_t, vp, vp, _cp, C.c_int, vp]
    _cr = C.POINTER(ChainRecord)
    L.bh_chain_accept_window_record.argtypes = [vp, _cc, _cs, C.c_int, C.c_int, C.c_int, C.c_ssize_t, vp, vp, _cr]
    L.bh_chain_accept_window_priors_record.argtypes = [vp, _cc, _cs, C.c_int, C.c_int, C.c_int, C.c_ssize_t, vp, vp, _cp, C.c_int, vp, _cr]
    L.bh_evaluate_sites.argtypes = [vp, C.c_int, vp, C.c_int, C.c_int, vp, vp, vp, vp, vp,
                                    C.c_ssize_t, C.c_ssize_t, vp, vp, vp, vp, vp, vp]
    L.bh_chain_propose.argtypes = [vp, C.POINTER(ChainConfig), C.POINTER(ChainState), C.c_int, C.c_int]
    L.bh_chain_accept.argtypes = [vp, C.POINTER(ChainConfig), C.POINTER(ChainState), C.c_int, C.c_int, vp, vp]
    L.bh_chain_propose_window.argtypes = [vp, C.POINTER(ChainConfig), C.POINTER(ChainState), C.c_int, C.c_int, C.c_int, C.c_ssize_t]
    L.bh_chain_accept_window.argtypes = [vp, C.POINTER(ChainConfig), C.POINTER(ChainState), C.c_int, C.c_int, C.c_int, C.c_ssize_t, vp, vp]
    L.bh_posterior_create.argtypes = [vp, C.POINTER(vp)]
    L.bh_posterior_destroy.argtypes = [vp]
    L.bh_posterior_destroy.restype = None
    L.bh_posterior_load.argtypes = [vp, C.c_int, vp, C.c_int, C.c_int64, C.c_int, C.c_int64, vp, vp, C.c_int, vp, vp, vp]
    L.bh_posterior_columns.argtypes = [vp, C.c_int, vp, vp, vp, vp, vp, vp, vp, vp, vp]
    L.bh_posterior_hist.argtypes = [vp, C.c_int, vp, vp, C.c_int, vp, vp, vp, vp]
    L.bh_posterior_interfaces.argtypes = [vp, C.c_int, vp, vp]
    for name in ("bh_posterior_create", "bh_posterior_load", "bh_posterior_columns", "bh_posterior_hist", "bh_posterior_interfaces"):
        getattr(L, name).restype = C.c_int
    L.bh_posterior_keep_rows.argtypes = [vp, C.c_int]
    L.bh_posterior_moho.argtypes = [vp, vp, vp, vp, vp]
    L.bh_posterior_attach.argtypes = [vp, C.c_int, vp, C.c_int, C.c_int, C.c_int64, vp, C.c_int]
    L.bh_posterior_scalar_cols.argtypes = [vp, C.c_int, vp]
    L.bh_posterior_scalar_stats.argtypes = [vp, C.c_int, vp, vp, vp, vp, vp, vp, vp, vp, vp]
    L.bh_posterior_scalar_hist.argtypes = [vp, C.c_int, C.c_int, vp, vp, vp]
    L.bh_posterior_scalar_hist2d.argtypes = [vp, C.c_int, C.c_int, C.c_int, vp, vp, vp, vp, vp, vp]
    for name in POSTERIOR_SCALARS_SYMBOLS:
        getattr(L, name).restype = C.c_int
    for name in ("bh_engine_create", "bh_engine_synchronize", "bh_engine_set_instrumentation", "bh_engine_set_swd_group", "bh_engine_set_swd_lookahead", "bh_engine_set_swd_search", "bh_engine_get_swd_search", "bh_engine_set_swd_arith", "bh_engine_get_swd_arith", "bh_engine_last_swd_kernel", "bh_engine_set_swd_trials", "bh_engine_get_swd_trials", "bh_engine_set_swd_scan", "bh_engine_get_swd_scan", "bh_engine_set_tuning", "bh_engine_get_tuning", "bh_engine_guard_stats", "bh_engine_set_typical_layers", "bh_engine_set_model_order",
                 "bh_timing_reset", "bh_timing_collect", "bh_timing_steps", "bh_last_neval", "bh_debug_counters", "bh_debug_trace", "bh_swd_batch", "bh_rf_batch", "bh_targets_set",
                 "bh_evaluate_batch", "bh_loglike_batch", "bh_probe_math", "bh_chain_propose", "bh_chain_accept",
                 "bh_chain_propose_window", "bh_chain_accept_window", "bh_sites_set", "bh_evaluate_sites", "bh_sites_set_rf", "bh_sites_set_x", "bh_sites_set_x_all",
                 "bh_sites_set_missing", "bh_chain_propose_sites", "bh_chain_propose_window_sites") + SITE_GAUSS_SYMBOLS + SITE_PRIORS_SYMBOLS + SITE_RF_AXIS_SYMBOLS + SITE_LAWS_SYMBOLS + CHAIN_RECORD_SYMBOLS:
        getattr(L, name).restype = C.c_int
    if L.bh_abi_version() != 10:
        raise EngineError("ABI version mismatch")
    _lib = L
    return L


EXPORTED_SYMBOLS = ("bh_abi_version", "bh_engine_create", "bh_engine_destroy", "bh_engine_last_error",
                    "bh_engine_stream", "bh_engine_synchronize", "bh_engine_set_swd_search", "bh_engine_get_swd_search",
                    "bh_engine_set_swd_arith", "bh_engine_get_swd_arith", "bh_engine_set_swd_trials", "bh_engine_get_swd_trials",
                    "bh_engine_guard_stats", "bh_engine_set_typical_layers", "bh_engine_set_model_order",
                    "bh_swd_batch", "bh_rf_batch", "bh_targets_set", "bh_evaluate_batch", "bh_loglike_batch",
                    "bh_chain_propose", "bh_chain_accept", "bh_chain_propose_window", "bh_chain_accept_window")
DEBUG_SYMBOLS = ("bh_engine_set_swd_group", "bh_engine_set_swd_lookahead", "bh_engine_last_swd_kernel", "bh_engine_last_swd_launches",
                 "bh_engine_set_swd_scan",
                 "bh_engine_get_swd_scan", "bh_engine_set_tuning",
                 "bh_engine_get_tuning", "bh_probe_math", "bh_engine_set_instrumentation", "bh_timing_reset",
                 "bh_timing_collect", "bh_timing_steps", "bh_last_neval", "bh_debug_counters", "bh_debug_trace")
SITE_SYMBOLS = ("bh_sites_set", "bh_evaluate_sites")
SITE_RF_SYMBOLS = ("bh_sites_set_rf",)
SITE_X_SYMBOLS = ("bh_sites_set_x",)
SITE_X_ALL_SYMBOLS = ("bh_sites_set_x_all",)
SITE_MISSING_SYMBOLS = ("bh_sites_set_missing", "bh_chain_propose_sites", "bh_chain_propose_window_sites")
SITE_GAUSS_SYMBOLS = ("bh_sites_set_gauss", "bh_sites_set_missing_gauss")
SITE_RF_AXIS_SYMBOLS = ("bh_sites_set_axes", "bh_sites_set_rf_axis")
SITE_LAWS_SYMBOLS = ("bh_sites_set_laws",)
SITE_PRIORS_SYMBOLS = ("bh_chain_propose_priors", "bh_chain_propose_window_priors", "bh_chain_accept_priors",
                       "bh_chain_accept_window_priors")
CHAIN_RECORD_SYMBOLS = ("bh_chain_accept_window_record", "bh_chain_accept_window_priors_record")
POSTERIOR_SYMBOLS = ("bh_posterior_create", "bh_posterior_destroy", "bh_posterior_load", "bh_posterior_columns",
                     "bh_posterior_hist", "bh_posterior_interfaces")
POSTERIOR_SCALARS_SYMBOLS = ("bh_posterior_keep_rows", "bh_posterior_moho", "bh_posterior_attach", "bh_posterior_scalar_cols", "bh_posterior_scalar_stats",
                             "bh_posterior_scalar_hist", "bh_posterior_scalar_hist2d")
SCALARS_MOHO, SCALARS_USER = 0, 1


def _f64(a):
    return np.ascontiguousarray(a, dtype=np.float64)


def _ptr(a):
    return C.c_void_p(a.ctypes.data) if a is not None else None


def pack_models(models, Lmax=None):
    B = len(models)
    nlay = np.array([len(m[0]) for m in models], dtype=np.int32)
    if Lmax is None:
        Lmax = int(nlay.max()) if B else 1
    out = [np.zeros((Lmax, B)) for _ in range(4)]
    for b, m in enumerate(models):
        for a, v in zip(out, m):
            a[:nlay[b], b] = v
    return nlay, out[0], out[1], out[2], out[3]


class Engine(object):

    def __init__(self, device=0):
        self._L = load_library()
        h = C.c_void_p()
        rc = self._L.bh_engine_create(int(device), C.byref(h))
        if rc != BH_OK:
            raise EngineError("bh_engine_create(device=%d) failed with %d: no usable HIP device "
                              "(this package has no CPU fallback)" % (device, rc))
        self._h = h
        self.device = int(device)
        self._owner = None
        self.ntargets = 0
        self.ldy = 0
        self.nsites = 0

    def close(self):
        if getattr(self, "_h", None):
            self._L.bh_engine_destroy(self._h)
            self._h = None

    def __del__(self):
        try:
            self.close()
        except Exception:
            pass

    def _check(self, rc):
        if rc != BH_OK:
            msg = self._L.bh_engine_last_error(self._h)
            raise EngineError("engine call failed (%d): %s" % (rc, msg.decode() if msg else "?"))

    @property
    def stream(self):
        return self._L.bh_engine_stream(self._h)

    def synchronize(self):
        self._check(self._L.bh_engine_synchronize(self._h))

    def set_instrumentation(self, timing=False, counting=False):
        self._check(self._L.bh_engine_set_instrumentation(self._h, int(timing), int(counting)))

    def set_swd_group(self, lanes_per_model):
        self._check(self._L.bh_engine_set_swd_group(self._h, int(lanes_per_model)))

    def set_typical_layers(self, nlay):
        self._check(self._L.bh_engine_set_typical_layers(self._h, int(nlay)))

    def set_model_order(self, sort_by_depth=True):
        self._check(self._L.bh_engine_set_model_order(self._h, int(bool(sort_by_depth))))

    def set_swd_lookahead(self, trials_per_round):
        self._check(self._L.bh_engine_set_swd_lookahead(self._h, int(trials_per_round)))

    def set_swd_search(self, search):
        codes = {"reference": SEARCH_REFERENCE, "fast": SEARCH_FAST, "fast_rayleigh": SEARCH_FAST_RAYLEIGH}
        codes.update({v: v for v in list(codes.values())})
        code = codes.get(search)
        if code is None:
            raise ValueError("search must be 'reference', 'fast' or 'fast_rayleigh'")
        self._check(self._L.bh_engine_set_swd_search(self._h, code))

    def swd_search(self):
        return {SEARCH_FAST: "fast", SEARCH_FAST_RAYLEIGH: "fast_rayleigh"}.get(self._L.bh_engine_get_swd_search(self._h), "reference")

    @contextlib.contextmanager
    def searching(self, search):
        prev = self.swd_search()
        self.set_swd_search(search)
        try:
            yield self
        finally:
            self.set_swd_search(prev)

    def set_swd_arith(self, arith):
        codes = {"exact": ARITH_EXACT, "fast": ARITH_FAST, ARITH_EXACT: ARITH_EXACT, ARITH_FAST: ARITH_FAST}
        code = codes.get(arith)
        if code is None:
            raise ValueError("arith must be 'exact' or 'fast'")
        self._check(self._L.bh_engine_set_swd_arith(self._h, code))

    def set_swd_trials(self, trials):
        self._check(self._L.bh_engine_set_swd_trials(self._h, int(trials)))

    def swd_trials(self):
        return int(self._L.bh_engine_get_swd_trials(self._h))

    @contextlib.contextmanager
    def trying(self, trials):
        prev = self.swd_trials()
        if trials is not None:
            self.set_swd_trials(trials)
        try:
            yield self
        finally:
            if trials is not None:
                self.set_swd_trials(prev)

    def last_swd_kernel(self):
        return {0: "group", 1: "lane", 2: "lean"}.get(self._L.bh_engine_last_swd_kernel(self._h))

    def last_swd_launches(self):
        out = (SwdLaunch * 32)()
        n = C.c_int(0)
        self._check(self._L.bh_engine_last_swd_launches(self._h, out, 32, C.byref(n)))
        return [dict(family={0: "group", 1: "lane", 2: "lean"}[r.family], role={0: "main", 1: "rerun", 2: "second"}[r.role],
                     key=tuple(r.key), two_classes=bool(r.two_classes), interleaved=bool(r.interleaved),
                     pair_order=bool(r.pair_order), restart=bool(r.restart), grid_x=int(r.grid_x), fair=int(r.fair))
                for r in out[:n.value]]

    def swd_arith(self):
        return "fast" if self._L.bh_engine_get_swd_arith(self._h) == ARITH_FAST else "exact"

    @contextlib.contextmanager
    def computing(self, arith):
        prev = self.swd_arith()
        self.set_swd_arith(arith)
        try:
            yield self
        finally:
            self.set_swd_arith(prev)

    def set_swd_scan(self, scan):
        codes = {"steps": SCAN_STEPS, "counted": SCAN_COUNTED, "auto": SCAN_AUTO}
        codes.update({v: v for v in list(codes.values())})
        code = codes.get(scan)
        if code is None:
            raise ValueError("scan must be 'steps', 'counted' or 'auto'")
        self._check(self._L.bh_engine_set_swd_scan(self._h, code))

    def swd_scan(self):
        return {SCAN_STEPS: "steps", SCAN_COUNTED: "counted"}.get(self._L.bh_engine_get_swd_scan(self._h), "auto")

    def guard_stats(self):
        counts = (C.c_int32 * 8)()
        n = C.c_uint64(0)
        self._check(self._L.bh_engine_guard_stats(self._h, counts, C.byref(n), None))
        return list(counts), int(n.value)

    def guard_total(self):
        return sum(self.guard_totals())

    def guard_totals(self):
        tot = (C.c_uint64 * 8)()
        self._check(self._L.bh_engine_guard_stats(self._h, None, None, tot))
        return [int(x) for x in tot]

    def timing_reset(self):
        self._check(self._L.bh_timing_reset(self._h))

    def timing_collect(self):
        n = C.c_int(0)
        tot = C.c_double(0)
        fam = (C.c_double * 3)()
        self._check(self._L.bh_timing_collect(self._h, C.byref(n), C.byref(tot), fam))
        return n.value, tot.value, {"swd": fam[0], "rf": fam[1], "like": fam[2]}

    def timing_steps(self, maxn=4096):
        out = np.zeros(int(maxn))
        n = C.c_int(0)
        self._check(self._L.bh_timing_steps(self._h, int(maxn), out.ctypes.data_as(_d), C.byref(n)))
        return out[:n.value].copy()

    def last_timing(self):
        n, tot, fam = self.timing_collect()
        self.timing_reset()
        return tot, fam

    def debug_counters(self):
        out = (C.c_uint64 * 16)()
        self._check(self._L.bh_debug_counters(self._h, out))
        return [int(v) for v in out]

    def debug_trace(self):
        n = min(self.debug_counters()[7], 16384)
        out = (C.c_uint64 * (4 * max(n, 1)))()
        self._check(self._L.bh_debug_trace(self._h, out, n))
        return np.frombuffer(out, dtype=np.uint64).reshape(-1, 4)[:n].copy()

    def last_neval(self):
        v = C.c_uint64(0)
        self._check(self._L.bh_last_neval(self._h, C.byref(v)))
        return int(v.value)

    @staticmethod
    def _model_args(nlay, h, vp, vs, rho, layout):
        h = _f64(h)
        if layout == "layer_major":
            Lmax, B = h.shape
            sl, sb = max(B, 1), 1
        elif layout == "model_major":
            B, Lmax = h.shape
            sl, sb = 1, Lmax
        else:
            raise ValueError("layout must be 'layer_major' or 'model_major'")
        arrs = [h] + [None if a is None else _f64(a) for a in (vp, vs, rho)]
        for a in arrs:
            if a is not None and a.shape != h.shape:
                raise ValueError("model arrays must have identical shapes")
        nlay = np.ascontiguousarray(nlay, dtype=np.int32)
        if nlay.shape != (B,):
            raise ValueError("nlay must have shape (B,)")
        if B and (nlay.min() < 1 or nlay.max() > Lmax):
            raise ValueError("nlay entries must be in 1..Lmax")
        return B, Lmax, sl, sb, nlay, arrs

    def swd_batch(self, nlay, h, vp, vs, rho, periods, iwave, igr, mode=1, flsph=0,
                  layout="layer_major"):
        B, Lmax, sl, sb, nlay, (h, vp, vs, rho) = self._model_args(nlay, h, vp, vs, rho, layout)
        periods = _f64(periods)
        K = periods.size
        vel = np.zeros((B, K))
        err = np.zeros(B, dtype=np.int32)
        self._check(self._L.bh_swd_batch(self._h, HOST, None, B, Lmax, _ptr(nlay), _ptr(h), _ptr(vp),
                                         _ptr(vs), _ptr(rho), sl, sb, K, _ptr(periods), int(iwave),
                                         int(igr), int(mode), int(flsph), _ptr(vel), _ptr(err)))
        return vel, err

    def rf_batch(self, nlay, h, vp, vs, rho, p, gauss, nsamp, fsamp, tshift, waveno, nkeep,
                 nsv=0.0, qp=None, qs=None, layout="layer_major"):
        B, Lmax, sl, sb, nlay, (h, vp, vs, rho) = self._model_args(nlay, h, vp, vs, rho, layout)
        qp = None if qp is None else _f64(qp)
        qs = None if qs is None else _f64(qs)
        rf = np.zeros((B, int(nkeep)))
        self._check(self._L.bh_rf_batch(self._h, HOST, None, B, Lmax, _ptr(nlay), _ptr(h), _ptr(vp),
                                        _ptr(vs), _ptr(rho), _ptr(qp), _ptr(qs), sl, sb, float(p),
                                        float(gauss), int(nsamp), float(fsamp), float(tshift),
                                        float(nsv), int(waveno), int(nkeep), _ptr(rf)))
        return rf

    def set_targets(self, descs):
        arr = (TargetDesc * max(1, len(descs)))()
        keep = []
        ldy = 0
        for i, d in enumerate(descs):
            t = arr[i]
            t.kind, t.law, t.n = int(d["kind"]), int(d["law"]), int(d["n"])
            t.iwave, t.igr = int(d.get("iwave", 2)), int(d.get("igr", 0))
            t.mode, t.flsph = int(d.get("mode", 1)), int(d.get("flsph", 0))
            t.waveno, t.nsamp = int(d.get("waveno", 0)), int(d.get("nsamp", 0))
            t.p_s_per_deg, t.gauss = float(d.get("p", 6.4)), float(d.get("gauss", 1.0))
            t.fsamp, t.tshift, t.nsv = float(d.get("fsamp", 1.0)), float(d.get("tshift", 0.0)), float(d.get("nsv", 0.0))
            for key in ("x", "yobs", "yerr", "rinv"):
                v = d.get(key)
                if v is not None:
                    v = _f64(v)
                    keep.append(v)
                    setattr(t, key, v.ctypes.data_as(_d))
            t.logdet_r = float(d.get("logdet_r", 0.0))
            ldy += t.n
        self._check(self._L.bh_targets_set(self._h, len(descs), arr))
        self.ntargets = len(descs)
        self.ldy = ldy
        self.nsites = 0

    def evaluate_batch(self, nlay, h, vp, vs, noise, rho=None, layout="layer_major", want_ymod=False):
        B, Lmax, sl, sb, nlay, (h, vp, vs, rho) = self._model_args(nlay, h, vp, vs, rho, layout)
        nt = self.ntargets
        noise = _f64(noise)
        if noise.shape != (B, 2 * nt):
            raise ValueError("noise must have shape (B, 2*ntargets)")
        logL = np.zeros(B)
        misf = np.zeros((B, nt + 1))
        err = np.zeros(B, dtype=np.int32)
        ymod = np.zeros((B, self.ldy)) if want_ymod else None
        self._check(self._L.bh_evaluate_batch(self._h, HOST, None, B, Lmax, _ptr(nlay), _ptr(h),
                                              _ptr(vp), _ptr(vs), _ptr(rho), sl, sb, _ptr(noise),
                                              _ptr(logL), _ptr(misf), _ptr(err), _ptr(ymod)))
        return (logL, misf, err, ymod) if want_ymod else (logL, misf, err)

    def set_sites(self, yobs, yerr=None):
        yobs = _f64(yobs)
        if yobs.ndim != 2 or yobs.shape[1] != self.ldy or yobs.shape[0] < 1:
            raise ValueError("yobs must have shape (nsites, %d)" % self.ldy)
        if yerr is not None:
            yerr = _f64(yerr)
            if yerr.shape != yobs.shape:
                raise ValueError("yerr must have the shape of yobs")
        self._check(self._L.bh_sites_set(self._h, yobs.shape[0], _ptr(yobs), _ptr(yerr)))
        self.nsites = yobs.shape[0]

    def set_sites_x(self, n, x, yobs, yerr=None):
        self._set_sites_x(self._L.bh_sites_set_x, n, x, yobs, yerr)

    def set_sites_x_all(self, n, x, yobs, yerr=None):
        self._set_sites_x(self._L.bh_sites_set_x_all, n, x, yobs, yerr)

    def set_sites_missing(self, n, x, yobs, yerr=None):
        self._set_sites_x(self._L.bh_sites_set_missing, n, x, yobs, yerr)

    def set_sites_missing_gauss(self, n, x, yobs, yerr=None):
        self._set_sites_x(self._L.bh_sites_set_missing_gauss, n, x, yobs, yerr)

    def set_sites_axes(self, n, x, yobs, yerr=None):
        self._set_sites_x(self._L.bh_sites_set_axes, n, x, yobs, yerr)

    def set_sites_rf_axis(self, nsamp, fsamp, tshift, gauss):
        nsamp = np.ascontiguousarray(nsamp, dtype=np.int32)
        fsamp, tshift, gauss = _f64(fsamp), _f64(tshift), _f64(gauss)
        if nsamp.ndim != 2 or nsamp.shape[1] != self.ntargets or any(a.shape != nsamp.shape for a in (fsamp, tshift, gauss)):
            raise ValueError("nsamp, fsamp, tshift and gauss must have shape (nsites, %d)" % self.ntargets)
        self._check(self._L.bh_sites_set_rf_axis(self._h, nsamp.shape[0], _ptr(nsamp), _ptr(fsamp), _ptr(tshift), _ptr(gauss)))

    def set_sites_laws(self, law, yerr=None):
        law = np.ascontiguousarray(law, dtype=np.int32)
        if law.ndim != 2 or law.shape[1] != self.ntargets:
            raise ValueError("law must have shape (nsites, %d)" % self.ntargets)
        if yerr is not None:
            yerr = _f64(yerr)
            if yerr.shape != (law.shape[0], self.ldy):
                raise ValueError("yerr must have shape (nsites, %d)" % self.ldy)
        self._check(self._L.bh_sites_set_laws(self._h, law.shape[0], _ptr(law), _ptr(yerr)))

    def set_sites_gauss(self, target, class_of, rinv, logdet_r):
        class_of = np.ascontiguousarray(class_of, dtype=np.int32)
        rinv, logdet_r = _f64(rinv), _f64(logdet_r)
        if class_of.ndim != 1:
            raise ValueError("class_of must have shape (nsites,)")
        if rinv.ndim != 3 or rinv.shape[1] != rinv.shape[2] or logdet_r.shape != rinv.shape[:1]:
            raise ValueError("rinv must have shape (nclass, n, n) and logdet_r (nclass,)")
        self._check(self._L.bh_sites_set_gauss(self._h, int(target), class_of.shape[0], rinv.shape[0], _ptr(class_of), _ptr(rinv),
                                               _ptr(logdet_r)))

    def _set_sites_x(self, entry, n, x, yobs, yerr):
        n = np.ascontiguousarray(n, dtype=np.int32)
        x, yobs = _f64(x), _f64(yobs)
        if yobs.ndim != 2 or yobs.shape[1] != self.ldy or yobs.shape[0] < 1:
            raise ValueError("yobs must have shape (nsites, %d)" % self.ldy)
        if x.shape != yobs.shape:
            raise ValueError("x must have the shape of yobs")
        if n.shape != (yobs.shape[0], self.ntargets):
            raise ValueError("n must have shape (nsites, %d)" % self.ntargets)
        if yerr is not None:
            yerr = _f64(yerr)
            if yerr.shape != yobs.shape:
                raise ValueError("yerr must have the shape of yobs")
        self._check(entry(self._h, yobs.shape[0], _ptr(n), _ptr(x), _ptr(yobs), _ptr(yerr)))
        self.nsites = yobs.shape[0]

    def set_sites_rf(self, p, nsv):
        p, nsv = _f64(p), _f64(nsv)
        if p.ndim != 2 or p.shape[1] != self.ntargets or nsv.shape != p.shape:
            raise ValueError("p and nsv must have shape (nsites, %d)" % self.ntargets)
        self._check(self._L.bh_sites_set_rf(self._h, p.shape[0], _ptr(p), _ptr(nsv)))

    def evaluate_sites(self, nlay, h, vp, vs, noise, site, rho=None, layout="layer_major", want_ymod=False):
        B, Lmax, sl, sb, nlay, (h, vp, vs, rho) = self._model_args(nlay, h, vp, vs, rho, layout)
        nt = self.ntargets
        noise = _f64(noise)
        if noise.shape != (B, 2 * nt):
            raise ValueError("noise must have shape (B, 2*ntargets)")
        site = np.ascontiguousarray(site, dtype=np.int32)
        if site.shape != (B,):
            raise ValueError("site must have shape (B,)")
        logL = np.zeros(B)
        misf = np.zeros((B, nt + 1))
        err = np.zeros(B, dtype=np.int32)
        ymod = np.zeros((B, self.ldy)) if want_ymod else None
        self._check(self._L.bh_evaluate_sites(self._h, HOST, None, B, Lmax, _ptr(nlay), _ptr(h), _ptr(vp), _ptr(vs), _ptr(rho),
                                              sl, sb, _ptr(site), _ptr(noise), _ptr(logL), _ptr(misf), _ptr(err), _ptr(ymod)))
        return (logL, misf, err, ymod) if want_ymod else (logL, misf, err)

    def loglike_batch(self, ymod, noise, fail=None):
        ymod = _f64(ymod)
        B = ymod.shape[0]
        nt = self.ntargets
        if ymod.shape != (B, self.ldy):
            raise ValueError("ymod must have shape (B, %d)" % self.ldy)
        noise = _f64(noise)
        if noise.shape != (B, 2 * nt):
            raise ValueError("noise must have shape (B, 2*ntargets)")
        if fail is not None:
            fail = np.ascontiguousarray(fail, dtype=np.int32)
            if fail.shape != (nt, B):
                raise ValueError("fail must have shape (ntargets, B)")
        logL = np.zeros(B)
        misf = np.zeros((B, nt + 1))
        err = np.zeros(B, dtype=np.int32)
        self._check(self._L.bh_loglike_batch(self._h, HOST, None, B, _ptr(ymod), _ptr(fail), _ptr(noise),
                                             _ptr(logL), _ptr(misf), _ptr(err)))
        return logL, misf, err

    def set_tuning(self, name, value):
        self._check(self._L.bh_engine_set_tuning(self._h, name.encode(), int(value)))

    def tuning(self, name):
        v = C.c_int(0)
        self._check(self._L.bh_engine_get_tuning(self._h, name.encode(), C.byref(v)))
        return int(v.value)

    def probe_math(self, op, x):
        x = _f64(x).ravel()
        out = np.zeros(x.size // 2 if op in (6, 7) else x.size)
        self._check(self._L.bh_probe_math(self._h, int(op), out.size, x.ctypes.data_as(_d), out.ctypes.data_as(_d)))
        return out

    def swd_batch_dev(self, B, Lmax, nlay, h, vp, vs, rho, sl, sb, K, periods, iwave, igr, vel, err,
                      stream=None, mode=1, flsph=0):
        self._check(self._L.bh_swd_batch(self._h, DEVICE, stream, B, Lmax, nlay, h, vp, vs, rho, sl, sb,
                                         K, periods, iwave, igr, mode, flsph, vel, err))

    def rf_batch_dev(self, B, Lmax, nlay, h, vp, vs, rho, sl, sb, p, gauss, nsamp, fsamp, tshift,
                     waveno, nkeep, rf, stream=None, nsv=0.0, qp=None, qs=None):
        self._check(self._L.bh_rf_batch(self._h, DEVICE, stream, B, Lmax, nlay, h, vp, vs, rho, qp, qs,
                                        sl, sb, p, gauss, nsamp, fsamp, tshift, nsv, waveno, nkeep, rf))

    def evaluate_batch_dev(self, B, Lmax, nlay, h, vp, vs, rho, sl, sb, noise, logL, misfits, err,
                           ymod=None, stream=None):
        self._check(self._L.bh_evaluate_batch(self._h, DEVICE, stream, B, Lmax, nlay, h, vp, vs, rho,
                                              sl, sb, noise, logL, misfits, err, ymod))

    def evaluate_sites_dev(self, B, Lmax, nlay, h, vp, vs, rho, sl, sb, site, noise, logL, misfits, err,
# ... 65 lines not shown
```

include/bh_engine_debug.h:

```cpp
#ifndef BH_ENGINE_DEBUG_H
#define BH_ENGINE_DEBUG_H

#include "bh_engine.h"

#ifdef __cplusplus
extern "C" {
#endif

int bh_engine_set_swd_group(bh_engine *e, int lanes_per_model);
int bh_engine_set_swd_lookahead(bh_engine *e, int trials_per_round);

#define BH_KERNEL_GROUP 0
#define BH_KERNEL_LANE 1
#define BH_KERNEL_LEAN 2
int bh_engine_last_swd_kernel(const bh_engine *e);

typedef struct {
    int family, role, key[6];
    int two_classes, interleaved, pair_order, restart, grid_x, fair;
} bh_swd_launch;
#define BH_SWD_MAIN 0
#define BH_SWD_RERUN 1
#define BH_SWD_SECOND 2
int bh_engine_last_swd_launches(const bh_engine *e, bh_swd_launch *out, int max, int *n);

#define BH_SCAN_STEPS 0
#define BH_SCAN_COUNTED 1
#define BH_SCAN_AUTO 2
int bh_engine_set_swd_scan(bh_engine *e, int scan);
int bh_engine_get_swd_scan(const bh_engine *e);

int bh_engine_set_tuning(bh_engine *e, const char *name, int value);
int bh_engine_get_tuning(bh_engine *e, const char *name, int *value);

int bh_probe_math(bh_engine *e, int op, int n, const double *in, double *out);

int bh_engine_set_instrumentation(bh_engine *e, int timing, int counting);
int bh_timing_reset(bh_engine *e);
int bh_timing_collect(bh_engine *e, int *ncalls, double *total_ms, double family_ms[3]);
int bh_timing_steps(bh_engine *e, int max, double *step_ms, int *n);
int bh_last_neval(bh_engine *e, uint64_t *neval);
int bh_debug_counters(bh_engine *e, uint64_t out[16]);
int bh_debug_trace(bh_engine *e, uint64_t *out, int nwaves);


#ifdef __cplusplus
}
#endif
#endif
```

Measured before the change: 6.093 million.

## Fold memsets into pair-order kernel and split length ordering across eight blocks

Guard, error-flag and counter zeroing memsets are folded into the model-ordering kernel's prologue whenever length or pair ordering runs, which removes separate small launches from the stream. The blocked (XCD-interleaved) length ordering moves from one 1024-thread workgroup to eight workgroups, each sorting its own slice by cost or depth into LDS buckets. Pair ordering now always launches the order kernel, with nt=0 when only fills are needed. This trades a few extra device launches and more ordering code paths for shorter serial prologue work, but the ordering inside each slice may differ slightly from the old global bucket scheme.

```diff
diff --git a/bayhunter_amd/csrc/bh_device.h b/bayhunter_amd/csrc/bh_device.h
--- a/bayhunter_amd/csrc/bh_device.h
+++ b/bayhunter_amd/csrc/bh_device.h
@@ -148,9 +148,15 @@
     int32_t *perm;
     int xcd;
 };
+struct SwdFills {
+    int32_t *guard = nullptr;
+    int32_t *err = nullptr;
+    unsigned long long *counter = nullptr;
+    int nguard = 0, nerr = 0, ncounter = 0;
+};
 bool bh_pair_order_fits(int B);
-void bh_launch_pair_order(int B, int Lmax, const int32_t *nlay, const double *vs, ptrdiff_t sl, ptrdiff_t sb, int nt,
-                          const PairOrderTarget *tg, hipStream_t stream);
+int bh_launch_pair_order(int B, int Lmax, const int32_t *nlay, const double *vs, ptrdiff_t sl, ptrdiff_t sb, int nt,
+                         const PairOrderTarget *tg, const SwdFills &fills, hipStream_t stream);
 struct SwdLaunchInfo {
     unsigned workgroups;
     long waves;
diff --git a/bayhunter_amd/csrc/bh_engine.hip b/bayhunter_amd/csrc/bh_engine.hip
--- a/bayhunter_amd/csrc/bh_engine.hip
+++ b/bayhunter_amd/csrc/bh_engine.hip
@@ -125,6 +125,7 @@
     int last_swd_kernel = -1;
     bh_swd_launch swd_launches[3 * BH_MAX_TARGETS]{};
     int n_swd_launches = 0;
+    int last_swd_order[3] = {0, 0, 0};
     int err_t_nt = -1, err_t_B = -1;
     std::string err;
     DevBuf nlay, h, vp, vs, rho, qp, qs, periods, vel, errb, rf, coef, ymod, noise, logL,
@@ -383,14 +384,19 @@
     SwdSiteJob sx{};
 };
 
-int swd_counter(bh_engine *e, hipStream_t st, unsigned long long **out)
+int swd_counter(bh_engine *e, hipStream_t st, SwdFills *prologue, unsigned long long **out)
 {
     *out = nullptr;
     if (!e->counting) return BH_OK;
     int rc = ensure(e, e->counter, BH_DEBUG_WORDS * sizeof(unsigned long long));
     if (rc) return rc;
     if (!e->neval_pending) {
-        HIPCHK(e, hipMemsetAsync(e->counter.p, 0, BH_COUNTER_WORDS * sizeof(unsigned long long), st));
+        if (prologue) {
+            prologue->counter = (unsigned long long *)e->counter.p;
+            prologue->ncounter = BH_COUNTER_WORDS;
+        } else {
+            HIPCHK(e, hipMemsetAsync(e->counter.p, 0, BH_COUNTER_WORDS * sizeof(unsigned long long), st));
+        }
         e->neval_pending = true;
     }
     *out = (unsigned long long *)e->counter.p;
@@ -398,7 +404,7 @@
 }
 
 constexpr int GUARD_HEAD = 24;
-int guard_space(bh_engine *e, hipStream_t st, int B, int32_t **counts, int32_t **lists)
+int guard_space(bh_engine *e, hipStream_t st, int B, SwdFills *prologue, int32_t **counts, int32_t **lists)
 {
     const size_t need = ((size_t)GUARD_HEAD + (size_t)BH_MAX_TARGETS * (size_t)(B + 4)) * sizeof(int32_t);
     if (need > e->guard.cap) {
@@ -414,7 +420,13 @@
     if (rc) return rc;
     *counts = (int32_t *)e->guard.p;
     *lists = (int32_t *)e->guard.p + GUARD_HEAD;
-    HIPCHK(e, hipMemsetAsync(e->guard.p, 0, (e->guard_fresh ? GUARD_HEAD : 2 * BH_MAX_TARGETS) * sizeof(int32_t), st));
+    const int words = e->guard_fresh ? GUARD_HEAD : 2 * BH_MAX_TARGETS;
+    if (prologue) {
+        prologue->guard = (int32_t *)e->guard.p;
+        prologue->nguard = words;
+    } else {
+        HIPCHK(e, hipMemsetAsync(e->guard.p, 0, (size_t)words * sizeof(int32_t), st));
+    }
     e->guard_fresh = false;
     return BH_OK;
 }
@@ -424,7 +436,7 @@
     return J.igr == BH_VEL_PHASE && J.mode <= 1 && (search == BH_SEARCH_FAST || (search == BH_SEARCH_FAST_RAYLEIGH && J.iwave == BH_WAVE_RAYLEIGH));
 }
 
-enum SwdOrder { ORDER_NONE, ORDER_DEPTH, ORDER_LENGTH, ORDER_PAIR };
+enum SwdOrder { ORDER_NONE = BH_ORDER_NONE, ORDER_DEPTH = BH_ORDER_DEPTH, ORDER_LENGTH = BH_ORDER_LENGTH, ORDER_PAIR = BH_ORDER_PAIR };
 
 struct SwdPlan {
     bool first_roots[BH_MAX_TARGETS];
@@ -435,6 +447,7 @@
     int kernel;
     int G, lean_trials;
     int order, Lcut;
+    bool prologue;
     int len_mpw, len_xcd;
     bool sitex;
     bool any_fast, farith, adapt_ok;
@@ -517,6 +530,7 @@
             if (shallow_bulk) p.Lcut = p.typ_layers + 2;
         }
     }
+    p.prologue = p.order == ORDER_LENGTH || p.order == ORDER_PAIR;
     p.any_fast = nfast > 0;
     p.farith = e->swd_arith == BH_ARITH_FAST;
     p.adapt_ok = e->force_group == 0 && e->force_look == 0 && tun.swd_look_r == 0 && tun.swd_look_l == 0;
@@ -664,6 +678,8 @@
     const int32_t *pair_perm[2] = {};
     unsigned long long *counter = nullptr;
     int32_t *gcounts = nullptr, *glists = nullptr;
+    SwdFills fills{};
+    int order_wgs = 0;
     SwdSiteXArgs sx{};
     int prio_low = 0;
     SwdLaunchInfo info{};
@@ -844,8 +860,8 @@
     const SwdGroupPlan &g = c.g;
     const int nt = c.p.ntargets, B = c.B;
     const int *n = g.pair_waves;
-    bool ok = true, geom = true;
-    if (pw.key_n0 != n[0] || pw.key_n1 != n[1]) {
+    bool ok = g.pair, geom = true;
+    if (ok && (pw.key_n0 != n[0] || pw.key_n1 != n[1])) {
         std::vector<int32_t> rank[2];
         geom = build_slot_ranks(n[0], n[1], pw.ncu, rank);
         for (int t = 0; ok && geom && t < nt; ++t) {
@@ -872,13 +888,11 @@
         }
         pw.cap_perm = ok ? B + B / 4 + 64 : 0;
     }
-    if (ok) {
-        PairOrderTarget tg[2];
-        for (int t = 0; t < nt; ++t) tg[t] = PairOrderTarget{g.pair_mpw[t], n[t], geom ? pw.slot_rank[t] : nullptr, pw.perm[t]};
-        const SwdTarget t0 = swd_target(c, c.p.job[0]);
-        bh_launch_pair_order(B, c.Lmax, c.m.nlay, t0.vs, t0.sl, t0.sb, nt, tg, c.st);
-        for (int t = 0; t < nt; ++t) c.pair_perm[t] = pw.perm[t];
-    }
+    PairOrderTarget tg[2] = {};
+    for (int t = 0; ok && t < nt; ++t) tg[t] = PairOrderTarget{g.pair_mpw[t], n[t], geom ? pw.slot_rank[t] : nullptr, pw.perm[t]};
+    const SwdTarget t0 = swd_target(c, c.p.job[0]);
+    c.order_wgs = bh_launch_pair_order(B, c.Lmax, c.m.nlay, t0.vs, t0.sl, t0.sb, ok ? nt : 0, tg, c.fills, c.st);
+    for (int t = 0; ok && t < nt; ++t) c.pair_perm[t] = pw.perm[t];
     (void)hipGetLastError();
     return BH_OK;
 }
@@ -887,16 +901,17 @@
 {
     const SwdPlan &p = c.p;
     if (p.order == ORDER_NONE) return BH_OK;
-    if (p.order == ORDER_PAIR) return c.g.pair ? pair_models(c) : BH_OK;
+    if (p.order == ORDER_PAIR) return pair_models(c);
     bh_engine *e = c.e;
     int rc;
     if ((rc = ensure(e, e->perm, ((size_t)c.B + 4) * sizeof(int32_t)))) return rc;
     int32_t *perm = (int32_t *)e->perm.p;
     if (p.order == ORDER_LENGTH) {
         const PairOrderTarget tg{p.len_mpw, c.B / p.len_mpw, nullptr, perm + 4, p.len_xcd};
-        bh_launch_pair_order(c.B, c.Lmax, c.m.nlay, c.m.vs, c.sl, c.sb, 1, &tg, c.st);
+        c.order_wgs = bh_launch_pair_order(c.B, c.Lmax, c.m.nlay, c.m.vs, c.sl, c.sb, 1, &tg, c.fills, c.st);
     } else {
         bh_launch_order(c.B, c.m.nlay, perm + 4, p.Lcut, perm, c.st);
+        c.order_wgs = 1;
         c.split = (p.Lcut < c.Lmax) ? perm : nullptr;
     }
     c.perm = perm + 4;
@@ -917,7 +932,7 @@
     for (int t = 0; t < n; ++t) lane_waves += (long)((B + 63) / 64) * p.look[t];
     e->guard_last = p.any_fast;
     ra.B = B; ra.Lmax = c.Lmax; ra.nlay = c.m.nlay; ra.neval = c.counter; ra.counted = e->swd_scan;
-    if (p.any_fast && ((rc = guard_space(e, c.st, B, &c.gcounts, &c.glists)) || (rc = swd_board(e, c.st, &ra.board)))) return rc;
+    if (p.any_fast && (rc = swd_board(e, c.st, &ra.board))) return rc;
     e->last_swd_kernel = BH_KERNEL_LANE;
     ev_begin(e, 0, c.st);
     if (fork && (rc = wait_for(e, e->ev_fork2, c.st, e->aux2))) return rc;
@@ -988,7 +1003,6 @@
     }
     e->guard_last = p.any_fast;
     if (p.any_fast) {
-        if ((rc = guard_space(e, c.st, B, &c.gcounts, &c.glists))) return rc;
         for (int t = 0; t < a.ntargets; ++t)
             if (a.t[t].igr == BH_VEL_PHASE) {
                 a.t[t].gcount = c.gcounts + t;
@@ -1058,13 +1072,18 @@
     return BH_OK;
 }
 
-int launch_swd_jobs(bh_engine *e, hipStream_t st, int B, int Lmax, const Staged &m, ptrdiff_t sl,
-                    ptrdiff_t sb, int njobs, const SwdJob *jobs, int prio_low, SwdLaunchInfo *main)
+SwdPlan plan_swd_call(const bh_engine *e, int B, int Lmax, const Staged &m, int njobs, const SwdJob *jobs)
+{
+    return plan_swd(e, B, Lmax, m.typ_layers > 0 ? m.typ_layers : e->hint_layers, njobs, jobs);
+}
+
+int launch_swd_jobs(bh_engine *e, hipStream_t st, int B, int Lmax, const Staged &m, ptrdiff_t sl, ptrdiff_t sb, int njobs,
+                    const SwdJob *jobs, const SwdPlan &p, const SwdFills &fills, int prio_low, SwdLaunchInfo *main)
 {
     if (B == 0 || njobs == 0) return BH_OK;
-    const SwdPlan p = plan_swd(e, B, Lmax, m.typ_layers > 0 ? m.typ_layers : e->hint_layers, njobs, jobs);
     SwdCall c{e, st, B, Lmax, m, sl, sb, jobs, p};
     c.prio_low = prio_low;
+    c.fills = fills;
     if (p.kernel == BH_KERNEL_GROUP) {
         c.g = plan_group(e, p, B, Lmax, jobs);
         if (!c.g.fits) return fail(e, BH_EINVAL, "model too deep for LDS");
@@ -1085,7 +1104,13 @@
         bh_launch_sphere(B, Lmax, m.nlay, m.h, m.vp, m.vs, m.rho, sl, sb, base, base + ne, base + 2 * ne, base + 3 * ne, base + 4 * ne, st);
         c.sph = base;
     }
-    if ((rc = swd_counter(e, st, &c.counter)) || (rc = order_models(c))) return rc;
+    SwdFills *const prologue = p.prologue ? &c.fills : nullptr;
+    if ((rc = swd_counter(e, st, prologue, &c.counter))) return rc;
+    if (p.any_fast && (rc = guard_space(e, st, B, prologue, &c.gcounts, &c.glists))) return rc;
+    if ((rc = order_models(c))) return rc;
+    e->last_swd_order[0] = p.order;
+    e->last_swd_order[1] = c.order_wgs;
+    e->last_swd_order[2] = !p.prologue ? 0 : (c.fills.nguard > 0 ? BH_FILL_GUARD : 0) | (c.fills.nerr > 0 ? BH_FILL_FLAGS : 0) | (c.fills.ncounter > 0 ? BH_FILL_COUNTERS : 0);
     SwdMultiArgs a{};
     rc = p.kernel == BH_KERNEL_LANE ? launch_swd_lanes(c, a) : launch_swd_multi(c, a);
     if (main) *main = c.info;
@@ -1292,6 +1317,12 @@
 }
 int bh_engine_get_swd_arith(const bh_engine *e) { return e ? e->swd_arith : 0; }
 int bh_engine_last_swd_kernel(const bh_engine *e) { return e ? e->last_swd_kernel : -1; }
+int bh_engine_last_swd_order(const bh_engine *e, int *workgroups, int *fills)
+{
+    if (workgroups) *workgroups = e ? e->last_swd_order[1] : 0;
+    if (fills) *fills = e ? e->last_swd_order[2] : 0;
+    return e ? e->last_swd_order[0] : -1;
+}
 int bh_engine_last_swd_launches(const bh_engine *e, bh_swd_launch *out, int max, int *n)
 {
     if (!e || !n || max < 0 || (max > 0 && !out)) return BH_EINVAL;
@@ -1503,7 +1534,7 @@
         job.periods_dev = (const double *)e->periods.p; job.vel = (double *)e->vel.p; job.err = (int32_t *)e->errb.p;
     }
     call_begin(e, st);
-    rc = launch_swd_jobs(e, st, B, Lmax, m, sl, sb, 1, &job, 0, nullptr);
+    rc = launch_swd_jobs(e, st, B, Lmax, m, sl, sb, 1, &job, plan_swd_call(e, B, Lmax, m, 1, &job), SwdFills{}, 0, nullptr);
     call_end(e, st);
     if (rc || !host) return rc;
     HIPCHK(e, hipMemcpyAsync(vel, e->vel.p, (size_t)B * K * sizeof(double), hipMemcpyDeviceToHost, st));
@@ -1723,11 +1754,6 @@
     const int B = p.B, nt = p.nt, ldy = p.ldy;
     hipStream_t st = c.st, rst = p.fork ? e->aux : st;
     int rc;
-    if (p.err_zero_always || e->err_t_nt != nt || e->err_t_B != B) {
-        HIPCHK(e, hipMemsetAsync(e->err_t.p, 0, (size_t)nt * B * sizeof(int32_t), st));
-        e->err_t_nt = nt;
-        e->err_t_B = B;
-    }
     SwdJob jobs[BH_MAX_TARGETS];
     int njobs = 0;
     const SwdSiteXArgs xtab{c.site, e->nsites, nt, ldy, (const int32_t *)e->site_xn.p, (const double *)e->site_xper.p, {}, {}};
@@ -1742,6 +1768,18 @@
             jobs[njobs++] = SwdJob{T.kfwd, d.iwave, d.igr, T.kfwd, (const double *)T.x60.p, (double *)T.vel60.p, errp, d.mode, d.flsph};
         }
     }
+    const SwdPlan sp = plan_swd_call(e, B, c.Lmax, c.m, njobs, jobs);
+    SwdFills fills{};
+    if (p.err_zero_always || e->err_t_nt != nt || e->err_t_B != B) {
+        if (sp.prologue) {
+            fills.err = (int32_t *)e->err_t.p;
+            fills.nerr = nt * B;
+        } else {
+            HIPCHK(e, hipMemsetAsync(e->err_t.p, 0, (size_t)nt * B * sizeof(int32_t), st));
+        }
+        e->err_t_nt = nt;
+        e->err_t_B = B;
+    }
     if (p.fork && (rc = wait_for(e, e->ev_fork, st, e->aux))) return rc;
     if (e->started != nullptr && e->started_expected > 0x70000000u) {
         HIPCHK(e, hipStreamSynchronize(st));
@@ -1750,7 +1788,7 @@
         e->started_expected = 0;
     }
     SwdLaunchInfo swd{};
-    if ((rc = launch_swd_jobs(e, st, B, c.Lmax, c.m, c.sl, c.sb, njobs, jobs, p.prio_low, &swd))) return rc;
+    if ((rc = launch_swd_jobs(e, st, B, c.Lmax, c.m, c.sl, c.sb, njobs, jobs, sp, fills, p.prio_low, &swd))) return rc;
     const bool gate = p.want_gate && swd.workgroups > 0;
     if (gate)
         HIPCHK(e, hipStreamWaitValue32(e->aux, e->started, e->started_expected - swd.workgroups + gate_need(swd), hipStreamWaitValueGte, 0xffffffffu));
diff --git a/bayhunter_amd/csrc/swd_kernel.hip b/bayhunter_amd/csrc/swd_kernel.hip
--- a/bayhunter_amd/csrc/swd_kernel.hip
+++ b/bayhunter_amd/csrc/swd_kernel.hip
@@ -223,14 +223,193 @@
 
 constexpr int PAIR_BUCKETS = 1024;
 constexpr int PAIR_MAX_B = 12288;
+constexpr int PAIR_BLOCKS = 8;
+constexpr int BLOCK_BUCKETS = PAIR_BUCKETS / PAIR_BLOCKS;
+constexpr int BLOCK_MAX_PER = PAIR_MAX_B / PAIR_BLOCKS;
+
+__device__ __forceinline__ void prologue_fills(const SwdFills &f, int tid, int nthreads)
+{
+    for (int i = tid; i < f.nguard; i += nthreads) f.guard[i] = 0;
+    for (int i = tid; i < f.nerr; i += nthreads) f.err[i] = 0;
+    for (int i = tid; i < f.ncounter; i += nthreads) f.counter[i] = 0ull;
+}
+
+__device__ __forceinline__ float pair_cost(const int32_t *nlay, const double *vs, ptrdiff_t sl, ptrdiff_t sb, int b, int Lmax, int &n)
+{
+    float lo = 1e30f, hi = -1e30f;
+    const double *col = vs + (ptrdiff_t)b * sb;
+    const int nraw = nlay[b];
+    auto sixteen = [&](int l0) {
+        double v[16];
+#pragma unroll
+        for (int k = 0; k < 16; ++k) {
+            const int l = l0 + k < Lmax ? l0 + k : Lmax - 1;
+            v[k] = col[(ptrdiff_t)l * sl];
+        }
+        __builtin_amdgcn_sched_barrier(0);
+        const int nl = nraw < 1 ? 1 : (nraw > Lmax ? Lmax : nraw);
+#pragma unroll
+        for (int k = 0; k < 16; ++k) {
+            const float f = (float)v[k];
+            if (l0 + k < nl) {
+                lo = f < lo ? f : lo;
+                hi = f > hi ? f : hi;
+            }
+        }
+    };
+    sixteen(0);
+    for (int l0 = 16; l0 < Lmax; l0 += 16) sixteen(l0);
+    n = nraw < 1 ? 1 : (nraw > Lmax ? Lmax : nraw);
+    const float c = hi - lo;
+    return (c >= 0.0f && c < 1e30f) ? c : 0.0f;
+}
+
+template <int PT>
+__global__ __launch_bounds__(1024) void pair_order_blocked_kernel(int B, int Lmax, const int32_t *nlay, const double *vs, ptrdiff_t sl,
+                                                                  ptrdiff_t sb, int nt, PairOrderTarget t0, PairOrderTarget t1, SwdFills fills)
+{
+    __shared__ int bin[BLOCK_BUCKETS];
+    __shared__ int sorted[BLOCK_MAX_PER];
+    __shared__ unsigned cmin_bits, cmax_bits;
+    __shared__ int nmin, nmax, half_sum;
+    __shared__ int deeper[BH_MAX_LAYERS + 2], before[BH_MAX_LAYERS + 2];
+    const int tid = threadIdx.x, nth = blockDim.x, x = blockIdx.x;
+    const int per = B / PAIR_BLOCKS;
+    prologue_fills(fills, x * nth + tid, PAIR_BLOCKS * nth);
+    if (tid < BLOCK_BUCKETS) bin[tid] = 0;
+    if (tid == 0) {
+        cmin_bits = 0x7f800000u;
+        cmax_bits = 0u;
+        nmin = BH_MAX_LAYERS + 1;
+        nmax = 0;
+    }
+    __syncthreads();
+    float cost[PT];
+    int depth[PT];
+    {
+        unsigned tcmin = 0x7f800000u, tcmax = 0u;
+        int tnmin = BH_MAX_LAYERS + 1, tnmax = 0;
+        int nb[8 * PT];
+#pragma unroll
+        for (int k = 0; k < 8 * PT; ++k) {
+            const int j = tid + nth * k;
+            nb[k] = nlay[j < B ? j : B - 1];
+        }
+#pragma unroll
+        for (int i = 0; i < PT; ++i) {
+            const int j = tid + nth * i;
+            cost[i] = 0.0f;
+            depth[i] = 1;
+            if (j >= per) continue;
+            const int b = x * per + j;
+            int n;
+            cost[i] = pair_cost(nlay, vs, sl, sb, b, Lmax, n);
+            depth[i] = n;
+            const unsigned cb = __float_as_uint(cost[i]);
+            tcmin = cb < tcmin ? cb : tcmin;
+            tcmax = cb > tcmax ? cb : tcmax;
+        }
+#pragma unroll
+        for (int k = 0; k < 8 * PT; ++k) {
+            const int n = nb[k] < 1 ? 1 : (nb[k] > Lmax ? Lmax : nb[k]);
+            tnmin = n < tnmin ? n : tnmin;
+            tnmax = n > tnmax ? n : tnmax;
+        }
+        for (int off = 32; off > 0; off >>= 1) {
+            tcmin = min(tcmin, (unsigned)__shfl_xor((int)tcmin, off));
+            tcmax = max(tcmax, (unsigned)__shfl_xor((int)tcmax, off));
+            tnmin = min(tnmin, __shfl_xor(tnmin, off));
+            tnmax = max(tnmax, __shfl_xor(tnmax, off));
+        }
+        if ((tid & (BH_WAVE - 1)) == 0) {
+            atomicMin(&cmin_bits, tcmin);
+            atomicMax(&cmax_bits, tcmax);
+            atomicMin(&nmin, tnmin);
+            atomicMax(&nmax, tnmax);
+        }
+    }
+    __syncthreads();
+    if (nmin != nmax) {
+        const int nbin = BH_MAX_LAYERS + 2, dmax = Lmax < BH_MAX_LAYERS + 1 ? Lmax : BH_MAX_LAYERS + 1;
+        for (int i = tid; i < nbin; i += nth) deeper[i] = before[i] = 0;
+        __syncthreads();
+        for (int j = tid; j < B; j += nth) {
+            int n = nlay[j];
+            n = n < 1 ? 1 : (n > dmax ? dmax : n);
+            atomicAdd(&deeper[n], 1);
+            if (j < x * per) atomicAdd(&before[n], 1);
+        }
+        __syncthreads();
+        if (tid == 0) {
+            int acc = 0;
+            for (int n = dmax; n >= 1; --n) {
+                const int c = deeper[n];
+                deeper[n] = acc + before[n];
+                acc += c;
+            }
+        }
+        __syncthreads();
+#pragma unroll
+        for (int i = 0; i < PT; ++i) {
+            const int j = tid + nth * i;
+            if (j >= per) continue;
+            const int n = depth[i] > dmax ? dmax : depth[i];
+            const int pos = atomicAdd(&deeper[n], 1);
+            t0.perm[pos] = x * per + j;
+            if (nt > 1) t1.perm[pos] = x * per + j;
+        }
+        return;
+    }
+    const float cmin = __uint_as_float(cmin_bits), cmax = __uint_as_float(cmax_bits);
+    const float scale = (cmax > cmin) ? (float)(BLOCK_BUCKETS - 1) / (cmax - cmin) : 0.0f;
+    int bucket[PT];
+#pragma unroll
+    for (int i = 0; i < PT; ++i) {
+        const int k = (int)((cmax - cost[i]) * scale);
+        bucket[i] = k < 0 ? 0 : (k > BLOCK_BUCKETS - 1 ? BLOCK_BUCKETS - 1 : k);
+        if (tid + nth * i < per) atomicAdd(&bin[bucket[i]], 1);
+    }
+    __syncthreads();
+    int mine = 0, acc = 0;
+    if (tid < BLOCK_BUCKETS) {
+        const int lane = tid & (BH_WAVE - 1);
+        mine = acc = bin[tid];
+        for (int off = 1; off < BH_WAVE; off <<= 1) {
+            const int o = __shfl_up(acc, off);
+            if (lane >= off) acc += o;
+        }
+        if (tid == BH_WAVE - 1) half_sum = acc;
+    }
+    __syncthreads();
+    if (tid < BLOCK_BUCKETS) bin[tid] = (tid >= BH_WAVE ? half_sum : 0) + acc - mine;
+    __syncthreads();
+#pragma unroll
+    for (int i = 0; i < PT; ++i)
+        if (tid + nth * i < per) sorted[atomicAdd(&bin[bucket[i]], 1)] = tid + nth * i;
+    __syncthreads();
+    for (int t = 0; t < nt; ++t) {
+        const PairOrderTarget T = t == 0 ? t0 : t1;
+#pragma unroll
+        for (int i = 0; i < PT; ++i) {
+            const int j = tid + nth * i;
+            if (j >= per) continue;
+            const int q = j / T.mpw, m = j - q * T.mpw;
+            const int wid = (T.xcd == 2) ? (((q >> 1) << 4) | (x << 1) | (q & 1)) : (((q >> 2) << 5) | (x << 2) | (q & 3));
+            T.perm[wid * T.mpw + m] = x * per + sorted[j];
+        }
+    }
+}
+
 __global__ __launch_bounds__(1024) void pair_order_kernel(int B, int Lmax, const int32_t *nlay, const double *vs, ptrdiff_t sl, ptrdiff_t sb,
-                                                          int nt, PairOrderTarget t0, PairOrderTarget t1)
+                                                          int nt, PairOrderTarget t0, PairOrderTarget t1, SwdFills fills)
 {
     __shared__ int bin[PAIR_BUCKETS];
     __shared__ int sorted[PAIR_MAX_B];
     __shared__ unsigned cmin_bits, cmax_bits;
     __shared__ int nmin, nmax;
     const int tid = threadIdx.x;
+    prologue_fills(fills, tid, 1024);
+    if (nt == 0) return;
     for (int i = tid; i < PAIR_BUCKETS; i += 1024) bin[i] = 0;
     if (tid == 0) {
         cmin_bits = 0x7f800000u;
@@ -284,15 +463,12 @@
     }
     __syncthreads();
     const bool ragged = nmin != nmax;
-    const bool blocked = !ragged && t0.xcd > 0;
-    const int per = B / 8;
     const float cmin = __uint_as_float(cmin_bits), cmax = __uint_as_float(cmax_bits);
     const float scale = (cmax > cmin) ? (float)(PAIR_BUCKETS - 1) / (cmax - cmin) : 0.0f;
     auto bucket = [&](int i) {
         if (ragged) return (nmax - depth[i]) < PAIR_BUCKETS ? (nmax - depth[i]) : PAIR_BUCKETS - 1;
         int k = (int)((cmax - cost[i]) * scale);
         k = k < 0 ? 0 : (k > PAIR_BUCKETS - 1 ? PAIR_BUCKETS - 1 : k);
-        if (blocked) k = ((tid + 1024 * i) / per) * (PAIR_BUCKETS / 8) + (k >> 3);
         return k;
     };
 #pragma unroll
@@ -332,11 +508,6 @@
             const int wid = pos / T.mpw, m = pos - wid * T.mpw;
             int src = pos;
             if (!ragged && T.slot_rank != nullptr && wid < T.nwaves - 1) src = T.slot_rank[wid] * T.mpw + m;
-            if (blocked) {
-                const int x = (T.xcd == 2) ? (wid >> 1) & 7 : (wid >> 2) & 7;
-                const int q = (T.xcd == 2) ? (((wid >> 4) << 1) | (wid & 1)) : (((wid >> 5) << 2) | (wid & 3));
-                src = x * per + q * T.mpw + m;
-            }
             T.perm[pos] = sorted[src];
         }
     }
@@ -456,10 +627,27 @@
     hipLaunchKernelGGL(order_kernel, dim3(1), dim3(1024), 0, stream, B, nlay, perm, Lcut, split);
 }
 
-void bh_launch_pair_order(int B, int Lmax, const int32_t *nlay, const double *vs, ptrdiff_t sl, ptrdiff_t sb, int nt,
-                          const PairOrderTarget *tg, hipStream_t stream)
-{
-    hipLaunchKernelGGL(pair_order_kernel, dim3(1), dim3(1024), 0, stream, B, Lmax, nlay, vs, sl, sb, nt, tg[0], tg[nt > 1 ? 1 : 0]);
+int bh_launch_pair_order(int B, int Lmax, const int32_t *nlay, const double *vs, ptrdiff_t sl, ptrdiff_t sb, int nt,
+                         const PairOrderTarget *tg, const SwdFills &fills, hipStream_t stream)
+{
+    bool blocked = nt > 0 && B > 0 && B <= PAIR_MAX_B && B % PAIR_BLOCKS == 0;
+    for (int t = 0; blocked && t < nt; ++t) {
+        const PairOrderTarget &T = tg[t];
+        blocked = (T.xcd == 2 || T.xcd == 4) && T.mpw > 0 && T.nwaves > 0 && (long)T.mpw * T.nwaves == B && T.nwaves % (PAIR_BLOCKS * T.xcd) == 0;
+    }
+    PairOrderTarget a = nt > 0 ? tg[0] : PairOrderTarget{}, b = nt > 1 ? tg[1] : a;
+    if (!blocked) {
+        hipLaunchKernelGGL(pair_order_kernel, dim3(1), dim3(1024), 0, stream, B, Lmax, nlay, vs, sl, sb, nt, a, b, fills);
+        return 1;
+    }
+    const int per = B / PAIR_BLOCKS;
+    if (per <= 1024) {
+        const int threads = per <= BLOCK_BUCKETS ? BLOCK_BUCKETS : (per + BH_WAVE - 1) / BH_WAVE * BH_WAVE;
+        hipLaunchKernelGGL(pair_order_blocked_kernel<1>, dim3(PAIR_BLOCKS), dim3(threads), 0, stream, B, Lmax, nlay, vs, sl, sb, nt, a, b, fills);
+    } else {
+        hipLaunchKernelGGL(pair_order_blocked_kernel<2>, dim3(PAIR_BLOCKS), dim3(1024), 0, stream, B, Lmax, nlay, vs, sl, sb, nt, a, b, fills);
+    }
+    return PAIR_BLOCKS;
 }
 bool bh_pair_order_fits(int B) { return B <= PAIR_MAX_B; }
 
diff --git a/bayhunter_amd/engine.py b/bayhunter_amd/engine.py
--- a/bayhunter_amd/engine.py
+++ b/bayhunter_amd/engine.py
@@ -115,6 +115,7 @@
     L.bh_engine_set_swd_arith.argtypes = [vp, C.c_int]
     L.bh_engine_last_swd_kernel.argtypes = [vp]
     L.bh_engine_last_swd_launches.argtypes = [vp, C.POINTER(SwdLaunch), C.c_int, C.POINTER(C.c_int)]
+    L.bh_engine_last_swd_order.argtypes = [vp, C.POINTER(C.c_int), C.POINTER(C.c_int)]
     L.bh_engine_set_swd_trials.argtypes = [vp, C.c_int]
     L.bh_engine_get_swd_trials.argtypes = [vp]
     L.bh_engine_get_swd_arith.argtypes = [vp]
@@ -204,6 +205,7 @@
                     "bh_swd_batch", "bh_rf_batch", "bh_targets_set", "bh_evaluate_batch", "bh_loglike_batch",
                     "bh_chain_propose", "bh_chain_accept", "bh_chain_propose_window", "bh_chain_accept_window")
 DEBUG_SYMBOLS = ("bh_engine_set_swd_group", "bh_engine_set_swd_lookahead", "bh_engine_last_swd_kernel", "bh_engine_last_swd_launches",
+                 "bh_engine_last_swd_order",
                  "bh_engine_set_swd_scan",
                  "bh_engine_get_swd_scan", "bh_engine_set_tuning",
                  "bh_engine_get_tuning", "bh_probe_math", "bh_engine_set_instrumentation", "bh_timing_reset",
@@ -355,6 +357,12 @@
                      key=tuple(r.key), two_classes=bool(r.two_classes), interleaved=bool(r.interleaved),
                      pair_order=bool(r.pair_order), restart=bool(r.restart), grid_x=int(r.grid_x), fair=int(r.fair))
                 for r in out[:n.value]]
+
+    def last_swd_order(self):
+        wg, fills = C.c_int(0), C.c_int(0)
+        order = self._L.bh_engine_last_swd_order(self._h, C.byref(wg), C.byref(fills))
+        return ({0: "none", 1: "depth", 2: "length", 3: "pair"}.get(order), int(wg.value),
+                {n for b, n in ((1, "guard"), (2, "flags"), (4, "counters")) if fills.value & b})
 
     def swd_arith(self):
         return "fast" if self._L.bh_engine_get_swd_arith(self._h) == ARITH_FAST else "exact"
diff --git a/include/bh_engine_debug.h b/include/bh_engine_debug.h
--- a/include/bh_engine_debug.h
+++ b/include/bh_engine_debug.h
@@ -24,6 +24,15 @@
 #define BH_SWD_SECOND 2
 int bh_engine_last_swd_launches(const bh_engine *e, bh_swd_launch *out, int max, int *n);
 
+#define BH_ORDER_NONE 0
+#define BH_ORDER_DEPTH 1
+#define BH_ORDER_LENGTH 2
+#define BH_ORDER_PAIR 3
+#define BH_FILL_GUARD 1
+#define BH_FILL_FLAGS 2
+#define BH_FILL_COUNTERS 4
+int bh_engine_last_swd_order(const bh_engine *e, int *workgroups, int *fills);
+
 #define BH_SCAN_STEPS 0
 #define BH_SCAN_COUNTED 1
 #define BH_SCAN_AUTO 2
```

New measurement: 6.177 million (median of 6 runs). 1.01x the previous value.
